# uci-cbcl/RP-Net

Hardware: AMD Instinct MI355X
Metric: support/query pairs/sec (fwd+bwd, 1-shot 256x256, T=5) (higher is better)
Workload: dtype f32

## Files before the change

include/rpnet_abi.h:

```cpp
#ifndef RPNET_ABI_H
#define RPNET_ABI_H

#include <stddef.h>
#include <stdint.h>

#ifdef __cplusplus
extern "C" {
#endif

typedef void* rpnet_stream_t;

enum rpnet_status {
    RPNET_OK = 0,
    RPNET_ERR_SHAPE = -1,
    RPNET_ERR_ARG = -2,
    RPNET_ERR_WORKSPACE = -3
};

#define RPNET_ABI_VERSION 109
int rpnet_version(void);
const char* rpnet_last_error_string(void);

int rpnet_pack_conv_weight(const float* w, float* wp, float* wd, int cout, int cin, int taps,
                           int cin_off0, int cin_split, int cin_off1, int cin_pad, rpnet_stream_t stream);

int rpnet_split_bf16(const float* x, const float* scale, int scale_mode, void* out, size_t rows, int C, int planes,
                     rpnet_stream_t stream);
int rpnet_predict_scales(const float* measured, float* bound, float* scale, int n, float safety, int check, int* violations,
                         rpnet_stream_t stream);
int rpnet_pow2_scale(const float* bound, float* s_out, rpnet_stream_t stream);
int rpnet_split_f16(const float* x, const float* mask, int mask_mode, const float* s_a, const float* s_b, float* s_out,
                    void* out, size_t rows, int C, int planes ,
                    int a_is_bound ,
                    rpnet_stream_t stream);
int rpnet_pack_conv_weight_split(const float* w, void* wp, void* wd, int cout, int cin, int taps, int cin_off0,
                                 int cin_split, int cin_off1, int cin_pad, int planes, float* row_scale_wp,
                                 float* row_scale_wd, rpnet_stream_t stream);
typedef struct rpnet_pack_item {
    const float* w; void* wp; void* wd;
    float* row_scale_wp; float* row_scale_wd;
    int cout, cin, taps, cin_off0, cin_split, cin_off1, cin_pad;
} rpnet_pack_item;
int rpnet_pack_conv_weights_split(const rpnet_pack_item* items, int n, int planes, rpnet_stream_t stream);

typedef struct rpnet_conv_desc {
    const float* x0; const float* x1;
    int C0, C1;
    const float* w;
    const float* bias;
    const float* in_scale;
    int in_scale_mode;
    float* y0; float* y1;
    int Co0, Co1;
    const float* ep_scale; const float* ep_shift;
    int ep_relu;
    const float* out_scale;
    int out_scale_mode;
    int accumulate;
    int N, H, W;
    int taps;
    int upsample;
    int groups;
    int dilation;
    double* stats_partial;
    int split_planes;
    void* y_split;
    int split_out_planes;
    const float* acc_scale_col; const float* acc_scale_x; const float* acc_scale_dy;
    const float* bnb_y; const float* bnb_stats; double* bnb_partial; float* bnb_pmax; int bnb_groups;
    const float* acc_scale_x1;
    float* out_absmax;
    int tune;
    const float* y_split_scale;
    void* splitk_ws;
    size_t splitk_ws_bytes;
    const float* skip_mask; int skip_mode; int skip_halo; unsigned char* skip_ws;
    const unsigned char* tile_skip;
    const float* y_enc; int y_enc_stride;
} rpnet_conv_desc;

int rpnet_conv_fwd(const rpnet_conv_desc* d, rpnet_stream_t stream);
int rpnet_conv_stats_blocks(const rpnet_conv_desc* d);
int rpnet_conv_tile_variant(const rpnet_conv_desc* d);
size_t rpnet_conv_splitk_workspace_bytes(const rpnet_conv_desc* d);

int rpnet_upconv_collapse_weights(const float* w, float* wc, int Cout, int Cin, rpnet_stream_t stream);
int rpnet_conv_up4_supported(const rpnet_conv_desc* d, int mode);
int rpnet_conv_up4_stats_blocks(const rpnet_conv_desc* d);
int rpnet_conv_up4(const rpnet_conv_desc* d, int mode, rpnet_stream_t stream);
int rpnet_conv_wgrad_up4_supported(const rpnet_conv_desc* d);
size_t rpnet_conv_wgrad_up4_workspace_bytes(int N, int H, int W, int cin, int cout);
int rpnet_conv_wgrad_up4(const rpnet_conv_desc* d, const void* dy, float* dw, void* workspace, size_t workspace_bytes,
                         rpnet_stream_t stream);

size_t rpnet_conv_wgrad_workspace_bytes(int N, int H, int W, int cin_gathered, int cout, int taps);
int rpnet_conv_wgrad(const rpnet_conv_desc* d, const float* dy, float* dw, int cin_w,
                     int cin_off0, int cin_split, int cin_off1,
                     void* workspace, size_t workspace_bytes, rpnet_stream_t stream);

int rpnet_conv1_fwd(const float* x, const float* w , const float* bias, float* y,
                    const float* ep_scale, const float* ep_shift, int N, int H, int W, int cout,
                    float* out_absmax ,
                    double* stats_partial ,
                    int groups, rpnet_stream_t stream);
int rpnet_conv1_stats_blocks(int N, int H, int W, int cout, int groups);
size_t rpnet_conv1_wgrad_workspace_bytes(int N, int H, int W, int cout);
int rpnet_conv1_wgrad(const float* x, const float* dy, float* dw, int N, int H, int W, int cout,
                      void* workspace, size_t workspace_bytes, rpnet_stream_t stream);
int rpnet_conv1_wgrad_bn(const float* x, const float* dz, const float* y ,
                         const float* stats, const float* coef, float* dw,
                         int N, int H, int W, int cout, int groups, void* workspace, size_t workspace_bytes,
                         const float* w , const float* bias, rpnet_stream_t stream);
int rpnet_conv1_bn_relu(const float* x, const float* w, const float* bias, const float* scale ,
                        const float* shift, float* z, void* z_split, int planes, const float* gamma, const float* beta,
                        float* split_scale, int N, int H, int W, int cout, int groups, rpnet_stream_t stream);
int rpnet_conv1_bn_bwd_rows(int N, int H, int W, int cout, int groups);
int rpnet_conv1_bn_bwd_partial(const float* x, const float* w, const float* bias, const float* dz,
                               const float* stats , double* partial,
                               int N, int H, int W, int cout, int groups, rpnet_stream_t stream);
int rpnet_conv1_dgrad_bn(const float* dz, const float* y, const float* stats, const float* coef, const float* w,
                         const float* bias, const float* x, float* dx, int N, int H, int W, int cout, int groups,
                         rpnet_stream_t stream);

size_t rpnet_bn_workspace_bytes(int C, int groups);
size_t rpnet_bn_bwd_coef_offset(int C, int groups);
int rpnet_bn_stats(const float* y, int N, int HW, int C, int groups, const float* gamma, const float* beta,
                   float* running_mean, float* running_var, long long* num_batches_tracked,
                   float momentum, float eps, float* scale, float* shift, float* mean, float* invstd,
                   void* workspace, size_t workspace_bytes, rpnet_stream_t stream);
int rpnet_bn_stats_from_partial(const double* partial, int nblk, int N, int HW, int C, int groups,
                                const float* gamma, const float* beta, float* running_mean, float* running_var,
                                long long* num_batches_tracked, float momentum, float eps, float* scale, float* shift, float* mean, float* invstd,
                                rpnet_stream_t stream);
int rpnet_bn_eval_affine(const float* gamma, const float* beta, const float* running_mean,
                         const float* running_var, float eps, float* scale, float* shift, int C,
                         rpnet_stream_t stream);
int rpnet_bn_relu(const float* y, const float* scale, const float* shift, float* z, void* z_split, int planes,
                  const float* gamma, const float* beta, float* split_scale, int N, int HW, int C, int groups,
                  int pool_w, const float* y_dec, int y_dec_stride, rpnet_stream_t stream);
int rpnet_bn_act_scale(const float* gamma, const float* beta, float* split_scale, int N, int HW, int C, int groups,
                       rpnet_stream_t stream);
int rpnet_bn_bwd(const float* dz, const float* y, const float* gamma, const float* scale, const float* shift,
                 const float* mean, const float* invstd, float* dy, void* dy_split, int planes, float* split_scale,
                 float* dgamma, float* dbeta, int N, int HW, int C, int groups, int accumulate,
                 const double* given_partial, const float* given_pmax, int given_rows ,
                 int pool_w, void* workspace, size_t workspace_bytes, const float* y_dec , int y_dec_stride,
                 rpnet_stream_t stream);

int rpnet_bn_eval_relu(const float* y, const float* scale, const float* shift, float* z, float* out_absmax, size_t P, int C,
                       rpnet_stream_t stream);
int rpnet_bn_eval_bwd(const float* dz, const float* y, const float* scale, const float* shift, const float* mean,
                      const float* invstd, float* dy, void* dy_split, int planes, float* split_scale, float* dgamma,
                      float* dbeta, int N, int HW, int C, int groups, int accumulate, void* workspace, size_t workspace_bytes,
                      rpnet_stream_t stream);

size_t rpnet_bias_relu_bwd_workspace_bytes(int C);
int rpnet_bias_relu_bwd(const float* dz, const float* z, float* dy, float* db, size_t P, int C,
                        void* workspace, size_t workspace_bytes, rpnet_stream_t stream);
int rpnet_maxpool3_fwd(const float* z, float* out, int N, int H, int W, int C, int stride, rpnet_stream_t stream);
int rpnet_maxpool3_bwd(const float* z, const float* dpool, float* dz, int N, int H, int W, int C, int stride,
                       rpnet_stream_t stream);

int rpnet_maxpool2_fwd(const float* z, float* out, int N, int H, int W, int C, rpnet_stream_t stream);
int rpnet_maxpool2_bwd(const float* z, const float* dpool, const float* skip, float* dz, int N, int H, int W,
                       int C, rpnet_stream_t stream);
int rpnet_upsample2_bwd(const float* dyu, float* dx, int N, int H, int W, int C, rpnet_stream_t stream);
int rpnet_sum_n(const float* const* srcs, int n, float* out, size_t numel, rpnet_stream_t stream);

int rpnet_mask_avgpool(const float* mask, float* out, int B, int H, int W, int scale, rpnet_stream_t stream);

int rpnet_local_corr_fwd(const float* f1, const float* f2, float* corr, int B, int h, int w, int C, int r,
                         int cstride, rpnet_stream_t stream);
size_t rpnet_local_corr_bwd_workspace_bytes(int B, int h, int w, int cstride);
int rpnet_local_corr_bwd(const float* f1, const float* f2, const float* dcorr, float* df1, float* df2,
                         int B, int h, int w, int C, int r, int cstride, const float* df1_add,
                         void* workspace, size_t workspace_bytes, rpnet_stream_t stream);
int rpnet_local_corr_split_fwd(const void* f1_split, const void* f2_split, float* corr, int B, int h, int w, int C, int r,
                               int cstride, int planes, const float* scale1, const float* scale2,
                               float* out_absmax ,
                               void* corr_planes ,
                               const float* corr_plane_scale, rpnet_stream_t stream);
int rpnet_local_corr_split_bwd(const void* f1_split, const void* f2_split, const float* dcorr, float* df1, float* df2,
                               int B, int h, int w, int C, int r, int cstride, int planes, const float* scale1,
                               const float* scale2, const float* df1_add, void* workspace, size_t workspace_bytes,
                               rpnet_stream_t stream);

int rpnet_mask_adjoint(const float* masks, float* am, float* msum, int B, int nmask, int H, int W, int h, int w,
                       rpnet_stream_t stream);
size_t rpnet_masked_pool_workspace_bytes(int B, int nmask, int hw, int C);
int rpnet_masked_pool_fwd(const float* f, const float* am, const float* msum, float* proto, int B, int nmask,
                          int hw, int C, void* workspace, size_t workspace_bytes, rpnet_stream_t stream);
int rpnet_masked_pool_bwd(const float* dproto, const float* am, const float* msum, float* df, int B, int nmask,
                          int hw, int C, int accumulate, rpnet_stream_t stream);

int rpnet_cosine_match_fwd(const float* f, const float* proto, float* pred, int B, int K, int hw, int C,
                           float scaler, rpnet_stream_t stream);
size_t rpnet_cosine_match_bwd_workspace_bytes(int B, int K, int hw, int C);
int rpnet_cosine_match_bwd(const float* f, const float* proto, const float* dpred, float* df, float* dproto,
                           int B, int K, int hw, int C, float scaler, int accumulate_df,
                           void* workspace, size_t workspace_bytes, rpnet_stream_t stream);

int rpnet_bilinear_up_fwd(const float* in, float* out, int planes, int h, int w, int H, int W, rpnet_stream_t stream);
int rpnet_bilinear_up_bwd(const float* dout, float* din, int planes, int h, int w, int H, int W, rpnet_stream_t stream);

int rpnet_softmax_thresh_pool(const float* logits, float* mask, int B, int K, int H, int W, int scale, int soft,
                              rpnet_stream_t stream);

int rpnet_refine_glue_supported(int K, int h, int w, int F, int C, int planes);
int rpnet_refine_glue_fwd(const float* y, const float* bn_scale, const float* bn_shift, const float* proto, float scaler,
                          float* z, float* pred, float* logits, float* mask_next, int soft, const float* x,
                          const float* x_scale, void* xk_planes, void* xq_planes, int planes, int B, int K, int h, int w,
                          int F, int C, rpnet_stream_t stream);
size_t rpnet_refine_glue_bwd_workspace_bytes(int B, int K, int h, int w, int F);
int rpnet_refine_glue_bwd(const float* dlogits, const float* f, const float* proto, float scaler, float* df, float* dproto,
                          int B, int K, int h, int w, int F, void* workspace, size_t workspace_bytes, rpnet_stream_t stream);

int rpnet_rowdot_scale(const float* g, const float* x, const float* scale, float* dx, float* dscale, size_t P, int C,
                       int mode, int accumulate_dscale, rpnet_stream_t stream);
int rpnet_softmax_pool_bwd(const float* logits, const float* dmask, float* dlogits, int B, int K, int H, int W,
                           int scale, rpnet_stream_t stream);

size_t rpnet_loss_workspace_bytes(int B, int K, int H, int W);
int rpnet_dice_ce_fwd(const float* logits, const int64_t* labels, float* loss, float* stats, int B, int K, int H,
                      int W, int with_dice, int ignore_index, int per_sample, const float* sample_weight,
                      void* workspace, size_t workspace_bytes, rpnet_stream_t stream);
int rpnet_dice_ce_bwd(const float* logits, const int64_t* labels, const float* stats, const float* gscale,
                      float* dlogits, int B, int K, int H, int W, int with_dice, int ignore_index, int per_sample,
                      const float* sample_weight, int accumulate, rpnet_stream_t stream);
int rpnet_dice_ce_multi_fwd(const float* const* logits, int n, const int64_t* labels, float* loss, float* stats, int B,
                            int K, int H, int W, void* workspace, size_t workspace_bytes, rpnet_stream_t stream);
int rpnet_dice_ce_multi_bwd(const float* const* logits, float* const* dlogits, int n, const int64_t* labels,
                            const float* stats, const float* gscale, int B, int K, int H, int W, rpnet_stream_t stream);
int rpnet_objective_fwd(const float* const* logits, const float* weights, int n, const int64_t* labels, const float* extra,
                        float extra_scale, float* loss, float* stats, int B, int K, int H, int W, void* workspace,
                        size_t workspace_bytes, rpnet_stream_t stream);
// ... 31 lines not shown
```

rpnet_amd/csrc/conv_epilogue.h:

```cpp
#pragma once
#include "common.h"
#include "split_bf16.h"

namespace rpnet {

struct LinearRows {
    static constexpr bool kAlwaysValid = false;
    int m0, M;
    __device__ __forceinline__ int operator()(int local) const { const int r = m0 + local; return r < M ? r : -1; }
};
template <int TW>
struct PatchRows {
    static constexpr bool kAlwaysValid = true;
    int base, W;
    __device__ __forceinline__ int operator()(int local) const { return base + (local / TW) * W + (local % TW); }
};

template <int WN, int WGM>
constexpr int epilogue_lds_bytes() {
    constexpr int stats = WGM * 64 * WN * (2 * 8 + 4), slabs = WGM * 2 * 32 * (WN * 32 + 4) * 4;
    return stats > slabs ? stats : slabs;
}
constexpr int cmax(int a, int b) { return a > b ? a : b; }

template <int WM, int WN, typename RowMap, bool AFF, bool ROWOPS>
__device__ __forceinline__ float conv_epilogue_store(const rpnet_conv_desc& d, f32x16 (&acc)[WM][WN], const RowMap rows, const int M,
                                                     const int Cout, const int per_group, const int n0, const int wm,
                                                     const int wn, const int li, const int h, float* slab, const int cso = 0) {
    constexpr int SW = WN * 32 + 4;
    const int lane = li + 32 * h;
    const int colbase = n0 + wn * WN * 32;
    const float xs = d.acc_scale_x ? *d.acc_scale_x : 1.f;
    float* dstb;
    int Cd, cd0;
    if (colbase < d.Co0) { dstb = d.y0; Cd = d.Co0; cd0 = colbase; } else { dstb = d.y1; Cd = d.Co1; cd0 = colbase - d.Co0; }
    float asv[WN], bvv[WN], es[WN], eh[WN];
    const int r_first = rows(wm * WM * 32), r_last = rows(wm * WM * 32 + WM * 32 - 1);
    const int g0 = (r_first >= 0 ? r_first : 0) / per_group;
    const bool one_group = !AFF || !d.ep_scale || RowMap::kAlwaysValid || (r_last >= 0 && r_last / per_group == g0);
#pragma unroll
    for (int j = 0; j < WN; ++j) {
        const int col = colbase + j * 32 + li;
        bvv[j] = d.bias ? d.bias[col] : 0.f;
        asv[j] = d.acc_scale_col ? d.acc_scale_col[col + cso] * xs : xs;
        es[j] = 1.f;
        eh[j] = 0.f;
        if (AFF && d.ep_scale) {
            es[j] = d.ep_scale[g0 * Cout + col];
            eh[j] = d.ep_shift[g0 * Cout + col];
        }
    }
    float amax = 0.f;
    constexpr int NQA = WN * 4;
    float sc_all[ROWOPS ? WM : 1][NQA];
    if (ROWOPS && d.out_scale_mode) {
#pragma unroll
        for (int i = 0; i < WM; ++i)
#pragma unroll
            for (int q = 0; q < NQA; ++q) {
                const int row = rows(wm * WM * 32 + i * 32 + (q * 64 + lane) / (WN * 8));
                const float f = (RowMap::kAlwaysValid || row >= 0) ? d.out_scale[row] : 0.f;
                sc_all[i][q] = d.out_scale_mode == 2 ? 1.f - f : f;
            }
    }
    unsigned short* ys = reinterpret_cast<unsigned short*>(d.y_split);
    const size_t yplane = (size_t)M * Cout;
    const float ysinv = (ROWOPS && d.y_split && d.y_split_scale) ? 1.f / *d.y_split_scale : 1.f;
#pragma unroll
    for (int i = 0; i < WM; ++i) {
#pragma unroll
        for (int r = 0; r < 16; ++r) {
            const int rl = (r & 3) + 8 * (r >> 2) + 4 * h;
#pragma unroll
            for (int j = 0; j < WN; ++j) {
                float v = acc[i][j][r] * asv[j] + bvv[j];
                if (AFF) {
                    if (one_group) v = v * es[j] + eh[j];
                    else {
                        const int row = rows(wm * WM * 32 + i * 32 + rl);
                        const int g = (row >= 0 ? row : 0) / per_group;
                        const int col = colbase + j * 32 + li;
                        v = v * d.ep_scale[g * Cout + col] + d.ep_shift[g * Cout + col];
                    }
                    if (d.ep_relu) v = fmaxf(v, 0.f);
                }
                slab[rl * SW + j * 32 + li] = v;
            }
        }
        __builtin_amdgcn_wave_barrier();
        constexpr int NQ = WN * 4;
        int orow[NQ];
        f32x4 v4[NQ];
#pragma unroll
        for (int q = 0; q < NQ; ++q) {
            const int gidx = q * 64 + lane;
            const int rr = gidx / (WN * 8), c4 = gidx - rr * (WN * 8);
            orow[q] = rows(wm * WM * 32 + i * 32 + rr);
            v4[q] = *reinterpret_cast<const f32x4*>(&slab[rr * SW + c4 * 4]);
        }
        if (ROWOPS) {
            if (d.out_scale_mode) {
#pragma unroll
                for (int q = 0; q < NQ; ++q) v4[q] *= sc_all[ROWOPS ? i : 0][q];
            }
            if (d.accumulate) {
                f32x4 prev[NQ];
#pragma unroll
                for (int q = 0; q < NQ; ++q) {
                    const int c4 = (q * 64 + lane) % (WN * 8);
                    prev[q] = (RowMap::kAlwaysValid || orow[q] >= 0) ? *reinterpret_cast<const f32x4*>(dstb + (size_t)orow[q] * Cd + cd0 + c4 * 4)
                                                                     : f32x4{0.f, 0.f, 0.f, 0.f};
                }
#pragma unroll
                for (int q = 0; q < NQ; ++q) v4[q] += prev[q];
            }
#pragma unroll
            for (int q = 0; q < NQ; ++q)
                if (RowMap::kAlwaysValid || orow[q] >= 0)
                    amax = fmaxf(fmaxf(amax, fmaxf(fabsf(v4[q][0]), fabsf(v4[q][1]))), fmaxf(fabsf(v4[q][2]), fabsf(v4[q][3])));
            if (d.y_split) {
#pragma unroll
                for (int q = 0; q < NQ; ++q) {
                    const int gidx = q * 64 + lane;
                    const int rr = gidx / (WN * 8), c4 = gidx - rr * (WN * 8);
                    *reinterpret_cast<f32x4*>(&slab[rr * SW + c4 * 4]) = v4[q];
                }
            }
        }
#pragma unroll
        for (int q = 0; q < NQ; ++q) {
            const int c4 = (q * 64 + lane) % (WN * 8);
            if (RowMap::kAlwaysValid || orow[q] >= 0)
                *reinterpret_cast<f32x4*>(dstb + (size_t)orow[q] * Cd + cd0 + c4 * 4) = v4[q];
        }
        __builtin_amdgcn_wave_barrier();
        if (ROWOPS && d.y_split) {
#pragma unroll
            for (int q = 0; q < 2 * WN; ++q) {
                const int gidx = q * 64 + lane;
                const int rr = gidx / (WN * 4), cg = gidx - rr * (WN * 4);
                const int row = rows(wm * WM * 32 + i * 32 + rr);
                if (RowMap::kAlwaysValid || row >= 0) {
                    const f32x4 a = *reinterpret_cast<const f32x4*>(&slab[rr * SW + cg * 8]);
                    const f32x4 b = *reinterpret_cast<const f32x4*>(&slab[rr * SW + cg * 8 + 4]);
                    float v8[8] = {a[0], a[1], a[2], a[3], b[0], b[1], b[2], b[3]};
                    const size_t o = (size_t)row * Cout + colbase + cg * 8;
                    if (d.split_out_planes == 3) {
                        u32x4 pl[3];
                        split8<3>(v8, pl);
#pragma unroll
                        for (int p = 0; p < 3; ++p) *reinterpret_cast<u32x4*>(ys + p * yplane + o) = pl[p];
                    } else {
#pragma unroll
                        for (int k = 0; k < 8; ++k) v8[k] *= ysinv;
                        if (d.split_out_planes == 2) {
                            u32x4 pl[2];
                            split8<2>(v8, pl);
#pragma unroll
                            for (int p = 0; p < 2; ++p) *reinterpret_cast<u32x4*>(ys + p * yplane + o) = pl[p];
                        } else {
                            u32x4 pl[1];
                            split8<1>(v8, pl);
                            *reinterpret_cast<u32x4*>(ys + o) = pl[0];
                        }
                    }
                }
            }
            __builtin_amdgcn_wave_barrier();
        }
    }
    return amax;
}

template <int WM, int WN, int WGM = 2, typename RowMap = LinearRows, bool WIDE = false>
__device__ __forceinline__ void conv_epilogue(const rpnet_conv_desc& d, f32x16 (&acc)[WM][WN], const RowMap rows,
                                              const int M, const int Cout, const int HW, const int n0, const int tm,
                                              const int wm, const int wn, const int li, const int h, void* lds, const int cso = 0) {
    const int per_group = d.groups > 0 ? (d.N / d.groups) * HW : M;
    const float xs = d.acc_scale_x ? *d.acc_scale_x : 1.f;
    if (d.stats_partial) {
        constexpr int BNC = 64 * WN;
        double* red = reinterpret_cast<double*>(lds);
        __syncthreads();
        bool valid[WM][16];
#pragma unroll
        for (int i = 0; i < WM; ++i)
#pragma unroll
            for (int r = 0; r < 16; ++r)
                valid[i][r] = RowMap::kAlwaysValid || rows(wm * WM * 32 + i * 32 + (r & 3) + 8 * (r >> 2) + 4 * h) >= 0;
#pragma unroll
        for (int j = 0; j < WN; ++j) {
            const int col = n0 + wn * WN * 32 + j * 32 + li;
            const float bv = d.bias ? d.bias[col] : 0.f;
            const float as = d.acc_scale_col ? d.acc_scale_col[col + cso] * xs : xs;
            double sm = 0.0, sq = 0.0;
#pragma unroll
            for (int i = 0; i < WM; ++i)
#pragma unroll
                for (int r = 0; r < 16; ++r) {
                    const double v = valid[i][r] ? (double)(acc[i][j][r] * as + bv) : 0.0;
                    sm += v;
                    sq += v * v;
                }
            sm += __shfl_xor(sm, 32, 64);
            sq += __shfl_xor(sq, 32, 64);
            if (h == 0) {
                double* o = red + ((size_t)wm * BNC + wn * WN * 32 + j * 32 + li) * 2;
                o[0] = sm;
                o[1] = sq;
            }
        }
        __syncthreads();
        for (int e = threadIdx.x; e < BNC * 2; e += WGM * 128) {
            double sacc = 0.0;
#pragma unroll
            for (int r = 0; r < WGM; ++r) sacc += red[(size_t)r * BNC * 2 + e];
            d.stats_partial[((size_t)tm * Cout + n0) * 2 + e] = sacc;
        }
    }
    __syncthreads();
    float* slab = reinterpret_cast<float*>(lds) + (size_t)(wm * 2 + wn) * 32 * (WN * 32 + 4);
    const bool aff = d.ep_scale != nullptr || d.ep_relu != 0;
    const bool rowops = d.out_scale_mode != 0 || d.accumulate != 0 || d.out_absmax != nullptr || d.y_split != nullptr;
    float amax = 0.f;
    if (!aff && !rowops) conv_epilogue_store<WM, WN, RowMap, false, false>(d, acc, rows, M, Cout, per_group, n0, wm, wn, li, h, slab, cso);
    else if (!aff) amax = conv_epilogue_store<WM, WN, RowMap, false, true>(d, acc, rows, M, Cout, per_group, n0, wm, wn, li, h, slab, cso);
    else if (!rowops) conv_epilogue_store<WM, WN, RowMap, true, false>(d, acc, rows, M, Cout, per_group, n0, wm, wn, li, h, slab, cso);
    else amax = conv_epilogue_store<WM, WN, RowMap, true, true>(d, acc, rows, M, Cout, per_group, n0, wm, wn, li, h, slab, cso);
    if (d.out_absmax) {
#pragma unroll
        for (int o = 32; o > 0; o >>= 1) amax = fmaxf(amax, __shfl_xor(amax, o, 64));
        if ((threadIdx.x & 63) == 0 && amax > __hip_atomic_load(d.out_absmax, __ATOMIC_RELAXED, __HIP_MEMORY_SCOPE_AGENT))
            atomicMax(reinterpret_cast<unsigned*>(d.out_absmax), __float_as_uint(amax));
    }
}

}
```

rpnet_amd/csrc/conv_igemm.hip:

```cpp
#include "conv_epilogue.h"

namespace rpnet {

template <int WM, int WN, bool INSCALE>
__global__ __launch_bounds__(256, (WM * WN >= 8 ? 2 : (WM * WN == 4 ? 3 : 4))) void conv_igemm_kernel(const rpnet_conv_desc d, const int M,
                                                          const int Cin, const int Cout,
                                                          const int tiles_n, const int ntiles) {
    constexpr int BM = 64 * WM, BN = 64 * WN, BK = 32;
    constexpr int ASTR = BK + 4;
    constexpr int A_F4 = BM / 32;
    constexpr int B_F4 = BN / 32;
    __shared__ __attribute__((aligned(16))) float smem[cmax(BM * ASTR + BK * BN, epilogue_lds_bytes<WN, 2>() / 4)];

    const int t = threadIdx.x;
    const int lane = t & 63, wv = t >> 6;
    const int li = lane & 31, h = lane >> 5;
    const int wm = wv >> 1, wn = wv & 1;

    const int tile = xcd_swizzle(blockIdx.x, ntiles);
    const int tm = tile / tiles_n, tn = tile - tm * tiles_n;
    const int m0 = tm * BM, n0 = tn * BN;

    const int H = d.H, W = d.W, HW = H * W;
    const int ups = d.upsample;
    const int Hs = H >> ups, Ws = W >> ups;
    const int dil = d.dilation > 1 ? d.dilation : 1;

    int rn[A_F4], ry[A_F4], rx[A_F4];
#pragma unroll
    for (int j = 0; j < A_F4; ++j) {
        const int m = m0 + (t >> 3) + 32 * j;
        if (m < M) {
            const int n = m / HW, rem = m - n * HW;
            rn[j] = n;
            ry[j] = rem / W;
            rx[j] = rem - ry[j] * W;
        } else {
            rn[j] = -1; ry[j] = 0; rx[j] = 0;
        }
    }
    const int acol = (t & 7) * 4;
    const int kchunks = Cin >> 5;
    const int nsteps = d.taps * kchunks;
    const int Cin4 = Cin >> 2;

    const int rot = (int)(blockIdx.x % (unsigned)kchunks);
    int l_tap = 0, l_c0 = rot << 5, l_kc = 0;
    const __amdgpu_buffer_rsrc_t rs0 = __builtin_amdgcn_make_buffer_rsrc(
        const_cast<float*>(d.x0), (short)0, (int)((size_t)d.N * Hs * Ws * d.C0 * 4), 0x00020000);
    const __amdgpu_buffer_rsrc_t rs1 = __builtin_amdgcn_make_buffer_rsrc(
        const_cast<float*>(d.x1 ? d.x1 : d.x0), (short)0, (int)((size_t)d.N * Hs * Ws * (d.x1 ? d.C1 : d.C0) * 4), 0x00020000);
    const __amdgpu_buffer_rsrc_t rsw = __builtin_amdgcn_make_buffer_rsrc(
        const_cast<float*>(d.w), (short)0, (int)((size_t)d.taps * Cin * Cout * 4), 0x00020000);
    int roff[A_F4];
    float rsc[A_F4];
    auto tap_setup = [&](int tap) {
        int ky = 0, kx = 0;
        if (d.taps == 9) { ky = (tap / 3 - 1) * dil; kx = (tap - (tap / 3) * 3 - 1) * dil; }
#pragma unroll
        for (int j = 0; j < A_F4; ++j) {
            const int iy = ry[j] + ky, ix = rx[j] + kx;
            const bool inb = rn[j] >= 0 && iy >= 0 && iy < H && ix >= 0 && ix < W;
            const int pix = (rn[j] * Hs + (iy >> ups)) * Ws + (ix >> ups);
            roff[j] = inb ? pix : -1;
            if (INSCALE) {
                const float sv = d.in_scale[inb ? pix : 0];
                rsc[j] = d.in_scale_mode == 2 ? 1.f - sv : sv;
            }
        }
    };
    tap_setup(0);
    int wvoff[B_F4];
#pragma unroll
    for (int j = 0; j < B_F4; ++j) {
        const int idx = t + 256 * j;
        const int k4 = idx / BN, nn = idx - k4 * BN;
        wvoff[j] = (k4 * Cout + nn) * 16;
    }

    f32x4 ra[A_F4], rb[B_F4];
    float rsc_st[A_F4];
    auto load_tile = [&]() {
        const bool first = l_c0 < d.C0;
        const int Cs = first ? d.C0 : d.C1;
        const int cc = first ? l_c0 : l_c0 - d.C0;
        const int soff = cc * 4;
        const int cs4 = Cs * 4, ac4 = acol * 4;
#pragma unroll
        for (int j = 0; j < A_F4; ++j) {
            const int voff = roff[j] * cs4 + ac4;
            ra[j] = first ? __builtin_bit_cast(f32x4, __builtin_amdgcn_raw_buffer_load_b128(rs0, voff, soff, 0))
                          : __builtin_bit_cast(f32x4, __builtin_amdgcn_raw_buffer_load_b128(rs1, voff, soff, 0));
            if (INSCALE) rsc_st[j] = rsc[j];
        }
        const int wsoff = ((l_tap * Cin4 + (l_c0 >> 2)) * Cout + n0) * 16;
#pragma unroll
        for (int j = 0; j < B_F4; ++j)
            rb[j] = __builtin_bit_cast(f32x4, __builtin_amdgcn_raw_buffer_load_b128(rsw, wvoff[j], wsoff, 0));
        l_c0 += 32;
        if (l_c0 == Cin) l_c0 = 0;
        if (++l_kc == kchunks) {
            l_kc = 0;
            if (++l_tap < d.taps) tap_setup(l_tap);
        }
    };
    auto store_tile = [&]() {
        float* As = smem;
        float* Bs = As + BM * ASTR;
#pragma unroll
        for (int j = 0; j < A_F4; ++j)
            *reinterpret_cast<f32x4*>(&As[((t >> 3) + 32 * j) * ASTR + acol]) = INSCALE ? ra[j] * rsc_st[j] : ra[j];
#pragma unroll
        for (int j = 0; j < B_F4; ++j) *reinterpret_cast<f32x4*>(&Bs[(t + 256 * j) * 4]) = rb[j];
    };

    f32x16 acc[WM][WN];
#pragma unroll
    for (int i = 0; i < WM; ++i)
#pragma unroll
        for (int j = 0; j < WN; ++j)
#pragma unroll
            for (int r = 0; r < 16; ++r) acc[i][j][r] = 0.f;

    auto mma_group = [&](const float* As, const float* Bs, int g) {
        f32x4 af[WM], bf[WN];
#pragma unroll
        for (int i = 0; i < WM; ++i)
            af[i] = *reinterpret_cast<const f32x4*>(&As[(wm * WM * 32 + i * 32 + li) * ASTR + g * 8 + h * 4]);
#pragma unroll
        for (int j = 0; j < WN; ++j)
            bf[j] = *reinterpret_cast<const f32x4*>(&Bs[((g * 2 + h) * BN + wn * WN * 32 + j * 32 + li) * 4]);
#pragma unroll
        for (int q = 0; q < 4; ++q)
#pragma unroll
            for (int i = 0; i < WM; ++i)
#pragma unroll
                for (int j = 0; j < WN; ++j)
                    acc[i][j] = __builtin_amdgcn_mfma_f32_32x32x2f32(af[i][q], bf[j][q], acc[i][j], 0, 0, 0);
    };

    load_tile();
    store_tile();
    __syncthreads();
    const float* As = smem;
    const float* Bs = As + BM * ASTR;
    for (int ks = 0; ks < nsteps; ++ks) {
        const bool more = ks + 1 < nsteps;
        if (more) load_tile();
        mma_group(As, Bs, 0);
        mma_group(As, Bs, 1);
        mma_group(As, Bs, 2);
        mma_group(As, Bs, 3);
        __syncthreads();
        if (more) store_tile();
        __syncthreads();
    }

    conv_epilogue<WM, WN>(d, acc, LinearRows{m0, M}, M, Cout, HW, n0, tm, wm, wn, li, h, smem);
}

template <int WM, int WN, bool INSCALE>
static int launch_igemm_t(const rpnet_conv_desc* d, int M, int Cin, int Cout, hipStream_t s) {
    constexpr int BM = 64 * WM, BN = 64 * WN;
    const int tiles_m = cdiv(M, BM), tiles_n = Cout / BN;
    const int ntiles = tiles_m * tiles_n;
    hipLaunchKernelGGL((conv_igemm_kernel<WM, WN, INSCALE>), dim3(ntiles), dim3(256), 0, s, *d, M, Cin, Cout, tiles_n, ntiles);
    return check_launch("conv_igemm");
}

template <int WM, int WN>
static int launch_igemm(const rpnet_conv_desc* d, int M, int Cin, int Cout, hipStream_t s) {
    if (d->in_scale_mode) return launch_igemm_t<WM, WN, true>(d, M, Cin, Cout, s);
    return launch_igemm_t<WM, WN, false>(d, M, Cin, Cout, s);
}

int choose_tile_split(const rpnet_conv_desc* d, int M, int Cout);
int split_tile_rows(int variant, int* wave_rows);
int conv_fwd_split(const rpnet_conv_desc* d, int M, int Cin, int Cout, hipStream_t s);
size_t conv_splitk_bytes(const rpnet_conv_desc* d, int M, int Cin, int Cout);

}


static int choose_tile(const rpnet_conv_desc* d, int M, int Cout) {
    const bool n128 = (Cout % 128 == 0) && (d->Co1 == 0 || d->Co0 % 128 == 0);
    struct Cand { int wm, wn, slots; } cands[4] = {{2, 2, 768}, {2, 1, 1024}, {1, 2, 1024}, {1, 1, 1536}};
    int best = -1;
    double best_fill = -1.0;
    for (int c = 0; c < 4; ++c) {
        if (cands[c].wn == 2 && !n128) continue;
        const long tiles = (long)rpnet::cdiv(M, 64 * cands[c].wm) * (Cout / (64 * cands[c].wn));
        const long waves = (tiles + cands[c].slots - 1) / cands[c].slots;
        const double fill = (double)tiles / (double)(waves * cands[c].slots);
        if (fill > best_fill + 0.02) { best_fill = fill; best = c; }
    }
    return best;
}

extern "C" int rpnet_conv_stats_blocks(const rpnet_conv_desc* d) {
    if (!d || d->groups < 1 || d->N % d->groups) return 0;
    const int M = d->N * d->H * d->W, Cout = d->Co0 + d->Co1;
    int bm, wave_rows = 2;
    if (d->split_planes) {
        bm = rpnet::split_tile_rows(rpnet::choose_tile_split(d, M, Cout), &wave_rows);
    } else {
        const int best = choose_tile(d, M, Cout);
        bm = (best == 0 || best == 1) ? 128 : 64;
    }
    const long per_group = (long)(d->N / d->groups) * d->H * d->W;
    if (per_group % bm) return 0;
    return (int)(per_group / bm);
}

extern "C" int rpnet_conv_tile_variant(const rpnet_conv_desc* d) {
    if (!d || !d->split_planes) return -1;
    return rpnet::choose_tile_split(d, d->N * d->H * d->W, d->Co0 + d->Co1);
}

extern "C" size_t rpnet_conv_splitk_workspace_bytes(const rpnet_conv_desc* d) {
    if (!d || !d->split_planes || d->taps != 9) return 0;
    return rpnet::conv_splitk_bytes(d, d->N * d->H * d->W, d->C0 + d->C1, d->Co0 + d->Co1);
}

extern "C" int rpnet_conv_fwd(const rpnet_conv_desc* d, rpnet_stream_t stream) {
    using namespace rpnet;
    RPNET_REQUIRE(d && d->x0 && d->w && d->y0, RPNET_ERR_ARG, "conv_fwd: null pointer");
    const int Cin = d->C0 + d->C1, Cout = d->Co0 + d->Co1;
    RPNET_REQUIRE(d->taps == 9 || d->taps == 1, RPNET_ERR_ARG, "conv_fwd: taps must be 9 or 1");
    RPNET_REQUIRE(Cin % 32 == 0 && d->C0 % 32 == 0 && (d->C1 == 0 || d->x1), RPNET_ERR_SHAPE,
                  "conv_fwd: Cin (%d+%d) must be a multiple of 32 per source", d->C0, d->C1);
    RPNET_REQUIRE(Cout % 64 == 0 && (d->Co1 == 0 || (d->y1 && d->Co0 % 64 == 0)), RPNET_ERR_SHAPE,
                  "conv_fwd: Cout (%d+%d) must be a multiple of 64 per destination", d->Co0, d->Co1);
    RPNET_REQUIRE(!d->stats_partial || rpnet_conv_stats_blocks(d) > 0, RPNET_ERR_SHAPE,
                  "conv_fwd: statistic groups do not split into whole tiles; use rpnet_bn_stats");
    RPNET_REQUIRE(!d->upsample || (d->H % 2 == 0 && d->W % 2 == 0), RPNET_ERR_SHAPE, "conv_fwd: odd size with upsample");
    RPNET_REQUIRE(!d->y_split || (d->Co1 == 0 && d->split_out_planes >= 1 && d->split_out_planes <= 3), RPNET_ERR_ARG,
                  "conv_fwd: y_split needs a single destination and 1 to 3 planes");
    RPNET_REQUIRE(!d->y_split || d->split_out_planes == 3 || d->y_split_scale, RPNET_ERR_ARG,
                  "conv_fwd: fp16 output planes (split_out_planes 1 / 2) need y_split_scale");
    RPNET_REQUIRE(!d->y_enc && !d->y_enc_stride, RPNET_ERR_ARG, "conv_fwd: y_enc / y_enc_stride are reserved (must be NULL / 0)");
    RPNET_REQUIRE(!d->bnb_y && !d->bnb_stats && !d->bnb_partial && !d->bnb_pmax, RPNET_ERR_ARG, "conv_fwd: the bnb_* fields are reserved (must be NULL)");
    RPNET_REQUIRE((long)d->N * d->H * d->W < (1L << 31), RPNET_ERR_SHAPE, "conv_fwd: too many pixels");
    RPNET_REQUIRE((size_t)d->N * d->H * d->W * (d->C0 > d->C1 ? d->C0 : d->C1) * 4 < (1UL << 31) &&
                      (size_t)d->taps * Cin * Cout * 4 < (1UL << 31),
                  RPNET_ERR_SHAPE, "conv_fwd: a source tensor exceeds the 2 GiB buffer-descriptor range");
    const int M = d->N * d->H * d->W;
    hipStream_t s = (hipStream_t)stream;
    if (d->split_planes) {
        RPNET_REQUIRE(d->split_planes >= 1 && d->split_planes <= 3 && d->in_scale_mode == 0, RPNET_ERR_ARG,
                      "conv_fwd: split operands take 1 to 3 planes and no in_scale (fold it into rpnet_split_bf16 / _f16)");
        RPNET_REQUIRE(d->split_planes == 3 || (d->acc_scale_col && d->acc_scale_x), RPNET_ERR_ARG,
                      "conv_fwd: one / two planes are fp16 planes of operand / scale: acc_scale_col and acc_scale_x are required");
        return conv_fwd_split(d, M, Cin, Cout, s);
    }
    const int best = choose_tile(d, M, Cout);
    switch (best) {
        case 0: return launch_igemm<2, 2>(d, M, Cin, Cout, s);
        case 1: return launch_igemm<2, 1>(d, M, Cin, Cout, s);
        case 2: return launch_igemm<1, 2>(d, M, Cin, Cout, s);
        default: return launch_igemm<1, 1>(d, M, Cin, Cout, s);
    }
}
```

rpnet_amd/csrc/conv_split.hip:

```cpp
#include <algorithm>

#include "conv_epilogue.h"
#include "split_bf16.h"

namespace rpnet {

constexpr bool IGLP = true;

template <int NP>
__global__ __launch_bounds__(256) void split_bf16_kernel(const float* __restrict__ x, const float* __restrict__ scale,
                                                          const int mode, unsigned short* __restrict__ out,
                                                          const size_t n8, const FastDiv fC, const size_t plane_elems) {
    RPNET_PASS_PRIORITY();
    for (size_t i = (size_t)blockIdx.x * 256 + threadIdx.x; i < n8; i += (size_t)gridDim.x * 256) {
        const f32x4 a = *reinterpret_cast<const f32x4*>(x + i * 8);
        const f32x4 b = *reinterpret_cast<const f32x4*>(x + i * 8 + 4);
        float v[8] = {a[0], a[1], a[2], a[3], b[0], b[1], b[2], b[3]};
        if (mode) {
            float s = scale[fC.div((unsigned)i)];
            if (mode == 2) s = 1.f - s;
#pragma unroll
            for (int q = 0; q < 8; ++q) v[q] *= s;
        }
        u32x4 o[NP];
// ... 240 lines not shown
    int roff[AJ];
    auto tap_setup = [&](int tap) {
        int ky = 0, kx = 0;
        if (d.taps == 9) { ky = (tap / 3 - 1) * dil; kx = (tap - (tap / 3) * 3 - 1) * dil; }
#pragma unroll
        for (int j = 0; j < AJ; ++j) {
            const int iy = ry[j] + ky, ix = rx[j] + kx;
            const bool inb = rn[j] >= 0 && iy >= 0 && iy < H && ix >= 0 && ix < W;
            roff[j] = inb ? (rn[j] * Hs + (iy >> ups)) * Ws + (ix >> ups) : -1;
        }
    };
    tap_setup(0);
    const bool stage_b = !B_PART || srow < BN;
    int wvoff[BJ];
#pragma unroll
    for (int j = 0; j < BJ; ++j) wvoff[j] = stage_b ? (srow + RP * j) * 64 + skg * 16 : -1;

    u32x4 ra[NP][AJ], rb[NP][BJ];
    auto load_tile = [&]() {
        const bool first = l_c0 < d.C0;
        const int Cs = first ? d.C0 : d.C1;
        const int cc = first ? l_c0 : l_c0 - d.C0;
        const int soff = cc * 2;
#pragma unroll
        for (int j = 0; j < AJ; ++j) {
            const int voff = roff[j] * (Cs * 2) + skg * 16;
#pragma unroll
            for (int p = 0; p < NP; ++p)
                ra[p][j] = first ? __builtin_bit_cast(u32x4, __builtin_amdgcn_raw_buffer_load_b128(rs0[p], voff, soff, 0))
                                 : __builtin_bit_cast(u32x4, __builtin_amdgcn_raw_buffer_load_b128(rs1[p], voff, soff, 0));
        }
        const int wsoff = ((l_tap * kchunks + (l_c0 >> 5)) * Cout + n0) * 64;
#pragma unroll
        for (int j = 0; j < BJ; ++j)
#pragma unroll
            for (int p = 0; p < NP; ++p)
                rb[p][j] = __builtin_bit_cast(u32x4, __builtin_amdgcn_raw_buffer_load_b128(rsw[p], wvoff[j], wsoff, 0));
        l_c0 += 32;
        if (l_c0 == Cin) l_c0 = 0;
        if (++l_kc == kchunks) {
            l_kc = 0;
            if (++l_tap < d.taps) tap_setup(l_tap);
        }
    };
    const int sdst = srow * 64 + 16 * (skg ^ ((srow >> 2) & 3));
    auto store_tile = [&](unsigned char* st) {
#pragma unroll
        for (int p = 0; p < NP; ++p) {
#pragma unroll
            for (int j = 0; j < AJ; ++j)
                *reinterpret_cast<u32x4*>(st + p * A_BYTES + j * (RP * 64) + sdst) = ra[p][j];
            if (stage_b) {
#pragma unroll
                for (int j = 0; j < BJ; ++j)
                    *reinterpret_cast<u32x4*>(st + NP * A_BYTES + p * B_BYTES + j * (RP * 64) + sdst) = rb[p][j];
            }
        }
    };

    f32x16 acc[WM][WN];
#pragma unroll
    for (int i = 0; i < WM; ++i)
#pragma unroll
        for (int j = 0; j < WN; ++j)
#pragma unroll
            for (int r = 0; r < 16; ++r) acc[i][j][r] = 0.f;

    const int sw = (li >> 2) & 3;
    const int a_row = (wm * WM * 32 + li) * 64, b_row = (wn * WN * 32 + li) * 64;
    auto mma_slice = [&](const unsigned char* st, int s) {
        const int koff = 16 * ((2 * s + h) ^ sw);
        bf16x8 af[NP][WM], bfr[NP][WN];
#pragma unroll
        for (int p = 0; p < NP; ++p) {
#pragma unroll
            for (int i = 0; i < WM; ++i)
                af[p][i] = *reinterpret_cast<const bf16x8*>(st + p * A_BYTES + a_row + i * 2048 + koff);
#pragma unroll
            for (int j = 0; j < WN; ++j)
                bfr[p][j] = *reinterpret_cast<const bf16x8*>(st + NP * A_BYTES + p * B_BYTES + b_row + j * 2048 + koff);
        }
        constexpr int NPROD = nprod<NP>();
#pragma unroll
        for (int q = 0; q < NPROD; ++q) {
            const int pa = prod_a<NP>(q), pb = prod_b<NP>(q);
#pragma unroll
            for (int i = 0; i < WM; ++i)
#pragma unroll
                for (int j = 0; j < WN; ++j)
                    acc[i][j] = mma16<NP>(af[pa][i], bfr[pb][j], acc[i][j]);
        }
    };

    const bool two_scales = d.acc_scale_x1 != nullptr && d.C1 > 0;
    const float r01 = two_scales ? *d.acc_scale_x / *d.acc_scale_x1 : 1.f;
    int cur_src = 0;
    auto enter_tile = [&](int ks) {
        if (!two_scales) return;
        int c = rot + ks;
        c -= (c / kchunks) * kchunks;
        const int src = (c << 5) < d.C0 ? 0 : 1;
        if (src != cur_src) {
            const float f = src ? r01 : 1.f / r01;
#pragma unroll
            for (int i = 0; i < WM; ++i)
#pragma unroll
                for (int j = 0; j < WN; ++j)
#pragma unroll
                    for (int r = 0; r < 16; ++r) acc[i][j][r] *= f;
            cur_src = src;
        }
    };
    if (DB) {
        load_tile();
        store_tile(smem);
        if (nsteps > 1) load_tile();
        __syncthreads();
        for (int ks = 0; ks < nsteps; ++ks) {
            enter_tile(ks);
            unsigned char* cur = smem + (ks & 1) * STAGE;
            unsigned char* nxt = smem + ((ks + 1) & 1) * STAGE;
            if (ks + 1 < nsteps) {
                store_tile(nxt);
                if (ks + 2 < nsteps) load_tile();
            }
            mma_slice(cur, 0);
            mma_slice(cur, 1);
            __syncthreads();
        }
    } else {
        load_tile();
        store_tile(smem);
        __syncthreads();
        for (int ks = 0; ks < nsteps; ++ks) {
            enter_tile(ks);
            const bool more = ks + 1 < nsteps;
            if (more) load_tile();
            mma_slice(smem, 0);
            mma_slice(smem, 1);
            __syncthreads();
            if (more) store_tile(smem);
            __syncthreads();
        }
    }
    if (two_scales && cur_src) {
        const float f = 1.f / r01;
#pragma unroll
        for (int i = 0; i < WM; ++i)
#pragma unroll
            for (int j = 0; j < WN; ++j)
#pragma unroll
                for (int r = 0; r < 16; ++r) acc[i][j][r] *= f;
    }
    conv_epilogue<WM, WN, WGM, LinearRows, NP == 1>(d, acc, LinearRows{m0, M}, M, Cout, HW, n0, tm, wm, wn, li, h, smem);
}

template <int TW, int NP, int WN>
__global__ __launch_bounds__(512, 1) void conv_igemm_split_halo_kernel(const rpnet_conv_desc d, const int Cin, const int Cout,
                                                                        const int tiles_n, const int ntiles) {
    constexpr int NT = 512, BM = 256, BN = 64 * WN, TH = BM / TW, PW = TW + 2, HALO = (TH + 2) * PW;
    constexpr int A_BYTES = HALO * 64, B_BYTES = BN * 64;
    constexpr int HJ = (HALO * 4 + NT - 1) / NT;
    constexpr int WM = 2;
    __shared__ __attribute__((aligned(16))) unsigned char smem[cmax(NP * A_BYTES + 2 * NP * B_BYTES, epilogue_lds_bytes<WN, 4>())];
    unsigned char* const bsm = smem + NP * A_BYTES;

    const int t = threadIdx.x;
    const int lane = t & 63, wv = t >> 6;
    const int li = lane & 31, h = lane >> 5;
    const int wm = wv >> 1, wn = wv & 1;

    const int tile = xcd_swizzle(blockIdx.x, ntiles);
    const int tm = tile / tiles_n, tn = tile - tm * tiles_n;
    const int n0 = tn * BN;
    const int H = d.H, W = d.W, HW = H * W;
    const int ups = d.upsample;
    const int Hs = H >> ups, Ws = W >> ups;
    const int pxn = W / TW, ppi = (H / TH) * pxn;
    const int n = tm / ppi, prem = tm - n * ppi;
    const int y0 = (prem / pxn) * TH, x0 = (prem % pxn) * TW;

    int hoff[HJ], hdst[HJ];
#pragma unroll
    for (int j = 0; j < HJ; ++j) {
        const int e = t + NT * j;
        const int hr = e >> 2, kg = e & 3;
        const int hy = hr / PW, hx = hr - hy * PW;
        const int iy = y0 + hy - 1, ix = x0 + hx - 1;
        const bool inb = e < HALO * 4 && iy >= 0 && iy < H && ix >= 0 && ix < W;
        hoff[j] = inb ? (n * Hs + (iy >> ups)) * Ws + (ix >> ups) : -1;
        hdst[j] = e < HALO * 4 ? hr * 64 + 16 * (kg ^ ((hr >> 2) & 3)) : -1;
    }
    const int skg16 = (t & 3) * 16;
    const int kchunks = Cin >> 5;
    const int nsteps = 9 * kchunks;
    const int rot = (int)(blockIdx.x % (unsigned)kchunks);
    auto chunk_c0 = [&](int ci) { int c = rot + ci; if (c >= kchunks) c -= kchunks; return c << 5; };

    const size_t plane0 = (size_t)d.N * Hs * Ws * d.C0, plane1 = (size_t)d.N * Hs * Ws * d.C1;
    const size_t planew = (size_t)9 * Cin * Cout;
    const unsigned short* x0p = reinterpret_cast<const unsigned short*>(d.x0);
    const unsigned short* x1p = reinterpret_cast<const unsigned short*>(d.x1 ? d.x1 : d.x0);
    const unsigned short* wq = reinterpret_cast<const unsigned short*>(d.w);
    __amdgpu_buffer_rsrc_t rs0[NP], rs1[NP], rsw[NP];
#pragma unroll
    for (int p = 0; p < NP; ++p) {
        rs0[p] = __builtin_amdgcn_make_buffer_rsrc(const_cast<unsigned short*>(x0p + p * plane0), (short)0,
                                                   (int)(plane0 * 2), 0x00020000);
        rs1[p] = __builtin_amdgcn_make_buffer_rsrc(const_cast<unsigned short*>(x1p + p * (d.x1 ? plane1 : plane0)), (short)0,
                                                   (int)((d.x1 ? plane1 : plane0) * 2), 0x00020000);
        rsw[p] = __builtin_amdgcn_make_buffer_rsrc(const_cast<unsigned short*>(wq + p * planew), (short)0,
                                                   (int)(planew * 2), 0x00020000);
    }
    u32x4 ha[NP][HJ], rb[NP];
    auto load_halo = [&](int c0) {
        const bool first = c0 < d.C0;
        const int Cs = first ? d.C0 : d.C1;
        const int soff = (first ? c0 : c0 - d.C0) * 2;
#pragma unroll
        for (int j = 0; j < HJ; ++j) {
            const int voff = hoff[j] * (Cs * 2) + skg16;
#pragma unroll
            for (int p = 0; p < NP; ++p)
                ha[p][j] = first ? __builtin_bit_cast(u32x4, __builtin_amdgcn_raw_buffer_load_b128(rs0[p], voff, soff, 0))
                                 : __builtin_bit_cast(u32x4, __builtin_amdgcn_raw_buffer_load_b128(rs1[p], voff, soff, 0));
        }
    };
    auto store_halo = [&]() {
#pragma unroll
        for (int p = 0; p < NP; ++p)
#pragma unroll
            for (int j = 0; j < HJ; ++j)
                if (hdst[j] >= 0) *reinterpret_cast<u32x4*>(smem + p * A_BYTES + hdst[j]) = ha[p][j];
    };
    const int brow = t >> 2;
    const bool stage_b = brow < BN;
    const int wvoff = stage_b ? brow * 64 + skg16 : -1;
    const int bdst = brow * 64 + 16 * ((t & 3) ^ ((brow >> 2) & 3));
    auto load_b = [&](int tap, int c0) {
        const int wsoff = ((tap * kchunks + (c0 >> 5)) * Cout + n0) * 64;
#pragma unroll
        for (int p = 0; p < NP; ++p)
            rb[p] = __builtin_bit_cast(u32x4, __builtin_amdgcn_raw_buffer_load_b128(rsw[p], wvoff, wsoff, 0));
    };
    auto store_b = [&](int stage) {
        if (stage_b) {
#pragma unroll
            for (int p = 0; p < NP; ++p) *reinterpret_cast<u32x4*>(bsm + (stage * NP + p) * B_BYTES + bdst) = rb[p];
        }
    };

    f32x16 acc[WM][WN];
#pragma unroll
    for (int i = 0; i < WM; ++i)
#pragma unroll
        for (int j = 0; j < WN; ++j)
#pragma unroll
            for (int r = 0; r < 16; ++r) acc[i][j][r] = 0.f;

    int hr00[WM];
#pragma unroll
    for (int i = 0; i < WM; ++i) {
        const int mloc = (wm * WM + i) * 32 + li;
        hr00[i] = (mloc / TW) * PW + (mloc % TW);
    }
    const int sw = (li >> 2) & 3;
    const int b_row = (wn * WN * 32 + li) * 64;
    auto mma_tap = [&](int tap, int stage) {
        const int ky = tap / 3, kx = tap - ky * 3;
        int arow[WM], asw[WM];
#pragma unroll
        for (int i = 0; i < WM; ++i) {
            const int hr = hr00[i] + ky * PW + kx;
            arow[i] = hr * 64;
            asw[i] = (hr >> 2) & 3;
        }
        const unsigned char* bst = bsm + stage * NP * B_BYTES;
#pragma unroll
        for (int s = 0; s < 2; ++s) {
            const int kg = 2 * s + h;
            bf16x8 af[NP][WM], bfr[NP][WN];
#pragma unroll
            for (int p = 0; p < NP; ++p) {
#pragma unroll
                for (int i = 0; i < WM; ++i)
                    af[p][i] = *reinterpret_cast<const bf16x8*>(smem + p * A_BYTES + arow[i] + 16 * (kg ^ asw[i]));
#pragma unroll
                for (int j = 0; j < WN; ++j)
                    bfr[p][j] = *reinterpret_cast<const bf16x8*>(bst + p * B_BYTES + b_row + j * 2048 + 16 * (kg ^ sw));
            }
            constexpr int NPROD = nprod<NP>();
#pragma unroll
            for (int q = 0; q < NPROD; ++q) {
                const int pa = prod_a<NP>(q), pb = prod_b<NP>(q);
#pragma unroll
                for (int i = 0; i < WM; ++i)
#pragma unroll
                    for (int j = 0; j < WN; ++j)
                        acc[i][j] = mma16<NP>(af[pa][i], bfr[pb][j], acc[i][j]);
            }
            if (NP <= 2 && IGLP) __builtin_amdgcn_iglp_opt(0);
        }
    };

    load_halo(chunk_c0(0));
    store_halo();
    load_b(0, chunk_c0(0));
    store_b(0);
    load_b(1, chunk_c0(0));
    __syncthreads();
    int ci = 0, tap = 0;
    for (int ks = 0; ks < nsteps; ++ks) {
        if (ks + 1 < nsteps) {
            store_b((ks + 1) & 1);
            if (ks + 2 < nsteps) {
                int t2 = tap + 2, c2 = ci;
                if (t2 >= 9) { t2 -= 9; ++c2; }
                load_b(t2, chunk_c0(c2));
            }
        }
        const bool next_chunk = ci + 1 < kchunks;
        if (tap == 0 && next_chunk) load_halo(chunk_c0(ci + 1));
        mma_tap(tap, ks & 1);
        __syncthreads();
        if (++tap == 9) {
            tap = 0;
            ++ci;
            if (next_chunk) {
                store_halo();
                __syncthreads();
            }
        }
    }
    conv_epilogue<WM, WN, 4, PatchRows<TW>, NP == 1>(d, acc, PatchRows<TW>{(n * H + y0) * W + x0, W}, d.N * HW, Cout, HW, n0, tm, wm, wn,
                                            li, h, smem);
}

template <int TW, int NP, int WN, int WMT = 2>
__global__ __launch_bounds__(256, 2) void conv_igemm_split_halo4_kernel(const rpnet_conv_desc d, const int Cin, const int Cout,
                                                                        const int tiles_n, const int ntiles) {
    constexpr int NT = 256, BM = 64 * WMT, BN = 64 * WN, TH = BM / TW, PW = TW + 2, HALO = (TH + 2) * PW;
    constexpr int A_BYTES = HALO * 64, B_BYTES = BN * 64;
    constexpr int HJ = (HALO * 4 + NT - 1) / NT;
    constexpr int WM = WMT;
    constexpr int BJ = (BN * 4 + NT - 1) / NT;
    __shared__ __attribute__((aligned(16))) unsigned char smem[cmax(NP * A_BYTES + NP * B_BYTES, epilogue_lds_bytes<WN, 2>())];
    unsigned char* const bsm = smem + NP * A_BYTES;

    const int t = threadIdx.x;
    const int lane = t & 63, wv = t >> 6;
    const int li = lane & 31, h = lane >> 5;
    const int wm = wv >> 1, wn = wv & 1;

    const int tile = xcd_swizzle(blockIdx.x, ntiles);
    const int tm = tile / tiles_n, tn = tile - tm * tiles_n;
    const int n0 = tn * BN;
    const int H = d.H, W = d.W, HW = H * W;
    const int ups = d.upsample;
    const int Hs = H >> ups, Ws = W >> ups;
    const int pxn = W / TW, ppi = (H / TH) * pxn;
    const int n = tm / ppi, prem = tm - n * ppi;
    const int y0 = (prem / pxn) * TH, x0 = (prem % pxn) * TW;

    int hoff[HJ], hdst[HJ];
#pragma unroll
    for (int j = 0; j < HJ; ++j) {
        const int e = t + NT * j;
        const int hr = e >> 2, kg = e & 3;
        const int hy = hr / PW, hx = hr - hy * PW;
        const int iy = y0 + hy - 1, ix = x0 + hx - 1;
        const bool inb = e < HALO * 4 && iy >= 0 && iy < H && ix >= 0 && ix < W;
        hoff[j] = inb ? (n * Hs + (iy >> ups)) * Ws + (ix >> ups) : -1;
        hdst[j] = e < HALO * 4 ? hr * 64 + 16 * (kg ^ ((hr >> 2) & 3)) : -1;
    }
    const int skg16 = (t & 3) * 16;
    const int kchunks = Cin >> 5;
    const int nsteps = 9 * kchunks;
    const int rot = (int)(blockIdx.x % (unsigned)kchunks);
    auto chunk_c0 = [&](int ci) { int c = rot + ci; if (c >= kchunks) c -= kchunks; return c << 5; };

    const size_t plane0 = (size_t)d.N * Hs * Ws * d.C0, plane1 = (size_t)d.N * Hs * Ws * d.C1;
    const size_t planew = (size_t)9 * Cin * Cout;
    const unsigned short* x0p = reinterpret_cast<const unsigned short*>(d.x0);
    const unsigned short* x1p = reinterpret_cast<const unsigned short*>(d.x1 ? d.x1 : d.x0);
    const unsigned short* wq = reinterpret_cast<const unsigned short*>(d.w);
    __amdgpu_buffer_rsrc_t rs0[NP], rs1[NP], rsw[NP];
#pragma unroll
    for (int p = 0; p < NP; ++p) {
        rs0[p] = __builtin_amdgcn_make_buffer_rsrc(const_cast<unsigned short*>(x0p + p * plane0), (short)0,
                                                   (int)(plane0 * 2), 0x00020000);
        rs1[p] = __builtin_amdgcn_make_buffer_rsrc(const_cast<unsigned short*>(x1p + p * (d.x1 ? plane1 : plane0)), (short)0,
                                                   (int)((d.x1 ? plane1 : plane0) * 2), 0x00020000);
        rsw[p] = __builtin_amdgcn_make_buffer_rsrc(const_cast<unsigned short*>(wq + p * planew), (short)0,
                                                   (int)(planew * 2), 0x00020000);
    }
    u32x4 ha[NP][HJ], rb[NP][BJ];
    auto load_halo = [&](int c0) {
        const bool first = c0 < d.C0;
        const int Cs = first ? d.C0 : d.C1;
        const int soff = (first ? c0 : c0 - d.C0) * 2;
#pragma unroll
        for (int j = 0; j < HJ; ++j) {
            const int voff = hoff[j] * (Cs * 2) + skg16;
#pragma unroll
            for (int p = 0; p < NP; ++p)
                ha[p][j] = first ? __builtin_bit_cast(u32x4, __builtin_amdgcn_raw_buffer_load_b128(rs0[p], voff, soff, 0))
                                 : __builtin_bit_cast(u32x4, __builtin_amdgcn_raw_buffer_load_b128(rs1[p], voff, soff, 0));
        }
    };
    auto store_halo = [&]() {
#pragma unroll
        for (int p = 0; p < NP; ++p)
#pragma unroll
            for (int j = 0; j < HJ; ++j)
                if (hdst[j] >= 0) *reinterpret_cast<u32x4*>(smem + p * A_BYTES + hdst[j]) = ha[p][j];
    };
    const int brow = t >> 2;
    const bool stage_b = brow < BN;
    const int bdst = brow * 64 + 16 * ((t & 3) ^ ((brow >> 2) & 3));
    auto load_b = [&](int tap, int c0) {
        const int wsoff = ((tap * kchunks + (c0 >> 5)) * Cout + n0) * 64;
#pragma unroll
        for (int j = 0; j < BJ; ++j) {
            const int wvoff = (brow + 64 * j) < BN ? (brow + 64 * j) * 64 + skg16 : -1;
#pragma unroll
            for (int p = 0; p < NP; ++p)
                rb[p][j] = __builtin_bit_cast(u32x4, __builtin_amdgcn_raw_buffer_load_b128(rsw[p], wvoff, wsoff, 0));
        }
    };
    auto store_b = [&]() {
#pragma unroll
        for (int j = 0; j < BJ; ++j)
            if (brow + 64 * j < BN) {
#pragma unroll
                for (int p = 0; p < NP; ++p) *reinterpret_cast<u32x4*>(bsm + p * B_BYTES + j * 4096 + bdst) = rb[p][j];
            }
    };
    (void)stage_b;

    f32x16 acc[WM][WN];
#pragma unroll
    for (int i = 0; i < WM; ++i)
#pragma unroll
        for (int j = 0; j < WN; ++j)
#pragma unroll
            for (int r = 0; r < 16; ++r) acc[i][j][r] = 0.f;

    int hr00[WM];
#pragma unroll
    for (int i = 0; i < WM; ++i) {
        const int mloc = (wm * WM + i) * 32 + li;
        hr00[i] = (mloc / TW) * PW + (mloc % TW);
    }
    const int sw = (li >> 2) & 3;
    const int b_row = (wn * WN * 32 + li) * 64;
    auto mma_tap = [&](int tap, int stage) {
        const int ky = tap / 3, kx = tap - ky * 3;
        int arow[WM], asw[WM];
#pragma unroll
        for (int i = 0; i < WM; ++i) {
            const int hr = hr00[i] + ky * PW + kx;
            arow[i] = hr * 64;
            asw[i] = (hr >> 2) & 3;
        }
        const unsigned char* bst = bsm + stage * NP * B_BYTES;
#pragma unroll
        for (int s = 0; s < 2; ++s) {
            const int kg = 2 * s + h;
            bf16x8 af[NP][WM], bfr[NP][WN];
#pragma unroll
            for (int p = 0; p < NP; ++p) {
#pragma unroll
                for (int i = 0; i < WM; ++i)
                    af[p][i] = *reinterpret_cast<const bf16x8*>(smem + p * A_BYTES + arow[i] + 16 * (kg ^ asw[i]));
#pragma unroll
                for (int j = 0; j < WN; ++j)
                    bfr[p][j] = *reinterpret_cast<const bf16x8*>(bst + p * B_BYTES + b_row + j * 2048 + 16 * (kg ^ sw));
            }
            constexpr int NPROD = nprod<NP>();
#pragma unroll
            for (int q = 0; q < NPROD; ++q) {
                const int pa = prod_a<NP>(q), pb = prod_b<NP>(q);
#pragma unroll
                for (int i = 0; i < WM; ++i)
#pragma unroll
                    for (int j = 0; j < WN; ++j)
                        acc[i][j] = mma16<NP>(af[pa][i], bfr[pb][j], acc[i][j]);
            }
        }
    };

    load_halo(chunk_c0(0));
    store_halo();
    load_b(0, chunk_c0(0));
    store_b();
    __syncthreads();
    int ci = 0, tap = 0;
    for (int ks = 0; ks < nsteps; ++ks) {
        const bool more = ks + 1 < nsteps;
        const bool next_chunk = ci + 1 < kchunks;
        if (more) {
            int t1 = tap + 1, c1 = ci;
            if (t1 == 9) { t1 = 0; ++c1; }
            load_b(t1, chunk_c0(c1));
        }
        if (WMT == 2 && tap == 0 && next_chunk) load_halo(chunk_c0(ci + 1));
        mma_tap(tap, 0);
        __syncthreads();
        if (more) store_b();
        if (tap == 8 && next_chunk) {
            if (WMT != 2) load_halo(chunk_c0(ci + 1));
            store_halo();
        }
        __syncthreads();
        if (++tap == 9) { tap = 0; ++ci; }
    }
    conv_epilogue<WM, WN, 2, PatchRows<TW>, NP == 1>(d, acc, PatchRows<TW>{(n * H + y0) * W + x0, W}, d.N * HW, Cout, HW, n0, tm, wm, wn,
                                            li, h, smem);
}

template <int TW, int WN>
static int launch_split_halo(const rpnet_conv_desc* d, int M, int Cin, int Cout, hipStream_t s) {
    const int tiles_m = M / 256, tiles_n = Cout / (64 * WN);
    const int ntiles = tiles_m * tiles_n;
    if (d->split_planes == 3)
        hipLaunchKernelGGL((conv_igemm_split_halo_kernel<TW, 3, WN>), dim3(ntiles), dim3(512), 0, s, *d, Cin, Cout, tiles_n, ntiles);
    else if (d->split_planes == 2)
        hipLaunchKernelGGL((conv_igemm_split_halo_kernel<TW, 2, WN>), dim3(ntiles), dim3(512), 0, s, *d, Cin, Cout, tiles_n, ntiles);
    else
        hipLaunchKernelGGL((conv_igemm_split_halo_kernel<TW, 1, WN>), dim3(ntiles), dim3(512), 0, s, *d, Cin, Cout, tiles_n, ntiles);
    return check_launch("conv_igemm_split_halo");
}

template <int TW, int WN, int WMT = 2>
static int launch_split_halo4(const rpnet_conv_desc* d, int M, int Cin, int Cout, hipStream_t s) {
    const int tiles_m = M / (64 * WMT), tiles_n = Cout / (64 * WN);
    const int ntiles = tiles_m * tiles_n;
    if (d->split_planes == 3) {
        if constexpr (WMT == 2)
            hipLaunchKernelGGL((conv_igemm_split_halo4_kernel<TW, 3, WN, WMT>), dim3(ntiles), dim3(256), 0, s, *d, Cin, Cout, tiles_n, ntiles);
        else {
            set_error("conv_igemm_split_halo4: the 4-wave 256-pixel form exists for fp16 planes only");
            return RPNET_ERR_ARG;
        }
    } else if (d->split_planes == 2)
        hipLaunchKernelGGL((conv_igemm_split_halo4_kernel<TW, 2, WN, WMT>), dim3(ntiles), dim3(256), 0, s, *d, Cin, Cout, tiles_n, ntiles);
    else
        hipLaunchKernelGGL((conv_igemm_split_halo4_kernel<TW, 1, WN, WMT>), dim3(ntiles), dim3(256), 0, s, *d, Cin, Cout, tiles_n, ntiles);
    return check_launch("conv_igemm_split_halo4");
}

static int halo_bn(const rpnet_conv_desc* d, int Cout) {
    return ((Cout % 128 == 0) && (d->Co1 == 0 || d->Co0 % 128 == 0)) ? 128 : 64;
}

static int halo_tw(const rpnet_conv_desc* d, int Cout) {
    if (d->taps != 9 || d->dilation > 1) return 0;
    if (d->W % 32 == 0 && d->H % 8 == 0) return 32;
    if (d->W % 16 == 0 && d->H % 16 == 0) return 16;
    return 0;
}

struct SplitVariant { int wgm, wm, wn, db, slots; };
static const SplitVariant kSplitVariants[] = {
    {2, 2, 2, 0, 768},
    {2, 2, 1, 0, 1024},
    {2, 1, 2, 0, 1024},
    {2, 1, 1, 0, 1536},
    {4, 2, 2, 1, 256},
    {4, 2, 2, 0, 256},
    {2, 2, 2, 1, 256},
    {4, 2, 2, 1, 256},
    {2, 2, 2, 0, 512},
    {2, 2, 1, 0, 512},
    {2, 4, 2, 0, 512},
    {2, 4, 2, 0, 256},
    {2, 4, 1, 0, 256},
    {2, 4, 2, 0, 256},
    {2, 2, 1, 0, 256},
};
constexpr int kNumSplitVariants = sizeof(kSplitVariants) / sizeof(kSplitVariants[0]);

template <int WGM, int WM, int WN, bool DB>
static int launch_split(const rpnet_conv_desc* d, int M, int Cin, int Cout, hipStream_t s) {
    constexpr int BM = 32 * WGM * WM, BN = 64 * WN;
    const int tiles_m = cdiv(M, BM), tiles_n = Cout / BN;
    const int ntiles = tiles_m * tiles_n;
    if (d->split_planes == 3)
        hipLaunchKernelGGL((conv_igemm_split_kernel<WGM, WM, WN, 3, DB>), dim3(ntiles), dim3(WGM * 128), 0, s, *d, M, Cin,
                           Cout, tiles_n, ntiles);
    else if (d->split_planes == 2)
        hipLaunchKernelGGL((conv_igemm_split_kernel<WGM, WM, WN, 2, DB>), dim3(ntiles), dim3(WGM * 128), 0, s, *d, M, Cin,
                           Cout, tiles_n, ntiles);
    else
        hipLaunchKernelGGL((conv_igemm_split_kernel<WGM, WM, WN, 1, DB>), dim3(ntiles), dim3(WGM * 128), 0, s, *d, M, Cin,
                           Cout, tiles_n, ntiles);
    return check_launch("conv_igemm_split");
}

static int halo4_tw(const rpnet_conv_desc* d) {
    if (d->taps != 9 || d->dilation > 1) return 0;
    if (d->W % 32 == 0 && d->H % 4 == 0) return 32;
    if (d->W % 16 == 0 && d->H % 8 == 0) return 16;
    return 0;
}

int conv_fwd_split_dma(const rpnet_conv_desc* d, int M, int Cin, int Cout, int tw, int wn, hipStream_t s, int parts = 1, int bm = 256);
int conv_splitk_parts(const rpnet_conv_desc* d, int M, int Cin, int Cout);

static bool dma_addressable(const rpnet_conv_desc* d, int Cout) {
    const size_t msrc = (size_t)d->N * (d->H >> d->upsample) * (d->W >> d->upsample);
    const size_t np = d->split_planes > 0 ? d->split_planes : 1, lim = (size_t)1 << 31;
    return np * msrc * d->C0 * 2 < lim && np * msrc * d->C1 * 2 < lim && np * 9 * (size_t)(d->C0 + d->C1) * Cout * 2 < lim;
}

int choose_tile_split(const rpnet_conv_desc* d, int M, int Cout) {
    const bool n128 = (Cout % 128 == 0) && (d->Co1 == 0 || d->Co0 % 128 == 0);
    const bool addr = dma_addressable(d, Cout);
    if (d->tune > 0) {
        const int v = (d->tune & 0xff) - 1;
        if ((v == 12 || v == 14) && d->split_planes == 2 && halo_tw(d, Cout) && addr) return v;
        if (v == 13 && d->split_planes == 1 && halo_tw(d, Cout) && halo_bn(d, Cout) == 128 && (d->C0 + d->C1) % 64 == 0 && d->C0 % 64 == 0 && addr)
            return v;
        if (((v == 7 || (v == 11 && d->split_planes == 2 && addr)) && halo_tw(d, Cout) &&
             halo_bn(d, Cout) == 128) ||
            ((v == 8 || v == 9) && halo4_tw(d)))
            return v;
        if (v >= 0 && v < 4 && (kSplitVariants[v].wn == 1 || n128)) return v;
    }
    const int hbn = halo_bn(d, Cout);
    if (d->split_planes == 1 && !(d->tune & 0x10000) && addr && hbn == 128 && halo_tw(d, Cout) && (d->C0 + d->C1) % 64 == 0 && d->C0 % 64 == 0 &&
        (long)(M / 256) * (Cout / 128) >= 192)
        return 13;
    const bool dma = d->split_planes == 2 && !(d->tune & 0x10000) && addr;
    if (hbn == 128 && halo_tw(d, Cout) && (long)(M / 256) * (Cout / 128) >= (dma ? 192 : 224)) return dma ? 11 : 7;
    if (dma && halo_tw(d, Cout) && d->C0 + d->C1 >= 128 && (long)(M / 256) * (Cout / 64) >= 128) return 12;
    if (halo4_tw(d)) {
        const long t8 = (long)(M / 128) * (Cout / hbn);
        if (hbn == 128 && t8 >= 1024) return 8;
        if ((long)(M / 128) * (Cout / 64) >= 64) return 9;
    }
    int best = -1;
    double best_fill = -1.0;
    for (int c = 0; c < 4; ++c) {
        const SplitVariant& v = kSplitVariants[c];
        if (v.wn == 2 && !n128) continue;
        const long tiles = (long)cdiv(M, 32 * v.wgm * v.wm) * (Cout / (64 * v.wn));
        const long waves = (tiles + v.slots - 1) / v.slots;
        const double fill = (double)tiles / (double)(waves * v.slots);
        if (fill > best_fill + 0.02) { best_fill = fill; best = c; }
    }
    return best;
}

int split_tile_rows(int variant, int* wave_rows) {
    const SplitVariant& v = kSplitVariants[variant];
    *wave_rows = v.wgm;
    return 32 * v.wgm * v.wm;
}

static int splitk_parts_for(const rpnet_conv_desc* d, int M, int Cin, int Cout) {
    if (!halo_tw(d, Cout) || !dma_addressable(d, Cout)) return 1;
    return conv_splitk_parts(d, M, Cin, Cout);
}

size_t conv_splitk_bytes(const rpnet_conv_desc* d, int M, int Cin, int Cout) {
    const int parts = splitk_parts_for(d, M, Cin, Cout);
    return parts > 1 ? (size_t)parts * M * Cout * sizeof(float) : 0;
}

// ... 120 lines not shown
```

rpnet_amd/csrc/conv_split_dma.hip:

```cpp
#include <type_traits>

#include "conv_epilogue.h"
#include "lds_dma.h"
#include "split_bf16.h"

namespace rpnet {

template <int N, int I = 0, typename F>
__device__ __forceinline__ void static_for(F&& f) {
    if constexpr (I < N) {
        f(std::integral_constant<int, I>{});
        static_for<N, I + 1>(f);
    }
}

template <int TW, int NP, int WN, bool K64 = false, int WM = 4>
__global__ __launch_bounds__(256, 1) void conv_igemm_split_dma_kernel(const rpnet_conv_desc d, const int Cin, const int Cout,
                                                                       const int tiles_n, const int ntiles, const int kshift) {
    constexpr int BM = 64 * WM, BN = 64 * WN, TH = BM / TW, PW = TW + 2, HALO = (TH + 2) * PW;
    constexpr int HP = (HALO + 15) / 16;
    constexpr int HPW = (HP + 3) / 4;
    constexpr int A_BYTES = HP * 1024, HBUF = NP * A_BYTES;
    constexpr int B_BYTES = BN * 64, STAGE = NP * B_BYTES;
    constexpr int NS = 4;
    constexpr int NW = WN * NP;
    static_assert(HPW <= 6, "halo pieces are issued during taps 0 .. HPW-1; the wait counts below assume HPW <= 6");
    __shared__ __attribute__((aligned(1024))) unsigned char smem[cmax(cmax(2 * HBUF + NS * STAGE, epilogue_lds_bytes<WN, 2>()),
                                                                       kLdsPerCu - kGuardedPassLds + 1024)];
    RPNET_ASSERT_NO_CORESIDENCE(sizeof(smem));
    constexpr int WOFF = 2 * HBUF;

    const int t = threadIdx.x;
    const int lane = t & 63;
    const int wv = __builtin_amdgcn_readfirstlane(t >> 6);
    const int li = lane & 31, h = lane >> 5;
    const int wm = wv >> 1, wn = wv & 1;

    const int tile = xcd_swizzle(blockIdx.x, ntiles);
    const int tm = uni(tile / tiles_n), tn = tile - tm * tiles_n;
    const int n0 = tn * BN;
    const int H = d.H, W = d.W, HW = H * W;
    const int ups = d.upsample;
    const int Hs = H >> ups, Ws = W >> ups;
    const int pxn = W / TW, ppi = (H / TH) * pxn;
    const int n = uni(tm / ppi), prem = tm - n * ppi;
    const int y0 = uni(prem / pxn) * TH, x0 = uni(prem % pxn) * TW;

    constexpr int CSH = K64 ? 6 : 5;
    const int kchunks = (Cin >> CSH) >> kshift;
    const int cbase = (int)blockIdx.y * kchunks;
    const int nsteps = 9 * kchunks;
    const int rot = uni((int)(blockIdx.x % (unsigned)kchunks));
    auto chunk_c0 = [&](int ci) { int c = rot + ci; if (c >= kchunks) c -= kchunks; return (cbase + c) << CSH; };

    const size_t plane0 = (size_t)d.N * Hs * Ws * d.C0, plane1 = (size_t)d.N * Hs * Ws * d.C1;
    const size_t planew = (size_t)9 * Cin * Cout;
    const unsigned short* x0p = reinterpret_cast<const unsigned short*>(d.x0);
    const unsigned short* x1p = reinterpret_cast<const unsigned short*>(d.x1 ? d.x1 : d.x0);
    const unsigned short* wq = reinterpret_cast<const unsigned short*>(d.w);
    const int pb0 = (int)(plane0 * 2), pb1 = (int)((d.x1 ? plane1 : plane0) * 2), pbw = (int)(planew * 2);
    constexpr int NPM = K64 ? 1 : NP;
    const __amdgpu_buffer_rsrc_t rs0 = __builtin_amdgcn_make_buffer_rsrc(const_cast<unsigned short*>(x0p), (short)0, NPM * pb0, 0x00020000);
    const __amdgpu_buffer_rsrc_t rs1 = __builtin_amdgcn_make_buffer_rsrc(const_cast<unsigned short*>(x1p), (short)0, NPM * pb1, 0x00020000);
    const __amdgpu_buffer_rsrc_t rsw = __builtin_amdgcn_make_buffer_rsrc(const_cast<unsigned short*>(wq), (short)0, NPM * pbw, 0x00020000);
    const int ps0 = K64 ? 64 : pb0, ps1 = K64 ? 64 : pb1, psw = K64 ? Cout * 64 : pbw;

    const int drow = lane >> 2;
    const int dkg16 = ((lane & 3) ^ ((lane >> 4) & 3)) * 16;
    int hoff[HPW];
    int hpos[HPW];
#pragma unroll
    for (int i = 0; i < HPW; ++i) {
        int pos = wv + 4 * i;
        if (pos >= HP) pos -= 4;
        hpos[i] = pos;
        const int hr = pos * 16 + drow;
        const int hy = hr / PW, hx = hr - hy * PW;
        const int iy = y0 + hy - 1, ix = x0 + hx - 1;
        const bool inb = hr < HALO && iy >= 0 && iy < H && ix >= 0 && ix < W;
        hoff[i] = inb ? (n * Hs + (iy >> ups)) * Ws + (ix >> ups) : -1;
    }
    auto dma_halo = [&](auto ic, int c0, int buf) {
        constexpr int i = decltype(ic)::value;
        const bool first = c0 < d.C0;
        const int Cs = first ? d.C0 : d.C1;
        const int soff = uni((first ? c0 : c0 - d.C0) * 2);
        const int voff = hoff[i] * (Cs * 2) + dkg16;
#pragma unroll
        for (int p = 0; p < NP; ++p) {
            auto* dst = (__attribute__((address_space(3))) void*)(smem + buf * HBUF + p * A_BYTES + hpos[i] * 1024);
            if (first) __builtin_amdgcn_raw_ptr_buffer_load_lds(rs0, dst, 16, voff, soff + p * ps0, 0, 0);
            else __builtin_amdgcn_raw_ptr_buffer_load_lds(rs1, dst, 16, voff, soff + p * ps1, 0, 0);
        }
    };
    const int wvoff = (16 * WN * wv + drow) * 64 + dkg16;
    auto dma_w = [&](int tap, int c0, int stage) {
        const int wsoff = uni(((tap * (Cin >> 5) + (c0 >> 5)) * Cout + n0) * 64);
#pragma unroll
        for (int p = 0; p < NP; ++p)
#pragma unroll
            for (int q = 0; q < WN; ++q) {
                auto* dst = (__attribute__((address_space(3))) void*)(smem + WOFF + stage * STAGE + p * B_BYTES + (16 * WN * wv + 16 * q) * 64);
                __builtin_amdgcn_raw_ptr_buffer_load_lds(rsw, dst, 16, wvoff + q * 1024, wsoff + p * psw, 0, 0);
            }
    };

    f32x16 acc[WM][WN];
#pragma unroll
    for (int i = 0; i < WM; ++i)
#pragma unroll
        for (int j = 0; j < WN; ++j)
#pragma unroll
            for (int r = 0; r < 16; ++r) acc[i][j][r] = 0.f;

    int hr00[WM];
#pragma unroll
    for (int i = 0; i < WM; ++i) {
        const int mloc = (wm * WM + i) * 32 + li;
        hr00[i] = (mloc / TW) * PW + (mloc % TW);
    }
    const int b_off = WOFF + (wn * WN * 32 + li) * 64 + 16 * (h ^ ((li >> 2) & 3));

    bf16x8 af[2][NP][WM], bfr[2][NP][WN];
    int aaddr[WM];
    auto a_addr_tap = [&](auto tapc) {
        constexpr int tap = decltype(tapc)::value;
        constexpr int ky = tap / 3, kx = tap - ky * 3;
#pragma unroll
        for (int i = 0; i < WM; ++i) {
            const int hr = hr00[i] + ky * PW + kx;
            aaddr[i] = hr * 64 + 16 * (h ^ ((hr >> 2) & 3));
        }
    };
    constexpr int NPROD = K64 ? 2 : nprod<NP>();
    constexpr int NR = NP * (WM + WN), NMMA = NPROD * WM * WN;
    static_assert(NR <= NMMA, "one fragment read of the next slice behind each MFMA of this one");
    auto read_frag = [&](auto sc, auto kc, const int abase, const int bbase) {
        constexpr int s = decltype(sc)::value, k = decltype(kc)::value;
        constexpr int grp = k / (WM + WN), r = k - grp * (WM + WN);
        constexpr int pa = K64 ? grp : NP - 1 - grp, pb = grp;
        if constexpr (r == 0 || r > WN) {
            constexpr int i = r == 0 ? 0 : r - WN;
            af[s][pa][i] = *reinterpret_cast<const bf16x8*>(smem + abase + (aaddr[i] ^ (32 * s)) + pa * A_BYTES);
        } else {
            constexpr int j = r - 1;
            bfr[s][pb][j] = *reinterpret_cast<const bf16x8*>(smem + bbase + (b_off ^ (32 * s)) + pb * B_BYTES + j * 2048);
        }
    };
    auto mma_one = [&](auto sc, auto mc) {
        constexpr int s = decltype(sc)::value, m = decltype(mc)::value;
        constexpr int q = m / (WM * WN), ij = m - q * (WM * WN), i = ij / WN, j = ij - i * WN;
        constexpr int pa = K64 ? q : prod_a<NP>(q), pb = K64 ? q : prod_b<NP>(q);
        acc[i][j] = mma16<NP>(af[s][pa][i], bfr[s][pb][j], acc[i][j]);
    };
    using I0 = std::integral_constant<int, 0>;
    using I1 = std::integral_constant<int, 1>;
    auto dma_w_one = [&](auto ec, const int wsoff, const int stage) {
        constexpr int e = decltype(ec)::value, p = e / WN, q = e - p * WN;
        auto* dst = (__attribute__((address_space(3))) void*)(smem + WOFF + stage * STAGE + p * B_BYTES + (16 * WN * wv + 16 * q) * 64);
        __builtin_amdgcn_raw_ptr_buffer_load_lds(rsw, dst, 16, wvoff + q * 1024, wsoff + p * psw, 0, 0);
    };

    const bool skip_tile = d.tile_skip != nullptr && d.tile_skip[tm] == 0;
    if (!skip_tile) {
    {
        const int c0 = chunk_c0(0);
        dma_halo(std::integral_constant<int, 0>{}, c0, 0);
        if constexpr (HPW > 1) dma_halo(std::integral_constant<int, 1>{}, c0, 0);
        if constexpr (HPW > 2) dma_halo(std::integral_constant<int, 2>{}, c0, 0);
        if constexpr (HPW > 3) dma_halo(std::integral_constant<int, 3>{}, c0, 0);
        if constexpr (HPW > 4) dma_halo(std::integral_constant<int, 4>{}, c0, 0);
        if constexpr (HPW > 5) dma_halo(std::integral_constant<int, 5>{}, c0, 0);
        dma_w(0, c0, 0);
        dma_w(1, c0, 1);
        dma_w(2, c0, 2);
    }
    static_assert(NW == 1 || NW == 2 || NW == 4, "weight DMAs per wave and step");
    if constexpr (NW == 4) asm volatile("s_waitcnt vmcnt(4)" ::: "memory");
    if constexpr (NW == 2) asm volatile("s_waitcnt vmcnt(2)" ::: "memory");
    if constexpr (NW == 1) asm volatile("s_waitcnt vmcnt(1)" ::: "memory");
    __builtin_amdgcn_s_barrier();
    a_addr_tap(I0{});
    static_for<NR>([&](auto kc) { read_frag(I0{}, kc, 0, 0); });

    auto step = [&](auto tapc, const int ci, const int ks) {
        constexpr int TAP = decltype(tapc)::value;
        const int hb = ci & 1;
        const bool last_chunk = ci + 1 >= kchunks;
        constexpr int t3 = TAP + 3 < 9 ? TAP + 3 : TAP - 6;
        const int c3 = chunk_c0((TAP + 3 < 9 || last_chunk) ? ci : ci + 1);
        const int wsoff = uni(((t3 * (Cin >> 5) + (c3 >> 5)) * Cout + n0) * 64);
        const int wstage = (ks + 3) & 3;
        const int abase = hb * HBUF, bbase = (ks & 3) * STAGE;
        static_for<NMMA>([&](auto mc) {
            constexpr int m = decltype(mc)::value;
            mma_one(I0{}, mc);
            __builtin_amdgcn_sched_barrier(0);
            if constexpr (m < NR) {
                read_frag(I1{}, mc, abase, bbase);
                __builtin_amdgcn_sched_barrier(0);
            }
            if constexpr (m >= NMMA - 2 * NW && (NMMA - 1 - m) % 2 == 0) {
                dma_w_one(std::integral_constant<int, NW - 1 - (NMMA - 1 - m) / 2>{}, wsoff, wstage);
                __builtin_amdgcn_sched_barrier(0);
            }
        });
        constexpr int TN = TAP < 8 ? TAP + 1 : 0;
        a_addr_tap(std::integral_constant<int, TN>{});
        const int abase_n = (TAP < 8 ? hb : hb ^ 1) * HBUF, bbase_n = ((ks + 1) & 3) * STAGE;
        __builtin_amdgcn_sched_barrier(0);
        static_for<NMMA>([&](auto mc) {
            constexpr int m = decltype(mc)::value;
            mma_one(I1{}, mc);
            __builtin_amdgcn_sched_barrier(0);
            if constexpr (m < NR) {
                read_frag(I0{}, mc, abase_n, bbase_n);
                __builtin_amdgcn_sched_barrier(0);
            }
            if constexpr (m == NMMA - 1 && TAP < HPW) {
                dma_halo(std::integral_constant<int, (TAP < HPW ? TAP : 0)>{}, chunk_c0(last_chunk ? ci : ci + 1), hb ^ 1);
                __builtin_amdgcn_sched_barrier(0);
            }
        });
        constexpr int HPREV = (TAP >= 1 && TAP - 1 < HPW) ? NP : 0;
        constexpr int HCUR = TAP < HPW ? NP : 0;
        constexpr int N = HPREV + NW + HCUR;
        static_assert(N == 1 || N == 2 || N == 3 || N == 4 || N == 6 || N == 8, "wait count");
        if constexpr (N == 1) asm volatile("s_waitcnt vmcnt(1)" ::: "memory");
        if constexpr (N == 2) asm volatile("s_waitcnt vmcnt(2)" ::: "memory");
        if constexpr (N == 3) asm volatile("s_waitcnt vmcnt(3)" ::: "memory");
        if constexpr (N == 4) asm volatile("s_waitcnt vmcnt(4)" ::: "memory");
        if constexpr (N == 6) asm volatile("s_waitcnt vmcnt(6)" ::: "memory");
        if constexpr (N == 8) asm volatile("s_waitcnt vmcnt(8)" ::: "memory");
        __builtin_amdgcn_s_barrier();
    };

    const int nchunks_run = ((d.tune >> 8) & 1) ? 1 : kchunks;
    int ks = 0;
    for (int ci = 0; ci < nchunks_run; ++ci) {
        step(std::integral_constant<int, 0>{}, ci, ks + 0);
        step(std::integral_constant<int, 1>{}, ci, ks + 1);
        step(std::integral_constant<int, 2>{}, ci, ks + 2);
        step(std::integral_constant<int, 3>{}, ci, ks + 3);
        step(std::integral_constant<int, 4>{}, ci, ks + 4);
        step(std::integral_constant<int, 5>{}, ci, ks + 5);
        step(std::integral_constant<int, 6>{}, ci, ks + 6);
        step(std::integral_constant<int, 7>{}, ci, ks + 7);
        step(std::integral_constant<int, 8>{}, ci, ks + 8);
        ks += 9;
    }
    (void)nsteps;
    asm volatile("s_waitcnt vmcnt(0)" ::: "memory");
    __builtin_amdgcn_s_barrier();
    }
    const int dbg = d.tune >> 8;
    if (dbg & 2) {
        float sacc = 0.f;
#pragma unroll
        for (int i = 0; i < WM; ++i)
#pragma unroll
            for (int j = 0; j < WN; ++j)
#pragma unroll
                for (int r = 0; r < 16; ++r) sacc += acc[i][j][r];
        if (sacc == 123.456f) d.y0[t] = sacc;
        return;
    }
    conv_epilogue<WM, WN, 2, PatchRows<TW>, false>(d, acc, PatchRows<TW>{(n * H + y0) * W + x0 + (int)blockIdx.y * d.N * HW, W},
                                                    d.N * HW, Cout, HW, n0, tm, wm, wn, li, h, smem);
}

__global__ __launch_bounds__(256) void conv_splitk_reduce_kernel(const float* __restrict__ ws, const int S, const size_t MC, const int Cout,
                                                                 const float* __restrict__ bias, const float* __restrict__ ep_scale,
                                                                 const float* __restrict__ ep_shift, const int relu, float* __restrict__ y,
                                                                 unsigned short* __restrict__ ys, const int planes,
                                                                 const float* __restrict__ ysc, float* __restrict__ out_absmax) {
    const size_t i = (size_t)blockIdx.x * 256 + threadIdx.x;
    float amax = 0.f;
    if (i * 8 < MC) {
        const int col = (int)((i * 8) % (size_t)Cout);
        f32x4 a = *reinterpret_cast<const f32x4*>(ws + i * 8), b = *reinterpret_cast<const f32x4*>(ws + i * 8 + 4);
        for (int s = 1; s < S; ++s) {
            a += *reinterpret_cast<const f32x4*>(ws + (size_t)s * MC + i * 8);
            b += *reinterpret_cast<const f32x4*>(ws + (size_t)s * MC + i * 8 + 4);
        }
        float v8[8] = {a[0], a[1], a[2], a[3], b[0], b[1], b[2], b[3]};
        if (bias) {
#pragma unroll
            for (int k = 0; k < 8; ++k) v8[k] += bias[col + k];
        }
        if (ep_scale) {
#pragma unroll
            for (int k = 0; k < 8; ++k) {
                v8[k] = v8[k] * ep_scale[col + k] + ep_shift[col + k];
                if (relu) v8[k] = fmaxf(v8[k], 0.f);
            }
        }
        *reinterpret_cast<f32x4*>(y + i * 8) = f32x4{v8[0], v8[1], v8[2], v8[3]};
        *reinterpret_cast<f32x4*>(y + i * 8 + 4) = f32x4{v8[4], v8[5], v8[6], v8[7]};
#pragma unroll
        for (int k = 0; k < 8; ++k) amax = fmaxf(amax, fabsf(v8[k]));
        if (ys) {
            if (planes == 3) {
                u32x4 pl[3];
                split8<3>(v8, pl);
#pragma unroll
                for (int p = 0; p < 3; ++p) *reinterpret_cast<u32x4*>(ys + p * MC + i * 8) = pl[p];
            } else {
                const float ysinv = 1.f / *ysc;
#pragma unroll
                for (int k = 0; k < 8; ++k) v8[k] *= ysinv;
                if (planes == 2) {
                    u32x4 pl[2];
                    split8<2>(v8, pl);
#pragma unroll
                    for (int p = 0; p < 2; ++p) *reinterpret_cast<u32x4*>(ys + p * MC + i * 8) = pl[p];
                } else {
                    u32x4 pl[1];
                    split8<1>(v8, pl);
                    *reinterpret_cast<u32x4*>(ys + i * 8) = pl[0];
                }
            }
        }
    }
    if (out_absmax) {
        __shared__ float wave_max[4];
#pragma unroll
        for (int o = 32; o > 0; o >>= 1) amax = fmaxf(amax, __shfl_xor(amax, o, 64));
        if ((threadIdx.x & 63) == 0) wave_max[threadIdx.x >> 6] = amax;
        __syncthreads();
        if (threadIdx.x == 0) {
            amax = fmaxf(fmaxf(wave_max[0], wave_max[1]), fmaxf(wave_max[2], wave_max[3]));
            if (amax > __hip_atomic_load(out_absmax, __ATOMIC_RELAXED, __HIP_MEMORY_SCOPE_AGENT))
                atomicMax(reinterpret_cast<unsigned*>(out_absmax), __float_as_uint(amax));
        }
    }
}

__global__ __launch_bounds__(64) void mask_tile_flags_kernel(const float* __restrict__ mask, const int mode, const int halo,
                                                              const int H, const int W, const int TW, const int TH,
                                                              unsigned char* __restrict__ flags) {
    const int tm = blockIdx.x, lane = threadIdx.x;
    const int pxn = W / TW, ppi = (H / TH) * pxn;
    const int n = tm / ppi, prem = tm - n * ppi;
    const int y0 = (prem / pxn) * TH - halo, x0 = (prem % pxn) * TW - halo;
    const int ph = TH + 2 * halo, pw = TW + 2 * halo;
    bool any = false;
    for (int i = lane; i < ph * pw; i += 64) {
        const int yy = y0 + i / pw, xx = x0 + i % pw;
        if (yy >= 0 && yy < H && xx >= 0 && xx < W) {
            const float m = mask[((size_t)n * H + yy) * W + xx];
            any = any || (mode == 2 ? (1.f - m) != 0.f : m != 0.f);
        }
    }
    const bool r = __any(any);
    if (lane == 0) flags[tm] = r ? 1 : 0;
}

int conv_splitk_parts(const rpnet_conv_desc* d, int M, int Cin, int Cout) {
    if (d->split_planes != 2 || d->tune != 0 || d->taps != 9 || d->dilation > 1 || Cin < 128 || M % 256) return 1;
    if (d->stats_partial || d->bnb_partial || d->bnb_y || d->accumulate || d->out_scale_mode || d->Co1 || d->y1 || d->acc_scale_x1 ||
        d->groups > 1)
        return 1;
    const long tiles = (long)(M / 256) * (Cout / 64);
    const int kchunks = Cin >> 5;
    if (tiles > 128 || (tiles > 64 && kchunks < 32)) return 1;
    int parts = 1;
    while (parts < 8 && tiles * parts * 2 <= 256 && kchunks % (parts * 2) == 0 && kchunks / (parts * 2) >= 2) parts *= 2;
    return parts;
}

int conv_fwd_split_dma(const rpnet_conv_desc* d, int M, int Cin, int Cout, int tw, int wn, hipStream_t s, int parts, int bm) {
    const int tiles_m = M / bm, tiles_n = Cout / (64 * wn);
    const int ntiles = tiles_m * tiles_n;
    rpnet_conv_desc dp = *d;
    dp.tile_skip = nullptr;
    if (d->skip_mask && d->skip_ws && (d->skip_mode == 1 || d->skip_mode == 2) && !d->upsample && d->H % (bm / tw) == 0 && d->W % tw == 0) {
        hipLaunchKernelGGL(mask_tile_flags_kernel, dim3(tiles_m), dim3(64), 0, s, d->skip_mask, d->skip_mode, d->skip_halo ? 1 : 0, d->H,
                           d->W, tw, bm / tw, d->skip_ws);
        dp.tile_skip = d->skip_ws;
    }
    int kshift = 0;
    if (parts > 1) {
        if (d->split_planes != 2 || wn != 1 || (size_t)parts * M * Cout * sizeof(float) > d->splitk_ws_bytes || !d->splitk_ws) {
            set_error("conv_igemm_split_dma: split K needs two planes, 64-wide tiles and the workspace");
            return RPNET_ERR_WORKSPACE;
        }
        while ((1 << kshift) < parts) ++kshift;
        dp.y0 = (float*)d->splitk_ws;
        dp.bias = nullptr; dp.ep_scale = nullptr; dp.ep_shift = nullptr; dp.ep_relu = 0;
        dp.out_absmax = nullptr; dp.y_split = nullptr; dp.split_out_planes = 0; dp.y_split_scale = nullptr;
    }
#define RPNET_DMA(TWV, WNV, K64V) \
    hipLaunchKernelGGL((conv_igemm_split_dma_kernel<TWV, 2, WNV, K64V>), dim3(ntiles, parts), dim3(256), 0, s, dp, Cin, Cout, tiles_n, ntiles, kshift)
    if (d->split_planes == 1) {
        if (wn != 2 || Cin % 64 || d->C0 % 64) {
            set_error("conv_igemm_split_dma: one plane needs 128-wide tiles and channel counts in multiples of 64 per source");
            return RPNET_ERR_ARG;
        }
        if (tw == 32) RPNET_DMA(32, 2, true); else RPNET_DMA(16, 2, true);
    } else if (d->split_planes == 2 && bm == 128) {
        if (wn != 1 || parts != 1) {
            set_error("conv_igemm_split_dma: 128-pixel patches come in 64-wide tiles, unsplit");
            return RPNET_ERR_ARG;
        }
        if (tw == 32)
            hipLaunchKernelGGL((conv_igemm_split_dma_kernel<32, 2, 1, false, 2>), dim3(ntiles, 1), dim3(256), 0, s, dp, Cin, Cout, tiles_n, ntiles, 0);
        else
            hipLaunchKernelGGL((conv_igemm_split_dma_kernel<16, 2, 1, false, 2>), dim3(ntiles, 1), dim3(256), 0, s, dp, Cin, Cout, tiles_n, ntiles, 0);
    } else if (d->split_planes == 2) {
        if (wn == 2) { if (tw == 32) RPNET_DMA(32, 2, false); else RPNET_DMA(16, 2, false); }
        else { if (tw == 32) RPNET_DMA(32, 1, false); else RPNET_DMA(16, 1, false); }
    } else {
        set_error("conv_igemm_split_dma: fp16 planes only");
        return RPNET_ERR_ARG;
    }
#undef RPNET_DMA
    if (parts > 1) {
        const size_t MC = (size_t)M * Cout;
        hipLaunchKernelGGL(conv_splitk_reduce_kernel, dim3((unsigned)((MC / 8 + 255) / 256)), dim3(256), 0, s, (const float*)d->splitk_ws, parts, MC,
                           Cout, d->bias, d->ep_scale, d->ep_shift, d->ep_relu, d->y0, (unsigned short*)d->y_split, d->split_out_planes,
                           d->y_split_scale, d->out_absmax);
    }
    return check_launch("conv_igemm_split_dma");
}

}
```

rpnet_amd/csrc/conv_up4_dma.hip:

```cpp
#include <type_traits>

#include "conv_epilogue.h"
#include "lds_dma.h"
#include "split_bf16.h"

namespace rpnet {

template <int N, int I = 0, typename F>
__device__ __forceinline__ void static_for_u(F&& f) {
    if constexpr (I < N) {
        f(std::integral_constant<int, I>{});
        static_for_u<N, I + 1>(f);
    }
}

template <int N>
__device__ __forceinline__ void wait_vmcnt() {
    static_assert(N >= 0 && N < 64, "vmcnt is a 6-bit counter");
    asm volatile("s_waitcnt vmcnt(%0)" ::"n"(N) : "memory");
}

template <int TW>
struct PatchRowsUp {
    static constexpr bool kAlwaysValid = true;
// ... 76 lines not shown
            const int ph = uni(c0 / C0);
            cs = c0 - ph * C0;
            pix += (ph >> 1) * W + (ph & 1);
        }
        const int voff = hok[i] ? pix * (C0 * 2) + dkg16 : (int)0x80000000;
#pragma unroll
        for (int p = 0; p < NP; ++p) {
            auto* dst = (__attribute__((address_space(3))) void*)(smem + buf * HBUF + p * A_BYTES + hpos[i] * 1024);
            __builtin_amdgcn_raw_ptr_buffer_load_lds(rs0, dst, 16, voff, uni(cs * 2) + p * ps0, 0, 0);
        }
    };
    const int wvoff = (16 * WN * wv + drow) * 64 + dkg16;
    auto w_soff = [&](int idx, int c0) { return uni(((idx * (Kc >> 5) + (c0 >> 5)) * Ncols + n0) * 64); };
    auto dma_w = [&](int idx, int c0, int stage) {
        const int wsoff = w_soff(idx, c0);
#pragma unroll
        for (int p = 0; p < NP; ++p)
#pragma unroll
            for (int q = 0; q < WN; ++q) {
                auto* dst = (__attribute__((address_space(3))) void*)(smem + WOFF + stage * STAGE + p * B_BYTES + (16 * WN * wv + 16 * q) * 64);
                __builtin_amdgcn_raw_ptr_buffer_load_lds(rsw, dst, 16, wvoff + q * 1024, wsoff + p * psw, 0, 0);
            }
    };

    f32x16 acc[WM][WN];
#pragma unroll
    for (int i = 0; i < WM; ++i)
#pragma unroll
        for (int j = 0; j < WN; ++j)
#pragma unroll
            for (int r = 0; r < 16; ++r) acc[i][j][r] = 0.f;

    int hr00[WM];
#pragma unroll
    for (int i = 0; i < WM; ++i) {
        const int mloc = (wm * WM + i) * 32 + li;
        hr00[i] = (mloc / TW) * PW + (mloc % TW);
    }
    const int b_off = WOFF + (wn * WN * 32 + li) * 64 + 16 * (h ^ ((li >> 2) & 3));

    bf16x8 af[2][NP][WM], bfr[2][NP][WN];
    int aaddr[WM];
    auto a_addr = [&](const int ky, const int kx) {
        const int off = ky * PW + kx;
#pragma unroll
        for (int i = 0; i < WM; ++i) {
            const int hr = hr00[i] + off;
            aaddr[i] = hr * 64 + 16 * (h ^ ((hr >> 2) & 3));
        }
    };
    constexpr int NPROD = K64 ? 2 : nprod<NP>();
    constexpr int NR = NP * (WM + WN), NMMA = NPROD * WM * WN;
    static_assert(NR <= NMMA, "one fragment read of the next slice behind each MFMA of this one");
    auto read_frag = [&](auto sc, auto kc, const int abase, const int bbase) {
        constexpr int s = decltype(sc)::value, k = decltype(kc)::value;
        constexpr int grp = k / (WM + WN), r = k - grp * (WM + WN);
        constexpr int pa = K64 ? grp : NP - 1 - grp, pb = grp;
        if constexpr (r == 0 || r > WN) {
            constexpr int i = r == 0 ? 0 : r - WN;
            af[s][pa][i] = *reinterpret_cast<const bf16x8*>(smem + abase + (aaddr[i] ^ (32 * s)) + pa * A_BYTES);
        } else {
            constexpr int j = r - 1;
            bfr[s][pb][j] = *reinterpret_cast<const bf16x8*>(smem + bbase + (b_off ^ (32 * s)) + pb * B_BYTES + j * 2048);
        }
    };
    auto mma_one = [&](auto sc, auto mc) {
        constexpr int s = decltype(sc)::value, m = decltype(mc)::value;
        constexpr int q = m / (WM * WN), ij = m - q * (WM * WN), i = ij / WN, j = ij - i * WN;
        constexpr int pa = K64 ? q : prod_a<NP>(q), pb = K64 ? q : prod_b<NP>(q);
        acc[i][j] = mma16<NP>(af[s][pa][i], bfr[s][pb][j], acc[i][j]);
    };
    using I0 = std::integral_constant<int, 0>;
    using I1 = std::integral_constant<int, 1>;
    auto dma_w_one = [&](auto ec, const int wsoff, const int stage) {
        constexpr int e = decltype(ec)::value, p = e / WN, q = e - p * WN;
        auto* dst = (__attribute__((address_space(3))) void*)(smem + WOFF + stage * STAGE + p * B_BYTES + (16 * WN * wv + 16 * q) * 64);
        __builtin_amdgcn_raw_ptr_buffer_load_lds(rsw, dst, 16, wvoff + q * 1024, wsoff + p * psw, 0, 0);
    };

    {
        const int c0 = chunk_c0(0);
        static_for_u<HPW>([&](auto ic) { dma_halo(ic, c0, 0); });
        dma_w(0, c0, 0);
        dma_w(1, c0, 1);
        dma_w(2, c0, 2);
        wait_vmcnt<NW>();
        __builtin_amdgcn_s_barrier();
        a_addr(chunk_py(c0), chunk_px(c0));
    }
    static_for_u<NR>([&](auto kc) { read_frag(I0{}, kc, 0, 0); });

    auto step = [&](auto idxc, const int ci, const int ks) {
        constexpr int IDX = decltype(idxc)::value;
        const int hb = ci & 1;
        const bool last_chunk = ci + 1 >= kchunks;
        constexpr int I3 = (IDX + 3) & 3;
        const int c3 = chunk_c0((IDX + 3 < 4 || last_chunk) ? ci : ci + 1);
        const int wsoff = w_soff(I3, c3);
        const int wstage = (ks + 3) & 3;
        const int abase = hb * HBUF, bbase = (ks & 3) * STAGE;
        static_for_u<NMMA>([&](auto mc) {
            constexpr int m = decltype(mc)::value;
            mma_one(I0{}, mc);
            __builtin_amdgcn_sched_barrier(0);
            if constexpr (m < NR) {
                read_frag(I1{}, mc, abase, bbase);
                __builtin_amdgcn_sched_barrier(0);
            }
            if constexpr (m >= NMMA - 2 * NW && (NMMA - 1 - m) % 2 == 0) {
                dma_w_one(std::integral_constant<int, NW - 1 - (NMMA - 1 - m) / 2>{}, wsoff, wstage);
                __builtin_amdgcn_sched_barrier(0);
            }
        });
        constexpr int IN = (IDX + 1) & 3;
        const int cn = chunk_c0((IDX < 3 || last_chunk) ? ci : ci + 1);
        a_addr(chunk_py(cn) + (IN >> 1), chunk_px(cn) + (IN & 1));
        const int abase_n = (IDX < 3 ? hb : hb ^ 1) * HBUF, bbase_n = ((ks + 1) & 3) * STAGE;
        const int ch = chunk_c0(last_chunk ? ci : ci + 1);
        __builtin_amdgcn_sched_barrier(0);
        static_for_u<NMMA>([&](auto mc) {
            constexpr int m = decltype(mc)::value;
            mma_one(I1{}, mc);
            __builtin_amdgcn_sched_barrier(0);
            if constexpr (m < NR) {
                read_frag(I0{}, mc, abase_n, bbase_n);
                __builtin_amdgcn_sched_barrier(0);
            }
            if constexpr (IDX == 0 && m >= NMMA - 3 * NPOS0 && (NMMA - 1 - m) % 3 == 0) {
                dma_halo(std::integral_constant<int, NPOS0 - 1 - (NMMA - 1 - m) / 3>{}, ch, hb ^ 1);
                __builtin_amdgcn_sched_barrier(0);
            }
            if constexpr (IDX == 1 && NPOS1 > 0 && m >= NMMA - 3 * NPOS1 && (NMMA - 1 - m) % 3 == 0) {
                dma_halo(std::integral_constant<int, NPOS0 + NPOS1 - 1 - (NMMA - 1 - m) / 3>{}, ch, hb ^ 1);
                __builtin_amdgcn_sched_barrier(0);
            }
        });
        constexpr int N = IDX == 0 ? NW + NPOS0 * NP : (IDX == 1 ? NPOS0 * NP + NW + NPOS1 * NP : NW);
        wait_vmcnt<N>();
        __builtin_amdgcn_s_barrier();
    };

    int ks = 0;
    for (int ci = 0; ci < kchunks; ++ci) {
        step(std::integral_constant<int, 0>{}, ci, ks + 0);
        step(std::integral_constant<int, 1>{}, ci, ks + 1);
        step(std::integral_constant<int, 2>{}, ci, ks + 2);
        step(std::integral_constant<int, 3>{}, ci, ks + 3);
        ks += 4;
    }
    asm volatile("s_waitcnt vmcnt(0)" ::: "memory");
    __builtin_amdgcn_s_barrier();

    if constexpr (DG) {
        conv_epilogue<WM, WN, 2, PatchRows<TW>, false>(d, acc, PatchRows<TW>{(n * Hl + y0) * Wl + x0, Wl}, d.N * Hl * Wl, Ncols, Hl * Wl, n0, tm,
                                                        wm, wn, li, h, smem);
    } else {
        conv_epilogue<WM, WN, 2, PatchRowsUp<TW>, false>(d, acc, PatchRowsUp<TW>{(n * H + 2 * y0 + fpy) * W + 2 * x0 + fpx, 2 * W}, d.N * H * W,
                                                          Cout_out, H * W, n0 - fphase * Cout_out, tm * 4 + fphase, wm, wn, li, h, smem,
                                                          fphase * Cout_out);
    }
}

__global__ __launch_bounds__(256) void upconv_collapse_kernel(const float* __restrict__ w, float* __restrict__ wc, const int Cout, const int Cin) {
    const size_t i = (size_t)blockIdx.x * 256 + threadIdx.x;
    if (i >= (size_t)4 * Cout * Cin) return;
    const int ci = (int)(i % Cin);
    const int co = (int)((i / Cin) % Cout), ph = (int)(i / ((size_t)Cin * Cout));
    const int py = ph >> 1, px = ph & 1;
    float k[9];
#pragma unroll
    for (int q = 0; q < 9; ++q) k[q] = w[((size_t)co * Cin + ci) * 9 + q];
    float o[4];
#pragma unroll
    for (int r = 0; r < 2; ++r)
#pragma unroll
        for (int c = 0; c < 2; ++c) {
            const int ya = r == 0 ? 0 : (py ? 2 : 1), yb = r == 0 ? (py ? 1 : 0) : 2;
            const int xa = c == 0 ? 0 : (px ? 2 : 1), xb = c == 0 ? (px ? 1 : 0) : 2;
            float s = 0.f;
            for (int ky = ya; ky <= yb; ++ky)
                for (int kx = xa; kx <= xb; ++kx) s += k[ky * 3 + kx];
            o[r * 2 + c] = s;
        }
    *reinterpret_cast<f32x4*>(wc + i * 4) = f32x4{o[0], o[1], o[2], o[3]};
}

static int up4_tw(int Hl, int Wl) {
    if (Wl % 32 == 0 && Hl % 8 == 0) return 32;
    if (Wl % 16 == 0 && Hl % 16 == 0) return 16;
    return 0;
}

static int up4_plan(const rpnet_conv_desc* d, int mode, int* tw, int* Kc, int* Ncols) {
    if (!d || (d->split_planes != 2 && d->split_planes != 1) || d->H % 2 || d->W % 2 || d->C1 || d->Co1 || d->x1 || d->y1) return 0;
    const int Hl = d->H / 2, Wl = d->W / 2;
    const bool one = d->split_planes == 1;
    *tw = up4_tw(Hl, Wl);
    if (!*tw || d->C0 % (one ? 64 : 32) || d->Co0 % (one ? 128 : 64)) return 0;
    *Kc = mode == 1 ? d->C0 : 4 * d->C0;
    *Ncols = mode == 1 ? 4 * d->Co0 : d->Co0;
    const size_t lim = (size_t)1 << 31;
    const size_t src = (size_t)d->N * (mode == 1 ? Hl * Wl : d->H * d->W) * d->C0 * 2 * d->split_planes;
    if (src >= lim || (size_t)2 * 4 * *Kc * *Ncols * 2 >= lim || (size_t)d->N * d->H * d->W >= lim) return 0;
    const long tiles_m = (long)d->N * Hl * Wl / 256;
    if (mode == 1) return (d->Co0 % 128 == 0) ? 2 : 1;
    if (one) return 2;
    return (*Ncols % 128 == 0 && tiles_m * (*Ncols / 128) >= 192) ? 2 : 1;
}

}

extern "C" int rpnet_conv_up4_supported(const rpnet_conv_desc* d, int mode) {
    int tw, Kc, Nc;
    return (mode == 1 || mode == 2) && rpnet::up4_plan(d, mode, &tw, &Kc, &Nc) > 0;
}

extern "C" int rpnet_conv_up4_stats_blocks(const rpnet_conv_desc* d) {
    int tw, Kc, Nc;
    if (!rpnet::up4_plan(d, 1, &tw, &Kc, &Nc) || d->groups < 1 || d->N % d->groups) return 0;
    return (int)((long)(d->N / d->groups) * d->H * d->W / 256);
}

extern "C" int rpnet_upconv_collapse_weights(const float* w, float* wc, int Cout, int Cin, rpnet_stream_t stream) {
    using namespace rpnet;
    RPNET_REQUIRE(w && wc && Cout > 0 && Cin > 0, RPNET_ERR_ARG, "upconv_collapse_weights: bad argument");
    hipLaunchKernelGGL(upconv_collapse_kernel, dim3(cdiv((long)4 * Cout * Cin, 256)), dim3(256), 0, (hipStream_t)stream, w, wc, Cout, Cin);
    return check_launch("upconv_collapse_weights");
}

extern "C" int rpnet_conv_up4(const rpnet_conv_desc* d, int mode, rpnet_stream_t stream) {
    using namespace rpnet;
    RPNET_REQUIRE(d && d->x0 && d->w && d->y0 && (mode == 1 || mode == 2), RPNET_ERR_ARG, "conv_up4: null pointer / mode");
    int tw = 0, Kc = 0, Nc = 0;
    const int wn = up4_plan(d, mode, &tw, &Kc, &Nc);
    RPNET_REQUIRE(wn > 0, RPNET_ERR_SHAPE, "conv_up4: N=%d H=%d W=%d C0=%d Co0=%d planes=%d do not fit (rpnet_conv_up4_supported)", d->N, d->H, d->W,
                  d->C0, d->Co0, d->split_planes);
    RPNET_REQUIRE(d->acc_scale_col && d->acc_scale_x, RPNET_ERR_ARG, "conv_up4: fp16 planes need acc_scale_col and acc_scale_x");
    RPNET_REQUIRE(mode == 1 || !d->stats_partial, RPNET_ERR_ARG, "conv_up4: statistics belong to the forward launch");
    RPNET_REQUIRE(!d->stats_partial || rpnet_conv_up4_stats_blocks(d) > 0, RPNET_ERR_SHAPE, "conv_up4: statistic groups do not split into whole tiles");
    RPNET_REQUIRE(!d->out_scale_mode && !d->y_split && !d->bnb_y && !d->tile_skip && !d->splitk_ws && !d->y_enc, RPNET_ERR_ARG,
                  "conv_up4: plain epilogue only (bias, eval affine, statistics, accumulate, out_absmax)");
    const int tiles_m = d->N * (d->H / 2) * (d->W / 2) / 256, tiles_n = Nc / (64 * wn), ntiles = tiles_m * tiles_n;
    hipStream_t s = (hipStream_t)stream;
#define RPNET_UP4(TWV, WNV, DGV) hipLaunchKernelGGL((conv_up4_dma_kernel<TWV, WNV, DGV>), dim3(ntiles), dim3(256), 0, s, *d, Kc, Nc, tiles_n, ntiles)
#define RPNET_UP4K(TWV, DGV) hipLaunchKernelGGL((conv_up4_dma_kernel<TWV, 2, DGV, true>), dim3(ntiles), dim3(256), 0, s, *d, Kc, Nc, tiles_n, ntiles)
    if (d->split_planes == 1) {
        if (mode == 1) { if (tw == 32) RPNET_UP4K(32, false); else RPNET_UP4K(16, false); }
        else { if (tw == 32) RPNET_UP4K(32, true); else RPNET_UP4K(16, true); }
    } else if (mode == 1) {
        if (tw == 32) { if (wn == 2) RPNET_UP4(32, 2, false); else RPNET_UP4(32, 1, false); }
        else { if (wn == 2) RPNET_UP4(16, 2, false); else RPNET_UP4(16, 1, false); }
    } else {
        if (tw == 32) { if (wn == 2) RPNET_UP4(32, 2, true); else RPNET_UP4(32, 1, true); }
        else { if (wn == 2) RPNET_UP4(16, 2, true); else RPNET_UP4(16, 1, true); }
    }
#undef RPNET_UP4
#undef RPNET_UP4K
    return check_launch("conv_up4");
}
```

rpnet_amd/functional.py:

```python
import collections
import ctypes as C
import os

import torch
from torch.autograd import Function
from torch.autograd.function import once_differentiable

from . import hip
from .hip import ConvDesc, call, ptr, query

BN_EPS = 1e-5
BN_MOMENTUM = 0.1

_ASYNC = {"on": False, "side": {}, "pending": set(), "queued": False, "fifo": [], "keep": []}

_MODES = {"f32": (0, False, 0), "bf16x3": (3, False, 0), "f16x2": (3, True, 2), "f16": (3, True, 1)}
_CORR16 = True
_CORR_PRED_PLANES = True
_MATH = {}


def set_conv_math(mode):
    _MATH["mode"] = mode
    _MATH["planes"], _MATH["f16"], _MATH["f16_planes"] = _MODES[mode]
# ... 210 lines not shown
    probe.N, probe.H, probe.W, probe.C0, probe.Co0, probe.split_planes = N, H, W, pw.cin, cout, planes
    probe.x0, probe.y0 = ptr(xs0), ptr(xs0)
    return bool(query("rpnet_conv_up4_supported", C.byref(probe), 1))


def up4_layer_ok(weight, planes, calls):
    cout, cin = weight.shape[0], weight.shape[1]
    if not (_UP4 and planes in (1, 2) and cin % 32 == 0 and cout % 64 == 0):
        return False
    for N, H, W in calls:
        probe = ConvDesc()
        probe.N, probe.H, probe.W, probe.C0, probe.Co0, probe.split_planes = N, H, W, cin, cout, planes
        probe.x0 = probe.y0 = ptr(weight)
        if not query("rpnet_conv_up4_supported", C.byref(probe), 1):
            return False
    return True


_ABSMAX = {}
_ABSMAX_SLOTS = 256


def reset_absmax_pool(device):
    pool = _ABSMAX.get(device)
    if pool is None or pool[1] > 0:
        if pool is None:
            _ABSMAX[device] = [torch.zeros(_ABSMAX_SLOTS, device=device, dtype=torch.float32), 0]
        else:
            pool[0].zero_()
            pool[1] = 0


def _absmax_slot(device):
    pool = _ABSMAX.get(device)
    if pool is None or pool[1] >= _ABSMAX_SLOTS:
        pool = _ABSMAX[device] = [torch.zeros(_ABSMAX_SLOTS, device=device, dtype=torch.float32), 0]
        torch.cuda.current_stream(device).synchronize()
    pool[1] += 1
    return pool[0][pool[1] - 1:pool[1]]


PRED_SAFETY = float(os.environ.get("RPNET_EVAL_PRED_SAFETY", "4"))
_EVAL_PREDICT = True
_PRED = {}


def _pred_dev(device):
    pd = _PRED.get(device)
    if pd is None:
        pd = _PRED[device] = {"by_key": {}, "cur": None, "last_key": None, "calls": 0, "predicted_calls": 0, "violations": 0}
    return pd


def _pred_state(device, key):
    pd = _pred_dev(device)
    st = pd["by_key"].get(key)
    if st is None:
        st = pd["by_key"][key] = {"scale": torch.zeros(_ABSMAX_SLOTS, device=device), "bound": torch.zeros(_ABSMAX_SLOTS, device=device),
                                  "viol": torch.zeros(1, device=device, dtype=torch.int32), "n": 0, "active": False, "pending": False}
    return st


def pred_ready(device, key):
    pd = _PRED.get(device)
    st = pd["by_key"].get(key) if pd is not None else None
    return _EVAL_PREDICT and st is not None and st["n"] > 0


def pred_begin(device, key, allow=True):
    pd = _pred_dev(device)
    ready = pred_ready(device, key)
    st = _pred_state(device, key)
    st["active"] = bool(allow and ready)
    pd["cur"] = st
    pd["calls"] += 1
    pd["predicted_calls"] += int(st["active"])
    return st["active"]


def pred_scale(device):
    pd = _PRED.get(device)
    st = pd["cur"] if pd is not None else None
    pool = _ABSMAX.get(device)
    if st is None or not st["active"] or pool is None or pool[1] > st["n"]:
        return None
    return st["scale"][pool[1] - 1:pool[1]]


def pred_end(device, key):
    pd = _pred_dev(device)
    st = _pred_state(device, key)
    pd["cur"], pd["last_key"] = None, key
    pool = _ABSMAX.get(device)
    n = pool[1] if pool is not None else 0
    ran_predicted = st["active"]
    if ran_predicted and n != st["n"]:
        raise RuntimeError(f"rpnet_amd: an eval call of key {key} took {n} absmax slots, its predecessor {st['n']}")
    st["active"] = False
    if n == 0:
        st["n"] = 0
        return False
    if ran_predicted:
        st["viol"].zero_()
    call("rpnet_predict_scales", ptr(pool[0]), ptr(st["bound"]), ptr(st["scale"]), n, PRED_SAFETY, 1 if ran_predicted else 0,
         ptr(st["viol"]))
    st["n"] = n
    if not ran_predicted:
        return False
    if torch.cuda.is_current_stream_capturing():
        st["pending"] = True
        return False
    bad = int(st["viol"].item()) > 0
    pd["violations"] += int(bad)
    if bad:
        st["n"] = 0
    return bad


def pred_last_key(device):
    pd = _PRED.get(device)
    return pd["last_key"] if pd is not None else None


def pred_check_pending(device, key=None):
    pd = _PRED.get(device)
    if pd is None:
        return False
    st = pd["by_key"].get(key if key is not None else pd["last_key"])
    if st is None or not st["pending"]:
        return False
    bad = int(st["viol"].item()) > 0
    pd["violations"] += int(bad)
    return bad


def pred_stats(device=None):
    out = {"calls": 0, "predicted_calls": 0, "violations": 0}
    for dv, pd in _PRED.items():
        if device is None or dv == device:
            for k in out:
                out[k] += pd[k]
    return out


def _empty(shape, like, dtype=torch.float32):
    return torch.empty(shape, device=like.device, dtype=dtype)


def _ws(nbytes, like):
    return torch.empty((max(int(nbytes), 16) + 7) // 8, device=like.device, dtype=torch.float64)


class Operand:
    __slots__ = ("x", "p16", "pbf", "scale", "planes_only", "deferred", "masked")

    def __init__(self, x, p16=None, pbf=None, scale=None, planes_only=False, deferred=None, masked=None):
        self.x, self.p16, self.pbf, self.scale = x, p16, pbf, scale
        self.deferred = deferred
        self.masked = masked
        self.planes_only = planes_only

    def values(self):
        if self.planes_only:
            raise RuntimeError("rpnet_amd: this operand exists as fp16 planes only (its producer was told that its single "
                               "consumer is a 3x3 convolution on fp16 planes); a consumer asked for the fp32 values")
        return self.x

    @property
    def shape(self):
        return self.x.shape

    def derive(self, x):
        return Operand(x, scale=self.scale)


_WGRAD_DEFER = 1
_EVAL_SPLITK = True
_POOL_FUSE = True
_CONV1_BN_FUSE = True
_CONV1_RECOMP = True
_UP4 = True
_MASK_SKIP = os.environ.get("RPNET_MASK_SKIP", "1") == "1"


_SKIP_STATS = None


def _set_skip(d, mask, mode, halo, N, H, W, on=None):
    if (_MASK_SKIP if on is None else on) and mask is not None and mode in (1, 2):
        if _SKIP_STATS is not None:
            d._skip_ws = torch.full((max(N * H * W // 128, 16),), 255, device=mask.device, dtype=torch.uint8)
            _SKIP_STATS.append(d._skip_ws)
        else:
            d._skip_ws = torch.empty(max(N * H * W // 128, 16), device=mask.device, dtype=torch.uint8)
        d.skip_mask, d.skip_mode, d.skip_halo, d.skip_ws = ptr(mask), mode, halo, ptr(d._skip_ws)
        ARITH[("zero_tile_skip", "armed")] += 1


def as_operand(t):
    return t if (t is None or isinstance(t, Operand)) else Operand(t)


def split_bf16(x, planes, scale=None, mode=0):
    hip.require_gpu(x)
    x = x.contiguous()
    out = torch.empty((planes,) + tuple(x.shape), device=x.device, dtype=torch.bfloat16)
    c = x.shape[-1]
    call("rpnet_split_bf16", ptr(x), ptr(scale), mode if scale is not None else 0, ptr(out), x.numel() // c, c, planes)
    return out


def _split_operand(op, planes, scale=None, mode=0):
    if scale is not None and mode:
        pre = op.masked
        if pre is not None and pre[0] is scale and pre[1] == mode and pre[2].shape[0] == planes and pre[2].dtype == torch.bfloat16:
            return pre[2]
        return split_bf16(op.values(), planes, scale, mode)
    if op.pbf is not None and op.pbf.shape[0] == planes and op.pbf.shape[1:] == op.x.shape:
        return op.pbf
    op.pbf = split_bf16(op.values(), planes)
    return op.pbf


_CONV1X1_SPLIT = True


def _use_split(pw, x0, x1):
    if not (_MATH["planes"] and pw is not None and x0.shape[-1] % 32 == 0 and (x1 is None or x1.shape[-1] % 32 == 0)):
        return False
    if pw.taps == 9:
        return (pw.cin_pad == pw.cin and pw.cin % 32 == 0) or (pw.cin_pad != pw.cin and pw.cin_pad % 64 == 0)
    return _CONV1X1_SPLIT and pw.taps == 1 and pw.cin_pad % 64 == 0 and pw.cout % 64 == 0 and x0.shape[-1] % 64 == 0


def split_f16(x, s_a, s_b=None, mask=None, mode=0, want_scale=True, planes=None, a_is_bound=False):
    hip.require_gpu(x)
    x = x.contiguous()
    planes = planes or _MATH["f16_planes"] or 2
    out = torch.empty((planes,) + tuple(x.shape), device=x.device, dtype=torch.float16)
    s = torch.empty(1, device=x.device, dtype=torch.float32) if want_scale else None
    c = x.shape[-1]
    call("rpnet_split_f16", ptr(x), ptr(mask), mode if mask is not None else 0, ptr(s_a), ptr(s_b), ptr(s), ptr(out),
         x.numel() // c, c, planes, 1 if a_is_bound else 0)
    return out, s


def _f16_sources(op0, op1, in_scale, in_mode, two_scales=False):
    s0 = op0.scale
    s1 = op1.scale if op1 is not None else None
    if s0 is None or (op1 is not None and s1 is None):
        return None
    masked = in_scale is not None and in_mode
    fp = _MATH["f16_planes"]

    def ready(op):
        return op.p16 is not None and op.p16.shape[1:] == op.x.shape and op.p16.shape[0] == fp

    if op1 is None and not masked and ready(op0):
        return op0.p16, None, s0, None
    pre = op0.masked
    if (op1 is None and masked and pre is not None and pre[0] is in_scale and pre[1] == in_mode and pre[2].shape[0] == fp
            and pre[2].dtype == torch.float16):
        return pre[2], None, s0, None
    if two_scales and op1 is not None and not masked and ready(op0) and ready(op1):
        return op0.p16, op1.p16, s0, s1
    xs0, s = split_f16(op0.values(), s0, s1, in_scale if masked else None, in_mode if masked else 0)
    xs1 = split_f16(op1.values(), s0, s1, want_scale=False)[0] if op1 is not None else None
    if op1 is None and not masked:
        op0.p16 = xs0
    return xs0, xs1, s, None


class PackedWeight:

    def __init__(self, weight, split=None, pool=None):
        cout, cin, kh, kw = weight.shape
        self._pool = pool
        self.taps = kh * kw
        if split is None:
            self.off0, self.split, self.off1, self.cin_pad = 0, cin, cin, cin
        else:
            n0, n0_pad = split[:2]
            self.off0, self.split, self.off1 = 0, n0, n0_pad
            self.cin_pad = split[2] if len(split) > 2 else n0_pad + (cin - n0)
        self.cout, self.cin = cout, cin
        self.has_wd = cin >= 32
        self._weight = weight
        self._wp = self._wd = self.wps = self.wds = None

    def _pack_f32(self):
        w, n = self._weight, self.taps * self.cin_pad * self.cout
        mk = torch.zeros if self.cin_pad != self.cin else torch.empty
        self._wp = mk(n, device=w.device, dtype=torch.float32)
        self._wd = mk(n, device=w.device, dtype=torch.float32) if self.has_wd else None
        call("rpnet_pack_conv_weight", ptr(w), ptr(self._wp), ptr(self._wd), self.cout, self.cin, self.taps, self.off0,
             self.split, self.off1, self.cin_pad)

    @property
    def wp(self):
        if self._wp is None:
            self._pack_f32()
        return self._wp

    @property
    def wd(self):
        if self._wp is None:
            self._pack_f32()
        return self._wd

    def split_packs(self, planes):
        pk = self.wps.get(planes) if self.wps else None
        if pk is None:
            w = self._weight
            pk = self.alloc_split(planes)
            call("rpnet_pack_conv_weight_split", ptr(w), ptr(pk[0]), ptr(pk[1]), self.cout, self.cin, self.taps,
                 self.off0, self.split, self.off1, self.cin_pad, planes, ptr(pk[2]) if planes <= 2 else None,
                 ptr(pk[3]) if planes <= 2 else None)
        return pk

    def up4_packs(self, planes):
        up = getattr(self, "_up4", None)
        if up is None:
            up = self._up4 = {}
        pk = up.get(planes)
        if pk is None:
            w = self._weight
            wc = torch.empty((4 * self.cout, self.cin, 2, 2), device=w.device, dtype=torch.float32)
            call("rpnet_upconv_collapse_weights", ptr(w), ptr(wc), self.cout, self.cin)
            n = 4 * self.cin * 4 * self.cout
            wp4 = torch.empty((planes, n), device=w.device, dtype=torch.float16)
            wd4 = torch.empty((planes, n), device=w.device, dtype=torch.float16)
            t4 = torch.empty(4 * self.cout, device=w.device, dtype=torch.float32)
# ... 168 lines not shown
                    d.split_planes = fp
                    d.acc_scale_col, d.acc_scale_x, d.acc_scale_x1 = ptr(t_row), ptr(f16[2]), ptr(f16[3])
                    d._keep = f16
                    if pw.taps == 9 and x1 is None and not upsample:
                        _set_skip(d, in_scale, in_mode, 1, N, H, W)
                else:
                    np_ = _MATH["planes"]
                    d = _desc(_split_operand(op0, np_, in_scale, in_mode), None if x1 is None else _split_operand(op1, np_),
                              pw.split_packs(np_)[0], bias, None, 0, z, None, N, H, W, pw.taps, upsample, 1, scale, shift, 1)
                    d.split_planes = np_
                if up4e:
                    d.out_absmax = ptr(mx)
                else:
                    d.y_split, d.split_out_planes, d.out_absmax = ptr(zs), np_out, ptr(mx)
                if sp is not None and out_split in (True, "corr") and not up4e:
                    fpo = _MATH["f16_planes"]
                    z16 = torch.empty((fpo, N, H, W, cout), device=x0.device, dtype=torch.float16)
                    d.y_split, d.split_out_planes, d.y_split_scale = ptr(z16), fpo, ptr(sp)
                if up4e:
                    _cup4(d, 1)
                else:
                    if _EVAL_SPLITK and d.split_planes == 2 and pw.taps == 9 and N * H * W * cout <= 128 * 256 * 64:
                        nb = query("rpnet_conv_splitk_workspace_bytes", C.byref(d))
                        if nb:
                            d._ws = _ws(nb, x0)
                            d.splitk_ws, d.splitk_ws_bytes = ptr(d._ws), nb
                    _cconv("rpnet_conv_fwd", d)
            else:
                d = _desc(x0, x1, pw.wp, bias, in_scale, in_mode, z, None, N, H, W, pw.taps, upsample, 1, scale, shift, 1)
                d.y_split, d.split_out_planes, d.out_absmax = ptr(zs), np_out, ptr(mx)
                _cconv("rpnet_conv_fwd", d)
            if zs is not None:
                produced["pbf"] = zs
            if want16 and sp is not None:
                if z16 is not None:
                    produced["p16"], produced["scale"] = z16, sp
                elif out_split in (True, "corr"):
                    produced["p16"], produced["scale"] = split_f16(z, sp, want_scale=False)[0], sp
                else:
                    produced["scale"] = sp
            elif want16:
                if out_split in (True, "corr"):
                    produced["p16"], produced["scale"] = split_f16(z, mx, a_is_bound=True)
                else:
                    sz = torch.empty(1, device=x0.device, dtype=torch.float32)
                    call("rpnet_pow2_scale", ptr(mx), ptr(sz))
                    produced["scale"] = sz
            ctx.eval_mode = True
            return z
        if bn_eval:
            groups = 1
        recomp = bool(not bn_eval and first and _CONV1_RECOMP and f16_mode() and cout % 8 == 0 and 256 % (cout // 8) == 0 and out_split is True
                      and produced.get("z_unused") and not produced.get("pool_req") and _CONV1_BN_FUSE
                      and query("rpnet_conv1_stats_blocks", N, H, W, cout, groups) > 0)
        y = None if recomp else _empty((N, H, W, cout), x0)
        stats = _empty((4, groups, cout), x0)
        fused, xs, sx, sx1 = 0, None, None, None
        if first:
            fused = 0 if bn_eval else query("rpnet_conv1_stats_blocks", N, H, W, cout, groups)
            part = torch.empty(groups * fused * cout * 2, device=x0.device, dtype=torch.float64) if fused else None
            call("rpnet_conv1_fwd", ptr(x0), ptr(weight), ptr(bias), ptr(y), None, None, N, H, W, cout, None, ptr(part), groups)
        else:
            f16 = _f16_sources(op0, op1, in_scale, in_mode, pw.taps == 1) if (f16_mode() and _use_split(pw, x0, x1)) else None
            if op0.planes_only and not (f16 is not None and op1 is None and in_scale is None and pw.cin % 64 == 0 and cout % 64 == 0):
                raise RuntimeError("rpnet_amd: a planes-only operand (conv_bn_relu_op(z_unused=True)) reached a convolution "
                                   "that cannot run forward AND weight gradient from its fp16 planes")
            if op1 is not None and op1.planes_only and not (f16 is not None and f16[1] is op1.p16 and pw.cin_pad % 64 == 0
                                                            and cout % 64 == 0 and x0.shape[-1] % 64 == 0):
                raise RuntimeError("rpnet_amd: a planes-only second source reached a convolution that does not read its "
                                   "fp16 planes as they are (forward and weight gradient)")
            up4 = False
            if f16 is not None:
                xs, sx, sx1 = (f16[0], f16[1]), f16[2], f16[3]
                fp = _MATH["f16_planes"]
                up4 = _up4_ok(pw, fp, upsample, x1, in_scale, xs[0], N, H, W, cout)
                wps, t_row = (pw.up4_packs(fp)[0], pw.up4_packs(fp)[2]) if up4 else (pw.split_packs(fp)[0], pw.split_packs(fp)[2])
                d = _desc(xs[0], xs[1], wps, bias, None, 0, y, None, N, H, W, pw.taps, upsample, groups)
                d.split_planes = fp
                d.acc_scale_col, d.acc_scale_x, d.acc_scale_x1 = ptr(t_row), ptr(sx), ptr(sx1)
                if pw.taps == 9 and x1 is None and not upsample:
                    _set_skip(d, in_scale, in_mode, 1, N, H, W)
            elif _use_split(pw, x0, x1):
                np_ = _MATH["planes"]
                xs = (_split_operand(op0, np_, in_scale, in_mode), None if x1 is None else _split_operand(op1, np_))
                d = _desc(xs[0], xs[1], pw.split_packs(np_)[0], bias, None, 0, y, None, N, H, W, pw.taps, upsample, groups)
                d.split_planes = np_
            else:
                d = _desc(x0, x1, pw.wp, bias, in_scale, in_mode, y, None, N, H, W, pw.taps, upsample, groups)
            fused = 0 if bn_eval else query("rpnet_conv_up4_stats_blocks" if up4 else "rpnet_conv_stats_blocks", C.byref(d))
            if fused:
                part = torch.empty(groups * fused * cout * 2, device=x0.device, dtype=torch.float64)
                d.stats_partial = ptr(part)
            if up4:
                _cup4(d, 1)
            else:
                _cconv("rpnet_conv_fwd", d)
        if bn_eval:
            return ConvBnRelu._eval_grad_tail(ctx, x0, x1, in_scale, weight, bias, gamma, beta, running_mean, running_var, y,
                                              z, pw, upsample, in_mode, first, out_split, produced, xs, sx, sx1,
                                              (not first) and up4)
        _order_wait(gamma.data_ptr())
        if fused:
            call("rpnet_bn_stats_from_partial", ptr(part), fused, N, H * W, cout, groups, ptr(gamma), ptr(beta),
                 ptr(running_mean), ptr(running_var), ptr(nbt), BN_MOMENTUM, BN_EPS, ptr(stats[0]), ptr(stats[1]),
                 ptr(stats[2]), ptr(stats[3]))
        else:
            wsb = query("rpnet_bn_workspace_bytes", cout, groups)
            ws = _ws(wsb, x0)
            call("rpnet_bn_stats", ptr(y), N, H * W, cout, groups, ptr(gamma), ptr(beta), ptr(running_mean),
                 ptr(running_var), ptr(nbt), BN_MOMENTUM, BN_EPS, ptr(stats[0]), ptr(stats[1]), ptr(stats[2]), ptr(stats[3]),
                 ptr(ws), wsb)
        _order_done(gamma.data_ptr())
        want16 = f16_mode() and cout % 32 == 0 and out_split in ((True, "scale", "corr") if _CORR16 else (True, "scale"))
        np_out = 0
        if out_split in (True, "corr") and cout % 32 == 0 and _MATH["planes"]:
            np_out = _MATH["f16_planes"] if want16 else _MATH["planes"]
        pool = bool(produced.get("pool")) and np_out > 0 and out_split is True and xs is not None and not first and \
            H % 2 == 0 and W % 2 == 0 and pw.cin_pad % 64 == 0 and cout % 64 == 0 and x0.shape[-1] % 64 == 0
        produced["pooled"] = pool
        Hz, Wz = (H // 2, W // 2) if pool else (H, W)
        if pool:
            z = _empty((N, Hz, Wz, cout), x0)
        zs = torch.empty((np_out, N, Hz, Wz, cout), device=x0.device, dtype=torch.float16 if np_out <= 2 else torch.bfloat16) if np_out else None
        sz = torch.empty(1, device=x0.device, dtype=torch.float32) if want16 else None
        if produced.get("z_unused") and want16 and np_out and out_split in (True, "corr") and (pool or not produced.get("pool_req")):
            z = torch.empty(1, device=x0.device, dtype=torch.float32).expand(N, Hz, Wz, cout)
            produced["planes_only"] = True
        defer = (bool(produced.get("defer_act")) and not pool and not np_out and not want16 and not recomp
                 and groups == 1 and not produced.get("planes_only"))
        if defer:
            produced["deferred"] = (y, stats[0], stats[1])
        elif recomp:
            if not (produced.get("planes_only") and want16 and np_out):
                raise RuntimeError("rpnet_amd: the first layer was run without its pre-BatchNorm tensor but its output is not planes-only")
            call("rpnet_conv1_bn_relu", ptr(x0), ptr(weight), ptr(bias), ptr(stats[0]), ptr(stats[1]), None, ptr(zs), np_out,
                 ptr(gamma), ptr(beta), ptr(sz), N, H, W, cout, groups)
            ARITH[("bn_relu", "first layer made again from the image")] += 1
        else:
            call("rpnet_bn_relu", ptr(y), ptr(stats[0]), ptr(stats[1]), None if produced.get("planes_only") else ptr(z), ptr(zs),
                 np_out, ptr(gamma), ptr(beta),
                 ptr(sz) if want16 else None, N, H * W, cout, groups, W if pool else 0, None, 0)
        if pool:
            ARITH[("bn_relu", "with the 2x2 max-pool")] += 1
        if want16 and np_out:
            produced["p16"] = zs
        elif zs is not None:
            produced["pbf"] = zs
        if want16:
            produced["scale"] = sz
        _tap("fwd:y,stats", weight, y, stats)
        ctx.save_for_backward(x0, x1, in_scale, weight, gamma, y, stats)
        ctx.yshape = (N, H, W, cout)
        ctx.pw, ctx.cfg, ctx.eval_mode, ctx.pool = pw, (groups, upsample, in_mode, first), False, pool
        ctx.up4 = (not first) and up4
        ctx.bias, ctx.beta, ctx.xs, ctx.sx, ctx.sx1 = bias, beta, xs, sx, sx1
        ctx.opts = (_ASYNC["on"], _MASK_SKIP)
        return z

    @staticmethod
    def _eval_grad_tail(ctx, x0, x1, in_scale, weight, bias, gamma, beta, running_mean, running_var, y, z, pw, upsample, in_mode,
                        first, out_split, produced, xs, sx, sx1, up4):
        N, H, W, cout = y.shape
        stats = _empty((4, 1, cout), y)
        call("rpnet_bn_eval_affine", ptr(gamma), ptr(beta), ptr(running_mean), ptr(running_var), BN_EPS, ptr(stats[0]),
             ptr(stats[1]), cout)
        stats[2, 0].copy_(running_mean)
        torch.rsqrt(running_var + BN_EPS, out=stats[3, 0])
        mx = torch.zeros(1, device=y.device, dtype=torch.float32)
        call("rpnet_bn_eval_relu", ptr(y), ptr(stats[0]), ptr(stats[1]), ptr(z), ptr(mx), N * H * W, cout)
        ARITH[("bn_relu", "eval mode, with a gradient")] += 1
        if f16_mode() and cout % 32 == 0 and bool(out_split) and (_CORR16 or out_split != "corr"):
            if out_split in (True, "corr"):
                produced["p16"], produced["scale"] = split_f16(z, mx, a_is_bound=True)
            else:
                sz = torch.empty(1, device=y.device, dtype=torch.float32)
                call("rpnet_pow2_scale", ptr(mx), ptr(sz))
                produced["scale"] = sz
        ctx.save_for_backward(x0, x1, in_scale, weight, gamma, y, stats)
        ctx.yshape = (N, H, W, cout)
        ctx.pw, ctx.cfg, ctx.eval_mode, ctx.pool, ctx.bn_eval = pw, (1, upsample, in_mode, first), False, False, True
        ctx.up4 = up4
        ctx.bias, ctx.beta, ctx.xs, ctx.sx, ctx.sx1 = bias, beta, xs, sx, sx1
        ctx.opts = (_ASYNC["on"], _MASK_SKIP)
        return z

    @staticmethod
    @once_differentiable
    def backward(ctx, dz):
        if ctx.eval_mode:
            raise RuntimeError("rpnet_amd: an eval-mode layer made without a gradient-capable forward reached backward "
                               "(conv_bn_relu_op decides from torch.is_grad_enabled() and requires_grad at call time)")
        x0, x1, in_scale, weight, gamma, y, stats = ctx.saved_tensors
        async_on, skip_on = getattr(ctx, "opts", (None, None))
        pw = ctx.pw
        groups, upsample, in_mode, first = ctx.cfg
        dz = dz.contiguous()
        _tap("bwd_in:y,stats,dz", weight, y, stats, dz)
        N, H, W, cout = ctx.yshape
        wsb = query("rpnet_bn_workspace_bytes", cout, groups)
        ws = _ws(wsb, dz)
        beta, bias = ctx.beta, ctx.bias
        if y is None:
            direct = _direct(gamma, async_on) and _direct(beta, async_on)
            dgamma, dbeta = (None, None) if direct else (_empty((cout,), dz), _empty((cout,), dz))
            rows = query("rpnet_conv1_bn_bwd_rows", N, H, W, cout, groups)
            part = torch.empty(groups * rows * cout * 2, device=dz.device, dtype=torch.float64)
            call("rpnet_conv1_bn_bwd_partial", ptr(x0), ptr(weight), ptr(bias), ptr(dz), ptr(stats), ptr(part), N, H, W, cout, groups)
            ARITH[("bn_bwd", "first layer made again from the image")] += 1
            if direct:
                _order_wait(gamma.data_ptr())
            call("rpnet_bn_bwd", ptr(dz), None, ptr(gamma), ptr(stats[0]), ptr(stats[1]), ptr(stats[2]), ptr(stats[3]), None, None, 0,
                 None, ptr(gamma.grad if direct else dgamma), ptr(beta.grad if direct else dbeta), N, H * W, cout, groups,
                 1 if direct else 0, ptr(part), None, rows, 0, ptr(ws), wsb, None, 0)
            if direct:
                _order_done(gamma.data_ptr())
            dw = torch.empty_like(weight)
            wb = query("rpnet_conv1_wgrad_workspace_bytes", N, H, W, cout)
            ws2 = _ws(wb, dz)
            coef = ws.data_ptr() + query("rpnet_bn_bwd_coef_offset", cout, groups)
            call("rpnet_conv1_wgrad_bn", ptr(x0), ptr(dz), None, ptr(stats), coef, ptr(dw), N, H, W, cout, groups, ptr(ws2), wb,
                 ptr(weight), ptr(bias))
            dw = _accumulate_direct(weight, dw, async_on)
            dx0 = None
            if ctx.needs_input_grad[0]:
                dx0 = _empty(x0.shape, dz)
                call("rpnet_conv1_dgrad_bn", ptr(dz), None, ptr(stats), coef, ptr(weight), ptr(bias), ptr(x0), ptr(dx0), N, H, W, cout,
                     groups)
            db = None if _direct(bias, async_on) else torch.zeros_like(gamma)
            return dx0, None, None, dw, db, dgamma, dbeta, None, None, None, None, None, None, None, None, None, None, None
        np_ = ctx.xs[0].shape[0] if ctx.xs is not None else 0
        need_d = not first and (ctx.needs_input_grad[0] or (x1 is not None and ctx.needs_input_grad[1]))
        wsplit = bool(np_) and pw.cin_pad % 64 == 0 and cout % 64 == 0 and x0.shape[-1] % 64 == 0
        dsplit = bool(np_) and cout % 32 == 0 and need_d
        dys = torch.empty((np_,) + tuple(y.shape), device=y.device, dtype=torch.bfloat16) if (wsplit or dsplit) else None
        sdy = torch.empty(1, device=y.device, dtype=torch.float32) if (dys is not None and np_ <= 2) else None
        dy = _empty(ctx.yshape, dz) if (first or not wsplit or (need_d and not dsplit)) else None
        fuse1 = first and _CONV1_BN_FUSE and stats.is_contiguous()
        if fuse1:
            dy = None
        if ctx.pool and (dys is None or dz.shape[1] * 2 != H):
            raise RuntimeError("rpnet_amd: the pooled BatchNorm backward needs dy as split planes and the pooled gradient")
        bn_eval = getattr(ctx, "bn_eval", False)
        direct = _direct(gamma, async_on) and _direct(beta, async_on) and not bn_eval
        dgamma, dbeta = (None, None) if direct else (_empty((cout,), y), _empty((cout,), y))
        ARITH[("bn_bwd", "eval mode" if bn_eval else "own reduction pass")] += 1
        if direct:
            _order_wait(gamma.data_ptr())
        if bn_eval:
            call("rpnet_bn_eval_bwd", ptr(dz), ptr(y), ptr(stats[0]), ptr(stats[1]), ptr(stats[2]), ptr(stats[3]), ptr(dy),
                 ptr(dys), np_ if dys is not None else 0, ptr(sdy), ptr(dgamma), ptr(dbeta), N, H * W, cout, groups, 0,
                 ptr(ws), wsb)
        else:
            call("rpnet_bn_bwd", ptr(dz), ptr(y), ptr(gamma), ptr(stats[0]), ptr(stats[1]), ptr(stats[2]), ptr(stats[3]),
                 ptr(dy), ptr(dys), np_ if dys is not None else 0, ptr(sdy), ptr(gamma.grad if direct else dgamma),
                 ptr(beta.grad if direct else dbeta), N, H * W, cout, groups, 1 if direct else 0, None, None, 0,
                 W if ctx.pool else 0, ptr(ws), wsb, None, 0)
        if direct:
            _order_done(gamma.data_ptr())
        _tap("bn_bwd:dz,dy,dys,sdy,ws", weight, dz, dy, dys, sdy, ws)
        dw = torch.empty_like(weight)
        dx0 = dx1 = dscale = None
        if first:
            wb = query("rpnet_conv1_wgrad_workspace_bytes", N, H, W, cout)
            ws2 = _ws(wb, y)
            coef = ws.data_ptr() + query("rpnet_bn_bwd_coef_offset", cout, groups)
            if fuse1:
                call("rpnet_conv1_wgrad_bn", ptr(x0), ptr(dz), ptr(y), ptr(stats), coef, ptr(dw), N, H, W, cout, groups,
                     ptr(ws2), wb, None, None)
            else:
                call("rpnet_conv1_wgrad", ptr(x0), ptr(dy), ptr(dw), N, H, W, cout, ptr(ws2), wb)
            dw = _accumulate_direct(weight, dw, async_on)
            if ctx.needs_input_grad[0]:
                dx0 = _empty(x0.shape, dz)
                call("rpnet_conv1_dgrad_bn", ptr(dz), ptr(y), ptr(stats), coef, ptr(weight), None, None, ptr(dx0), N, H, W, cout,
                     groups)
        else:
            if wsplit:
                dyp = dys
                d = _desc(ctx.xs[0], ctx.xs[1], None, None, None, 0, None, None, N, H, W, pw.taps, upsample,
                          co_split=(cout, 0), wgrad=True)
                d.split_planes = np_
                if np_ <= 2:
                    d.acc_scale_x, d.acc_scale_dy, d.acc_scale_x1 = ptr(ctx.sx), ptr(sdy), ptr(ctx.sx1)
            else:
                dyp = dy
                d = _desc(x0, x1, None, None, in_scale, in_mode, dy, None, N, H, W, pw.taps, upsample, wgrad=True)
            wb = query("rpnet_conv_wgrad_workspace_bytes", N, H, W, pw.cin_pad, cout, pw.taps)
            wup4 = bool(getattr(ctx, "up4", False)) and wsplit and np_ in (1, 2) and bool(query("rpnet_conv_wgrad_up4_supported", C.byref(d)))
            if wup4:
                wb = query("rpnet_conv_wgrad_up4_workspace_bytes", N, H, W, pw.cin, cout)

            def wgrad(dy_ptr, dw_ptr, ws_t):
                if wup4:
                    if dy_ptr is not None:
                        ARITH[("wgrad3x3_up4", _PLANE_NAME[d.split_planes])] += 1
                    call("rpnet_conv_wgrad_up4", C.byref(d), dy_ptr, dw_ptr, ptr(ws_t), wb)
                else:
                    _cconv("rpnet_conv_wgrad", d, dy_ptr, dw_ptr, pw.cin, pw.off0, pw.split, pw.off1, ptr(ws_t), wb)
            deferred = None
            if _direct(weight, async_on):
                prod = torch.cuda.current_stream(y.device)

                def launch_async():
                    dev = y.device
                    side, main = _side_stream(dev), prod
                    side.wait_stream(main)
                    d.accumulate = 1
                    with torch.cuda.stream(side):
                        ws2 = _ws(wb, y)
                        if wsplit:
                            wgrad(ptr(dyp), None, ws2)
                            red = _reduce_stream(dev)
                            red.wait_stream(side)
                            _ASYNC["keep"].append(ws2)
                            with torch.cuda.stream(red):
                                wgrad(None, ptr(weight.grad), ws2)
                        else:
                            wgrad(ptr(dyp), ptr(weight.grad), ws2)
                    _ASYNC["keep"].append((x0, x1, in_scale, dy, dyp, ctx.sx, ctx.sx1, sdy, ctx.xs))
                    if not _ASYNC["queued"]:
                        torch.autograd.Variable._execution_engine.queue_callback(join_side_streams)
                        _ASYNC["queued"] = True
                    _ASYNC["pending"].add(dev)
                if _WGRAD_DEFER:
                    _defer_wgrad(launch_async)
                    deferred = True
                else:
                    launch_async()
                dw = None
            else:
                ws2 = _ws(wb, y)
                wgrad(ptr(dyp), ptr(dw), ws2)
            need0 = ctx.needs_input_grad[0]
            need1 = x1 is not None and ctx.needs_input_grad[1]
            if need0 or need1:
                c0, c1 = x0.shape[-1], (x1.shape[-1] if x1 is not None else 0)
                need_s = in_scale is not None and ctx.needs_input_grad[2]
                up4 = bool(getattr(ctx, "up4", False)) and dsplit and np_ in (1, 2)
                if up4:
                    pk4 = pw.up4_packs(np_)
                    g0, g1 = _empty(x0.shape, y), None
                    dd = _desc(dys, None, pk4[1], None, None, 0, g0, None, N, H, W, pw.taps, 1)
                    dd.split_planes = np_
                    dd.acc_scale_col, dd.acc_scale_x = ptr(pk4[3]), ptr(sdy)
                    up4 = bool(query("rpnet_conv_up4_supported", C.byref(dd), 2))
                if not up4:
                    g0 = _empty((N, H, W, c0), y)
                    g1 = _empty((N, H, W, c1), y) if x1 is not None else None
                if up4:
                    pass
                elif dsplit:
                    pk = pw.split_packs(np_)
                    dd = _desc(dys, None, pk[1], None, None, 0, g0, g1, N, H, W,
                               pw.taps, 0, out_scale=None if need_s else in_scale, out_mode=in_mode)
                    dd.split_planes = np_
                    if np_ <= 2:
                        dd.acc_scale_col, dd.acc_scale_x = ptr(pk[3]), ptr(sdy)
                        if pw.taps == 9 and x1 is None and not upsample and not need_s:
                            _set_skip(dd, in_scale, in_mode, 0, N, H, W, skip_on)
                else:
                    dd = _desc(dy, None, pw.wd, None, None, 0, g0, g1, N, H, W, pw.taps, 0,
                               out_scale=None if need_s else in_scale, out_mode=in_mode)
                if up4:
                    _cup4(dd, 2)
                else:
                    _cconv("rpnet_conv_fwd", dd)
                _tap("dgrad:g0,g1", weight, g0, g1)
                if deferred:
                    _release_wgrads(_WGRAD_DEFER - 1)
                    deferred = None
                if need_s:
                    gx, dscale = torch.empty_like(g0), torch.empty_like(in_scale)
                    call("rpnet_rowdot_scale", ptr(g0), ptr(x0), ptr(in_scale), ptr(gx), ptr(dscale), N * H * W, c0,
                         in_mode, 0)
                    g0 = gx
                if upsample and not up4:
                    h0 = _empty(x0.shape, y)
                    call("rpnet_upsample2_bwd", ptr(g0), ptr(h0), N, H, W, c0)
                    g0 = h0
                dx0 = g0 if need0 else None
                dx1 = g1 if need1 else None
            if deferred:
                _release_wgrads(_WGRAD_DEFER - 1)
        if bn_eval:
            db = _accumulate_direct(bias, stats[0, 0] * dbeta, async_on)
        else:
            db = None if _direct(bias, async_on) else torch.zeros_like(gamma)
        return dx0, dx1, dscale, dw, db, dgamma, dbeta, None, None, None, None, None, None, None, None, None, None, None


def conv_bn_relu_op(x0, conv, bn, cache, training, x1=None, in_scale=None, in_mode=0, groups=1, upsample=False, split=None,
                    out_split=True, z_unused=False, pool=False, defer_act=False):
    op0, op1 = as_operand(x0), as_operand(x1)
    pw = cache.get(conv.weight, split) if (conv.weight.shape[1] >= 32 or split is not None) else None
    produced = {"z_unused": bool(z_unused) and training and conv.weight.shape[0] % 64 == 0,
                "pool": bool(pool) and training and _POOL_FUSE, "pool_req": bool(pool),
                "defer_act": bool(defer_act) and training and not out_split}
    if not training and torch.is_grad_enabled() and any(
            t is not None and t.requires_grad for t in (op0.x, None if op1 is None else op1.x, in_scale, conv.weight, conv.bias,
                                                        bn.weight, bn.bias)):
        produced["eval_grad"] = True
    z = ConvBnRelu.apply(op0.x, None if op1 is None else op1.x, in_scale, conv.weight, conv.bias, bn.weight, bn.bias,
                         bn.running_mean, bn.running_var, bn.num_batches_tracked if training else None, pw, training, groups,
                         1 if upsample else 0, in_mode, out_split, (op0, op1), produced)
    out = Operand(z, produced.get("p16"), produced.get("pbf"), produced.get("scale"), bool(produced.get("planes_only")),
                  produced.get("deferred"))
    if pool and not produced.get("pooled"):
        out = maxpool2(out)
    return out


def conv_bn_relu(x0, conv, bn, cache, training, **kw):
    return conv_bn_relu_op(x0, conv, bn, cache, training, **kw).x


class ConvRelu(Function):

    @staticmethod
    def forward(ctx, x, weight, bias, pw, relu, dilation):
        hip.require_gpu(x, weight)
        N, H, W, _ = x.shape
        cout = weight.shape[0]
        z = _empty((N, H, W, cout), x)
        xs = None
        if _use_split(pw, x, None):
            np_ = _MATH["planes"]
            xs = split_bf16(x, np_)
            d = _desc(xs, None, pw.split_packs(np_)[0], bias, None, 0, z, None, N, H, W, pw.taps, 0, ep_relu=1 if relu else 0)
            d.split_planes = np_
        else:
            d = _desc(x, None, pw.wp, bias, None, 0, z, None, N, H, W, pw.taps, 0, ep_relu=1 if relu else 0)
        d.dilation = dilation
        _cconv("rpnet_conv_fwd", d)
        ctx.save_for_backward(x, weight, z)
        ctx.pw, ctx.cfg, ctx.xs = pw, (relu, dilation), xs
        return z

    @staticmethod
    @once_differentiable
    def backward(ctx, dz):
        x, weight, z = ctx.saved_tensors
        pw, xs = ctx.pw, ctx.xs
        relu, dilation = ctx.cfg
        N, H, W, cout = z.shape
        dy, db = torch.empty_like(z), _empty((cout,), z)
        wb = query("rpnet_bias_relu_bwd_workspace_bytes", cout)
        ws = _ws(wb, z)
        call("rpnet_bias_relu_bwd", ptr(dz.contiguous()), ptr(z) if relu else None, ptr(dy), ptr(db), N * H * W, cout,
             ptr(ws), wb)
        dw = torch.empty_like(weight)
        dys = split_bf16(dy, xs.shape[0]) if xs is not None and cout % 32 == 0 else None
        if dys is not None and dilation <= 1 and pw.cin % 64 == 0 and cout % 64 == 0:
            d = _desc(xs, None, None, None, None, 0, dy, None, N, H, W, pw.taps, 0, wgrad=True)
            d.split_planes, dyp = xs.shape[0], dys
        else:
            d = _desc(x, None, None, None, None, 0, dy, None, N, H, W, pw.taps, 0, wgrad=True)
            dyp = dy
        d.Co0, d.dilation = cout, dilation
        wb2 = query("rpnet_conv_wgrad_workspace_bytes", N, H, W, pw.cin_pad, cout, pw.taps)
        ws2 = _ws(wb2, z)
        _cconv("rpnet_conv_wgrad", d, ptr(dyp), ptr(dw), pw.cin, pw.off0, pw.split, pw.off1, ptr(ws2), wb2)
        dx = None
        if ctx.needs_input_grad[0] and pw.has_wd:
            dx = _empty(x.shape, z)
            if dys is not None:
                dd = _desc(dys, None, pw.split_packs(xs.shape[0])[1], None, None, 0, dx, None, N, H, W, pw.taps, 0)
                dd.split_planes = xs.shape[0]
            else:
                dd = _desc(dy, None, pw.wd, None, None, 0, dx, None, N, H, W, pw.taps, 0)
            dd.dilation = dilation
            _cconv("rpnet_conv_fwd", dd)
        return dx, dw, db, None, None, None


class MaxPool3(Function):

    @staticmethod
    def forward(ctx, z, stride):
        N, H, W, Cc = z.shape
        out = _empty((N, (H - 1) // stride + 1, (W - 1) // stride + 1, Cc), z)
        call("rpnet_maxpool3_fwd", ptr(z), ptr(out), N, H, W, Cc, stride)
        ctx.save_for_backward(z)
        ctx.stride = stride
        return out

    @staticmethod
    @once_differentiable
    def backward(ctx, dpool):
        (z,) = ctx.saved_tensors
        N, H, W, Cc = z.shape
        dz = torch.empty_like(z)
        call("rpnet_maxpool3_bwd", ptr(z), ptr(dpool.contiguous()), ptr(dz), N, H, W, Cc, ctx.stride)
        return dz, None


def sum_n(tensors):
    out = torch.empty_like(tensors[0])
    for i in range(0, len(tensors), 15):
        chunk = ([out] if i else []) + [t.contiguous() for t in tensors[i:i + 15]]
        arr = (C.c_void_p * len(chunk))(*[t.data_ptr() for t in chunk])
        call("rpnet_sum_n", arr, len(chunk), ptr(out), out.numel())
    return out


class FanOut(Function):

    @staticmethod
    def forward(ctx, x, n):
        ctx.shape = x.shape
        return tuple(x.view_as(x) for _ in range(n))

    @staticmethod
    @once_differentiable
    def backward(ctx, *grads):
        live = [g for g in grads if g is not None]
        if not live:
            return None, None
        return (live[0] if len(live) == 1 else sum_n(live)), None


class SplitRows(Function):

    @staticmethod
    def forward(ctx, x, n0):
        ctx.n = (n0, x.shape[0] - n0)
        ctx.meta = (tuple(x.shape[1:]), x.device, x.dtype)
        return x[:n0], x[n0:]

    @staticmethod
    @once_differentiable
    def backward(ctx, g0, g1):
        tail, dev, dt = ctx.meta
        parts = [g if g is not None else torch.zeros((n,) + tail, device=dev, dtype=dt) for g, n in zip((g0, g1), ctx.n)]
        return torch.cat(parts, 0), None


class SplitFan(Function):

    @staticmethod
    def forward(ctx, x, n0, k0, k1):
        ctx.cfg = (n0, k0, k1)
        ctx.meta = (tuple(x.shape), x.device, x.dtype)
        a, b = x[:n0], x[n0:]
        return tuple(a.view_as(a) for _ in range(k0)) + tuple(b.view_as(b) for _ in range(k1))

    @staticmethod
    @once_differentiable
    def backward(ctx, *grads):
        n0, k0, k1 = ctx.cfg
        shape, dev, dt = ctx.meta
        out = torch.empty(shape, device=dev, dtype=dt)
        for dst, gs in ((out[:n0], grads[:k0]), (out[n0:], grads[k0:])):
            live = [g.contiguous() for g in gs if g is not None]
            if not live:
                dst.zero_()
                continue
            for i in range(0, len(live), 15):
                chunk = ([dst] if i else []) + live[i:i + 15]
                if len(chunk) == 1:
# ... 437 lines not shown
```

rpnet_amd/hip.py:

```python
import ctypes as C
import os

import torch

_LIB_PATH = os.environ.get("RPNET_LIB_PATH") or os.path.join(os.path.dirname(os.path.abspath(__file__)), "librpnet_hip.so")
_lib = None

vp, ci, cf, cs, cd = C.c_void_p, C.c_int, C.c_float, C.c_size_t, C.c_double


class ConvDesc(C.Structure):
    _fields_ = [("x0", vp), ("x1", vp), ("C0", ci), ("C1", ci), ("w", vp), ("bias", vp), ("in_scale", vp),
                ("in_scale_mode", ci), ("y0", vp), ("y1", vp), ("Co0", ci), ("Co1", ci), ("ep_scale", vp),
                ("ep_shift", vp), ("ep_relu", ci), ("out_scale", vp), ("out_scale_mode", ci), ("accumulate", ci),
                ("N", ci), ("H", ci), ("W", ci), ("taps", ci), ("upsample", ci), ("groups", ci), ("dilation", ci), ("stats_partial", vp), ("split_planes", ci), ("y_split", vp), ("split_out_planes", ci),
                ("acc_scale_col", vp), ("acc_scale_x", vp), ("acc_scale_dy", vp), ("bnb_y", vp), ("bnb_stats", vp), ("bnb_partial", vp), ("bnb_pmax", vp), ("bnb_groups", ci),
                ("acc_scale_x1", vp), ("out_absmax", vp), ("tune", ci), ("y_split_scale", vp), ("splitk_ws", vp), ("splitk_ws_bytes", cs),
                ("skip_mask", vp), ("skip_mode", ci), ("skip_halo", ci), ("skip_ws", vp), ("tile_skip", vp),
                ("y_enc", vp), ("y_enc_stride", ci)]


PACK_MAX = 24


class PackItem(C.Structure):
    _fields_ = [("w", vp), ("wp", vp), ("wd", vp), ("row_scale_wp", vp), ("row_scale_wd", vp), ("cout", ci), ("cin", ci),
                ("taps", ci), ("cin_off0", ci), ("cin_split", ci), ("cin_off1", ci), ("cin_pad", ci)]


_SIGS = {
    "rpnet_version": (ci, []),
    "rpnet_last_error_string": (C.c_char_p, []),
    "rpnet_pack_conv_weight": (ci, [vp, vp, vp, ci, ci, ci, ci, ci, ci, ci, vp]),
    "rpnet_split_bf16": (ci, [vp, vp, ci, vp, cs, ci, ci, vp]),
    "rpnet_split_f16": (ci, [vp, vp, ci, vp, vp, vp, vp, cs, ci, ci, ci, vp]),
    "rpnet_pack_conv_weight_split": (ci, [vp, vp, vp, ci, ci, ci, ci, ci, ci, ci, ci, vp, vp, vp]),
    "rpnet_pack_conv_weights_split": (ci, [C.POINTER(PackItem), ci, ci, vp]),
    "rpnet_conv_fwd": (ci, [C.POINTER(ConvDesc), vp]),
    "rpnet_upconv_collapse_weights": (ci, [vp, vp, ci, ci, vp]),
    "rpnet_conv_up4_supported": (ci, [C.POINTER(ConvDesc), ci]),
    "rpnet_conv_up4_stats_blocks": (ci, [C.POINTER(ConvDesc)]),
    "rpnet_conv_up4": (ci, [C.POINTER(ConvDesc), ci, vp]),
    "rpnet_conv_wgrad_up4_supported": (ci, [C.POINTER(ConvDesc)]),
    "rpnet_conv_wgrad_up4_workspace_bytes": (cs, [ci, ci, ci, ci, ci]),
    "rpnet_conv_wgrad_up4": (ci, [C.POINTER(ConvDesc), vp, vp, vp, cs, vp]),
    "rpnet_conv_stats_blocks": (ci, [C.POINTER(ConvDesc)]),
    "rpnet_conv_tile_variant": (ci, [C.POINTER(ConvDesc)]),
    "rpnet_conv_splitk_workspace_bytes": (cs, [C.POINTER(ConvDesc)]),
    "rpnet_bn_stats_from_partial": (ci, [vp, ci, ci, ci, ci, ci, vp, vp, vp, vp, vp, cf, cf, vp, vp, vp, vp, vp]),
    "rpnet_conv_wgrad_workspace_bytes": (cs, [ci, ci, ci, ci, ci, ci]),
    "rpnet_conv_wgrad": (ci, [C.POINTER(ConvDesc), vp, vp, ci, ci, ci, ci, vp, cs, vp]),
    "rpnet_conv1_fwd": (ci, [vp, vp, vp, vp, vp, vp, ci, ci, ci, ci, vp, vp, ci, vp]),
    "rpnet_conv1_stats_blocks": (ci, [ci, ci, ci, ci, ci]),
    "rpnet_pow2_scale": (ci, [vp, vp, vp]),
    "rpnet_predict_scales": (ci, [vp, vp, vp, ci, cf, ci, vp, vp]),
    "rpnet_conv1_wgrad_workspace_bytes": (cs, [ci, ci, ci, ci]),
    "rpnet_conv1_wgrad": (ci, [vp, vp, vp, ci, ci, ci, ci, vp, cs, vp]),
    "rpnet_conv1_wgrad_bn": (ci, [vp, vp, vp, vp, vp, vp, ci, ci, ci, ci, ci, vp, cs, vp, vp, vp]),
    "rpnet_conv1_bn_relu": (ci, [vp, vp, vp, vp, vp, vp, vp, ci, vp, vp, vp, ci, ci, ci, ci, ci, vp]),
    "rpnet_conv1_bn_bwd_rows": (ci, [ci, ci, ci, ci, ci]),
    "rpnet_conv1_bn_bwd_partial": (ci, [vp, vp, vp, vp, vp, vp, ci, ci, ci, ci, ci, vp]),
    "rpnet_conv1_dgrad_bn": (ci, [vp, vp, vp, vp, vp, vp, vp, vp, ci, ci, ci, ci, ci, vp]),
    "rpnet_bn_bwd_coef_offset": (cs, [ci, ci]),
    "rpnet_bn_workspace_bytes": (cs, [ci, ci]),
    "rpnet_bn_stats": (ci, [vp, ci, ci, ci, ci, vp, vp, vp, vp, vp, cf, cf, vp, vp, vp, vp, vp, cs, vp]),
    "rpnet_bn_eval_affine": (ci, [vp, vp, vp, vp, cf, vp, vp, ci, vp]),
    "rpnet_bn_relu": (ci, [vp, vp, vp, vp, vp, ci, vp, vp, vp, ci, ci, ci, ci, ci, vp, ci, vp]),
    "rpnet_bn_act_scale": (ci, [vp, vp, vp, ci, ci, ci, ci, vp]),
    "rpnet_bn_bwd": (ci, [vp, vp, vp, vp, vp, vp, vp, vp, vp, ci, vp, vp, vp, ci, ci, ci, ci, ci, vp, vp, ci, ci, vp, cs, vp, ci, vp]),
    "rpnet_bn_eval_relu": (ci, [vp, vp, vp, vp, vp, cs, ci, vp]),
    "rpnet_bn_eval_bwd": (ci, [vp, vp, vp, vp, vp, vp, vp, vp, ci, vp, vp, vp, ci, ci, ci, ci, ci, vp, cs, vp]),
    "rpnet_bias_relu_bwd_workspace_bytes": (cs, [ci]),
    "rpnet_bias_relu_bwd": (ci, [vp, vp, vp, vp, cs, ci, vp, cs, vp]),
    "rpnet_maxpool3_fwd": (ci, [vp, vp, ci, ci, ci, ci, ci, vp]),
    "rpnet_maxpool3_bwd": (ci, [vp, vp, vp, ci, ci, ci, ci, ci, vp]),
    "rpnet_maxpool2_fwd": (ci, [vp, vp, ci, ci, ci, ci, vp]),
    "rpnet_maxpool2_bwd": (ci, [vp, vp, vp, vp, ci, ci, ci, ci, vp]),
    "rpnet_upsample2_bwd": (ci, [vp, vp, ci, ci, ci, ci, vp]),
    "rpnet_mask_avgpool": (ci, [vp, vp, ci, ci, ci, ci, vp]),
    "rpnet_local_corr_fwd": (ci, [vp, vp, vp, ci, ci, ci, ci, ci, ci, vp]),
    "rpnet_local_corr_bwd_workspace_bytes": (cs, [ci, ci, ci, ci]),
    "rpnet_local_corr_bwd": (ci, [vp, vp, vp, vp, vp, ci, ci, ci, ci, ci, ci, vp, vp, cs, vp]),
    "rpnet_local_corr_split_fwd": (ci, [vp, vp, vp, ci, ci, ci, ci, ci, ci, ci, vp, vp, vp, vp, vp, vp]),
    "rpnet_local_corr_split_bwd": (ci, [vp, vp, vp, vp, vp, ci, ci, ci, ci, ci, ci, ci, vp, vp, vp, vp, cs, vp]),
    "rpnet_affine_register": (ci, [vp, vp, vp, vp, vp, vp, ci, ci, ci, ci, cd, cd, cd, cd, vp]),
    "rpnet_sum_n": (ci, [vp, ci, vp, cs, vp]),
    "rpnet_demons_workspace_bytes": (cs, [ci, ci, ci]),
    "rpnet_demons_register": (ci, [vp, vp, vp, ci, vp, vp, vp, ci, ci, ci, ci, cd, cd, cd, cd, vp, cs, vp]),
    "rpnet_displacement_warp": (ci, [vp, vp, vp, ci, ci, ci, cf, cf, cf, vp]),
    "rpnet_affine_warp": (ci, [vp, vp, vp, vp, vp, ci, ci, ci, cf, cf, cf, vp]),
    "rpnet_identity_grid_warp": (ci, [vp, vp, ci, ci, ci, cf, cf, cf, vp]),
    "rpnet_mask_adjoint": (ci, [vp, vp, vp, ci, ci, ci, ci, ci, ci, vp]),
    "rpnet_masked_pool_workspace_bytes": (cs, [ci, ci, ci, ci]),
    "rpnet_masked_pool_fwd": (ci, [vp, vp, vp, vp, ci, ci, ci, ci, vp, cs, vp]),
    "rpnet_masked_pool_bwd": (ci, [vp, vp, vp, vp, ci, ci, ci, ci, ci, vp]),
    "rpnet_cosine_match_fwd": (ci, [vp, vp, vp, ci, ci, ci, ci, cf, vp]),
    "rpnet_cosine_match_bwd_workspace_bytes": (cs, [ci, ci, ci, ci]),
    "rpnet_cosine_match_bwd": (ci, [vp, vp, vp, vp, vp, ci, ci, ci, ci, cf, ci, vp, cs, vp]),
    "rpnet_bilinear_up_fwd": (ci, [vp, vp, ci, ci, ci, ci, ci, vp]),
    "rpnet_bilinear_up_bwd": (ci, [vp, vp, ci, ci, ci, ci, ci, vp]),
    "rpnet_softmax_thresh_pool": (ci, [vp, vp, ci, ci, ci, ci, ci, ci, vp]),
    "rpnet_refine_glue_supported": (ci, [ci, ci, ci, ci, ci, ci]),
    "rpnet_refine_glue_fwd": (ci, [vp, vp, vp, vp, cf, vp, vp, vp, vp, ci, vp, vp, vp, vp, ci, ci, ci, ci, ci, ci, ci, vp]),
    "rpnet_refine_glue_bwd_workspace_bytes": (cs, [ci, ci, ci, ci, ci]),
    "rpnet_refine_glue_bwd": (ci, [vp, vp, vp, cf, vp, vp, ci, ci, ci, ci, ci, vp, cs, vp]),
    "rpnet_rowdot_scale": (ci, [vp, vp, vp, vp, vp, cs, ci, ci, ci, vp]),
    "rpnet_softmax_pool_bwd": (ci, [vp, vp, vp, ci, ci, ci, ci, ci, vp]),
    "rpnet_loss_workspace_bytes": (cs, [ci, ci, ci, ci]),
    "rpnet_dice_ce_fwd": (ci, [vp, vp, vp, vp, ci, ci, ci, ci, ci, ci, ci, vp, vp, cs, vp]),
    "rpnet_dice_ce_bwd": (ci, [vp, vp, vp, vp, vp, ci, ci, ci, ci, ci, ci, ci, vp, ci, vp]),
    "rpnet_dice_ce_multi_fwd": (ci, [C.POINTER(vp), ci, vp, vp, vp, ci, ci, ci, ci, vp, cs, vp]),
    "rpnet_dice_ce_multi_bwd": (ci, [C.POINTER(vp), C.POINTER(vp), ci, vp, vp, vp, ci, ci, ci, ci, vp]),
    "rpnet_objective_fwd": (ci, [C.POINTER(vp), C.POINTER(cf), ci, vp, vp, cf, vp, vp, ci, ci, ci, ci, vp, cs, vp]),
    "rpnet_objective_bwd": (ci, [C.POINTER(vp), C.POINTER(vp), C.POINTER(cf), ci, vp, vp, vp, vp, cf, ci, ci, ci, ci, vp]),
    "rpnet_argmax_masks": (ci, [vp, vp, vp, vp, ci, ci, ci, vp]),
    "rpnet_align_labels": (ci, [vp, vp, vp, cs, vp]),
    "rpnet_debug_lds_canary": (ci, [ci, ci, C.c_longlong, vp, vp]),
    "rpnet_debug_fastdiv_selftest": (C.c_longlong, [ci]),
    "rpnet_debug_mfma_spin": (ci, [ci, ci, C.c_longlong, vp, vp]),
}
ABI_SYMBOLS = tuple(_SIGS)
ABI_VERSION = 109


def lib_path():
    return _LIB_PATH


def load():
    global _lib
    if _lib is None:
        if not os.path.exists(_LIB_PATH):
            raise RuntimeError(f"{_LIB_PATH} not found: build it with `make -C rpnet_amd/csrc` "
                               "(or __graft_entry__.build()); rpnet_amd has no CPU fallback")
        lib = C.CDLL(_LIB_PATH)
        lib.rpnet_version.restype = ci
        if lib.rpnet_version() != ABI_VERSION:
            raise RuntimeError(f"{_LIB_PATH} has ABI version {lib.rpnet_version()}, this binding was written for {ABI_VERSION} "
                               "(include/rpnet_abi.h RPNET_ABI_VERSION): rebuild it with `make -C rpnet_amd/csrc`")
        for name, (res, args) in _SIGS.items():
            fn = getattr(lib, name)
            fn.restype, fn.argtypes = res, args
        _lib = lib
    return _lib


def ptr(t):
    return None if t is None else t.data_ptr()


try:
    _raw_stream, _cur_device = torch._C._cuda_getCurrentRawStream, torch._C._cuda_getDevice
except AttributeError:
    _raw_stream = None


def stream():
    if _raw_stream is not None:
        return _raw_stream(_cur_device())
    return torch.cuda.current_stream().cuda_stream


def call(name, *args):
    lib = load()
    rc = getattr(lib, name)(*args, stream())
    if rc != 0:
        raise RuntimeError(f"{name} failed (rc={rc}): {lib.rpnet_last_error_string().decode()}")


def query(name, *args):
    return getattr(load(), name)(*args)


def require_gpu(*tensors):
    for t in tensors:
        if t is not None and not t.is_cuda:
            raise RuntimeError("rpnet_amd runs on MI355X only: got a CPU tensor (there is no CPU fallback; "
                               "the CPU restatement lives in oracle/ and is test infrastructure)")
```

Measured before the change: 508.8.

## Fuse BatchNorm-backward channel sums into the preceding conv dgrad epilogue

During the dgrad convolution that produces dz for an upstream BatchNorm, the epilogue now also reads the saved pre-BN output and statistics, applies the ReLU mask, and accumulates per-tile, per-channel sums of dz and dz*xhat plus a max. These partials go to a workspace that rpnet_bn_bwd consumes instead of running its own reduction pass over dz and y. This removes one full read of two activation tensors per eligible BN layer, at the cost of extra loads, double-precision accumulation and LDS reductions in the conv epilogue, plus more register pressure and Python-side linking logic between layers.

```diff
diff --git a/include/rpnet_abi.h b/include/rpnet_abi.h
--- a/include/rpnet_abi.h
+++ b/include/rpnet_abi.h
@@ -17,7 +17,7 @@
     RPNET_ERR_WORKSPACE = -3
 };
 
-#define RPNET_ABI_VERSION 109
+#define RPNET_ABI_VERSION 110
 int rpnet_version(void);
 const char* rpnet_last_error_string(void);
 
@@ -81,6 +81,7 @@
 
 int rpnet_conv_fwd(const rpnet_conv_desc* d, rpnet_stream_t stream);
 int rpnet_conv_stats_blocks(const rpnet_conv_desc* d);
+int rpnet_conv_bn_bwd_rows(const rpnet_conv_desc* d);
 int rpnet_conv_tile_variant(const rpnet_conv_desc* d);
 size_t rpnet_conv_splitk_workspace_bytes(const rpnet_conv_desc* d);
 
diff --git a/rpnet_amd/csrc/conv_epilogue.h b/rpnet_amd/csrc/conv_epilogue.h
--- a/rpnet_amd/csrc/conv_epilogue.h
+++ b/rpnet_amd/csrc/conv_epilogue.h
@@ -23,10 +23,17 @@
 }
 constexpr int cmax(int a, int b) { return a > b ? a : b; }
 
-template <int WM, int WN, typename RowMap, bool AFF, bool ROWOPS>
+struct BnbAcc {
+    double s1[4], s2[4];
+    float mx[4];
+    f32x4 sc, sh, mu, is;
+};
+
+template <int WM, int WN, typename RowMap, bool AFF, bool ROWOPS, bool BNB = false>
 __device__ __forceinline__ float conv_epilogue_store(const rpnet_conv_desc& d, f32x16 (&acc)[WM][WN], const RowMap rows, const int M,
                                                      const int Cout, const int per_group, const int n0, const int wm,
-                                                     const int wn, const int li, const int h, float* slab, const int cso = 0) {
+                                                     const int wn, const int li, const int h, float* slab, const int cso = 0,
+                                                     BnbAcc* ba = nullptr) {
     constexpr int SW = WN * 32 + 4;
     const int lane = li + 32 * h;
     const int colbase = n0 + wn * WN * 32;
@@ -126,6 +133,21 @@
                     *reinterpret_cast<f32x4*>(&slab[rr * SW + c4 * 4]) = v4[q];
                 }
             }
+        }
+        if constexpr (BNB) {
+            const float* yl = d.bnb_y + colbase + (lane % (WN * 8)) * 4;
+#pragma unroll
+            for (int q = 0; q < NQ; ++q)
+                if (RowMap::kAlwaysValid || orow[q] >= 0) {
+                    const f32x4 yb = *reinterpret_cast<const f32x4*>(yl + (size_t)orow[q] * Cout);
+#pragma unroll
+                    for (int k = 0; k < 4; ++k) {
+                        const float dm = (yb[k] * ba->sc[k] + ba->sh[k] > 0.f) ? v4[q][k] : 0.f;
+                        ba->s1[k] += dm;
+                        ba->s2[k] += (double)dm * ((yb[k] - ba->mu[k]) * ba->is[k]);
+                        ba->mx[k] = fmaxf(ba->mx[k], fabsf(dm));
+                    }
+                }
         }
 #pragma unroll
         for (int q = 0; q < NQ; ++q) {
@@ -172,7 +194,7 @@
     return amax;
 }
 
-template <int WM, int WN, int WGM = 2, typename RowMap = LinearRows, bool WIDE = false>
+template <int WM, int WN, int WGM = 2, typename RowMap = LinearRows, bool WIDE = false, bool BNB = true>
 __device__ __forceinline__ void conv_epilogue(const rpnet_conv_desc& d, f32x16 (&acc)[WM][WN], const RowMap rows,
                                               const int M, const int Cout, const int HW, const int n0, const int tm,
                                               const int wm, const int wn, const int li, const int h, void* lds, const int cso = 0) {
@@ -223,7 +245,58 @@
     const bool aff = d.ep_scale != nullptr || d.ep_relu != 0;
     const bool rowops = d.out_scale_mode != 0 || d.accumulate != 0 || d.out_absmax != nullptr || d.y_split != nullptr;
     float amax = 0.f;
-    if (!aff && !rowops) conv_epilogue_store<WM, WN, RowMap, false, false>(d, acc, rows, M, Cout, per_group, n0, wm, wn, li, h, slab, cso);
+    if (BNB && d.bnb_partial) {
+        static_assert(64 % (WN * 8) == 0, "a lane keeps the same 4 channels in every row it visits");
+        constexpr int BNC = 64 * WN;
+        const int lane = li + 32 * h;
+        const int col = n0 + wn * WN * 32 + (lane % (WN * 8)) * 4;
+        const int r0 = rows(wm * WM * 32);
+        const int pgb = (d.N / d.bnb_groups) * HW;
+        const int gb = (r0 >= 0 ? r0 : 0) / pgb, G = d.bnb_groups;
+        BnbAcc ba;
+        ba.sc = *reinterpret_cast<const f32x4*>(d.bnb_stats + (size_t)(0 * G + gb) * Cout + col);
+        ba.sh = *reinterpret_cast<const f32x4*>(d.bnb_stats + (size_t)(1 * G + gb) * Cout + col);
+        ba.mu = *reinterpret_cast<const f32x4*>(d.bnb_stats + (size_t)(2 * G + gb) * Cout + col);
+        ba.is = *reinterpret_cast<const f32x4*>(d.bnb_stats + (size_t)(3 * G + gb) * Cout + col);
+#pragma unroll
+        for (int k = 0; k < 4; ++k) { ba.s1[k] = 0.0; ba.s2[k] = 0.0; ba.mx[k] = 0.f; }
+        if (!rowops) conv_epilogue_store<WM, WN, RowMap, false, false, true>(d, acc, rows, M, Cout, per_group, n0, wm, wn, li, h, slab, cso, &ba);
+        else amax = conv_epilogue_store<WM, WN, RowMap, false, true, true>(d, acc, rows, M, Cout, per_group, n0, wm, wn, li, h, slab, cso, &ba);
+#pragma unroll
+        for (int o = WN * 8; o < 64; o <<= 1)
+#pragma unroll
+            for (int k = 0; k < 4; ++k) {
+                ba.s1[k] += __shfl_xor(ba.s1[k], o, 64);
+                ba.s2[k] += __shfl_xor(ba.s2[k], o, 64);
+                ba.mx[k] = fmaxf(ba.mx[k], __shfl_xor(ba.mx[k], o, 64));
+            }
+        double* red = reinterpret_cast<double*>(lds);
+        float* redm = reinterpret_cast<float*>(red + WGM * BNC * 2);
+        __syncthreads();
+        if (lane < WN * 8) {
+            const int cl = wn * WN * 32 + lane * 4;
+#pragma unroll
+            for (int k = 0; k < 4; ++k) {
+                red[((size_t)wm * BNC + cl + k) * 2] = ba.s1[k];
+                red[((size_t)wm * BNC + cl + k) * 2 + 1] = ba.s2[k];
+                redm[wm * BNC + cl + k] = ba.mx[k];
+            }
+        }
+        __syncthreads();
+        for (int e = threadIdx.x; e < BNC * 2; e += WGM * 128) {
+            double sacc = 0.0;
+#pragma unroll
+            for (int r = 0; r < WGM; ++r) sacc += red[(size_t)r * BNC * 2 + e];
+            d.bnb_partial[((size_t)tm * Cout + n0) * 2 + e] = sacc;
+        }
+        if (d.bnb_pmax)
+            for (int e = threadIdx.x; e < BNC; e += WGM * 128) {
+                float m = 0.f;
+#pragma unroll
+                for (int r = 0; r < WGM; ++r) m = fmaxf(m, redm[r * BNC + e]);
+                d.bnb_pmax[(size_t)tm * Cout + n0 + e] = m;
+            }
+    } else if (!aff && !rowops) conv_epilogue_store<WM, WN, RowMap, false, false>(d, acc, rows, M, Cout, per_group, n0, wm, wn, li, h, slab, cso);
     else if (!aff) amax = conv_epilogue_store<WM, WN, RowMap, false, true>(d, acc, rows, M, Cout, per_group, n0, wm, wn, li, h, slab, cso);
     else if (!rowops) conv_epilogue_store<WM, WN, RowMap, true, false>(d, acc, rows, M, Cout, per_group, n0, wm, wn, li, h, slab, cso);
     else amax = conv_epilogue_store<WM, WN, RowMap, true, true>(d, acc, rows, M, Cout, per_group, n0, wm, wn, li, h, slab, cso);
diff --git a/rpnet_amd/csrc/conv_igemm.hip b/rpnet_amd/csrc/conv_igemm.hip
--- a/rpnet_amd/csrc/conv_igemm.hip
+++ b/rpnet_amd/csrc/conv_igemm.hip
@@ -2,7 +2,7 @@
 
 namespace rpnet {
 
-template <int WM, int WN, bool INSCALE>
+template <int WM, int WN, bool INSCALE, bool BNB = false>
 __global__ __launch_bounds__(256, (WM * WN >= 8 ? 2 : (WM * WN == 4 ? 3 : 4))) void conv_igemm_kernel(const rpnet_conv_desc d, const int M,
                                                           const int Cin, const int Cout,
                                                           const int tiles_n, const int ntiles) {
@@ -156,21 +156,22 @@
         __syncthreads();
     }
 
-    conv_epilogue<WM, WN>(d, acc, LinearRows{m0, M}, M, Cout, HW, n0, tm, wm, wn, li, h, smem);
-}
-
-template <int WM, int WN, bool INSCALE>
+    conv_epilogue<WM, WN, 2, LinearRows, false, BNB>(d, acc, LinearRows{m0, M}, M, Cout, HW, n0, tm, wm, wn, li, h, smem);
+}
+
+template <int WM, int WN, bool INSCALE, bool BNB = false>
 static int launch_igemm_t(const rpnet_conv_desc* d, int M, int Cin, int Cout, hipStream_t s) {
     constexpr int BM = 64 * WM, BN = 64 * WN;
     const int tiles_m = cdiv(M, BM), tiles_n = Cout / BN;
     const int ntiles = tiles_m * tiles_n;
-    hipLaunchKernelGGL((conv_igemm_kernel<WM, WN, INSCALE>), dim3(ntiles), dim3(256), 0, s, *d, M, Cin, Cout, tiles_n, ntiles);
+    hipLaunchKernelGGL((conv_igemm_kernel<WM, WN, INSCALE, BNB>), dim3(ntiles), dim3(256), 0, s, *d, M, Cin, Cout, tiles_n, ntiles);
     return check_launch("conv_igemm");
 }
 
 template <int WM, int WN>
 static int launch_igemm(const rpnet_conv_desc* d, int M, int Cin, int Cout, hipStream_t s) {
     if (d->in_scale_mode) return launch_igemm_t<WM, WN, true>(d, M, Cin, Cout, s);
+    if (d->bnb_partial) return launch_igemm_t<WM, WN, false, true>(d, M, Cin, Cout, s);
     return launch_igemm_t<WM, WN, false>(d, M, Cin, Cout, s);
 }
 
@@ -197,8 +198,8 @@
     return best;
 }
 
-extern "C" int rpnet_conv_stats_blocks(const rpnet_conv_desc* d) {
-    if (!d || d->groups < 1 || d->N % d->groups) return 0;
+static int tiles_per_group(const rpnet_conv_desc* d, int groups) {
+    if (!d || groups < 1 || d->N % groups) return 0;
     const int M = d->N * d->H * d->W, Cout = d->Co0 + d->Co1;
     int bm, wave_rows = 2;
     if (d->split_planes) {
@@ -207,9 +208,17 @@
         const int best = choose_tile(d, M, Cout);
         bm = (best == 0 || best == 1) ? 128 : 64;
     }
-    const long per_group = (long)(d->N / d->groups) * d->H * d->W;
+    const long per_group = (long)(d->N / groups) * d->H * d->W;
     if (per_group % bm) return 0;
     return (int)(per_group / bm);
+}
+
+extern "C" int rpnet_conv_stats_blocks(const rpnet_conv_desc* d) { return d ? tiles_per_group(d, d->groups) : 0; }
+
+extern "C" int rpnet_conv_bn_bwd_rows(const rpnet_conv_desc* d) {
+    if (!d || d->Co1 || d->y1 || d->stats_partial || d->ep_scale || d->ep_relu || d->in_scale_mode) return 0;
+    if (d->split_planes && rpnet::choose_tile_split(d, d->N * d->H * d->W, d->Co0) < 11) return 0;
+    return tiles_per_group(d, d->bnb_groups);
 }
 
 extern "C" int rpnet_conv_tile_variant(const rpnet_conv_desc* d) {
@@ -239,7 +248,11 @@
     RPNET_REQUIRE(!d->y_split || d->split_out_planes == 3 || d->y_split_scale, RPNET_ERR_ARG,
                   "conv_fwd: fp16 output planes (split_out_planes 1 / 2) need y_split_scale");
     RPNET_REQUIRE(!d->y_enc && !d->y_enc_stride, RPNET_ERR_ARG, "conv_fwd: y_enc / y_enc_stride are reserved (must be NULL / 0)");
-    RPNET_REQUIRE(!d->bnb_y && !d->bnb_stats && !d->bnb_partial && !d->bnb_pmax, RPNET_ERR_ARG, "conv_fwd: the bnb_* fields are reserved (must be NULL)");
+    RPNET_REQUIRE((!d->bnb_y && !d->bnb_stats && !d->bnb_partial && !d->bnb_pmax) || (d->bnb_y && d->bnb_stats && d->bnb_partial),
+                  RPNET_ERR_ARG, "conv_fwd: BatchNorm-backward sums need bnb_y, bnb_stats and bnb_partial");
+    RPNET_REQUIRE(!d->bnb_partial || rpnet_conv_bn_bwd_rows(d) > 0, RPNET_ERR_SHAPE,
+                  "conv_fwd: BatchNorm-backward sums need one destination, no epilogue affine or statistics, and source "
+                  "statistic groups that split into whole tiles; use rpnet_bn_bwd's own reduction pass");
     RPNET_REQUIRE((long)d->N * d->H * d->W < (1L << 31), RPNET_ERR_SHAPE, "conv_fwd: too many pixels");
     RPNET_REQUIRE((size_t)d->N * d->H * d->W * (d->C0 > d->C1 ? d->C0 : d->C1) * 4 < (1UL << 31) &&
                       (size_t)d->taps * Cin * Cout * 4 < (1UL << 31),
diff --git a/rpnet_amd/csrc/conv_split.hip b/rpnet_amd/csrc/conv_split.hip
--- a/rpnet_amd/csrc/conv_split.hip
+++ b/rpnet_amd/csrc/conv_split.hip
@@ -416,7 +416,7 @@
 #pragma unroll
                 for (int r = 0; r < 16; ++r) acc[i][j][r] *= f;
     }
-    conv_epilogue<WM, WN, WGM, LinearRows, NP == 1>(d, acc, LinearRows{m0, M}, M, Cout, HW, n0, tm, wm, wn, li, h, smem);
+    conv_epilogue<WM, WN, WGM, LinearRows, NP == 1, false>(d, acc, LinearRows{m0, M}, M, Cout, HW, n0, tm, wm, wn, li, h, smem);
 }
 
 template <int TW, int NP, int WN>
@@ -596,7 +596,7 @@
             }
         }
     }
-    conv_epilogue<WM, WN, 4, PatchRows<TW>, NP == 1>(d, acc, PatchRows<TW>{(n * H + y0) * W + x0, W}, d.N * HW, Cout, HW, n0, tm, wm, wn,
+    conv_epilogue<WM, WN, 4, PatchRows<TW>, NP == 1, false>(d, acc, PatchRows<TW>{(n * H + y0) * W + x0, W}, d.N * HW, Cout, HW, n0, tm, wm, wn,
                                             li, h, smem);
 }
 
@@ -779,7 +779,7 @@
         __syncthreads();
         if (++tap == 9) { tap = 0; ++ci; }
     }
-    conv_epilogue<WM, WN, 2, PatchRows<TW>, NP == 1>(d, acc, PatchRows<TW>{(n * H + y0) * W + x0, W}, d.N * HW, Cout, HW, n0, tm, wm, wn,
+    conv_epilogue<WM, WN, 2, PatchRows<TW>, NP == 1, false>(d, acc, PatchRows<TW>{(n * H + y0) * W + x0, W}, d.N * HW, Cout, HW, n0, tm, wm, wn,
                                             li, h, smem);
 }
 
diff --git a/rpnet_amd/csrc/conv_split_dma.hip b/rpnet_amd/csrc/conv_split_dma.hip
--- a/rpnet_amd/csrc/conv_split_dma.hip
+++ b/rpnet_amd/csrc/conv_split_dma.hip
@@ -14,7 +14,7 @@
     }
 }
 
-template <int TW, int NP, int WN, bool K64 = false, int WM = 4>
+template <int TW, int NP, int WN, bool K64 = false, int WM = 4, bool BNB = false>
 __global__ __launch_bounds__(256, 1) void conv_igemm_split_dma_kernel(const rpnet_conv_desc d, const int Cin, const int Cout,
                                                                        const int tiles_n, const int ntiles, const int kshift) {
     constexpr int BM = 64 * WM, BN = 64 * WN, TH = BM / TW, PW = TW + 2, HALO = (TH + 2) * PW;
@@ -265,7 +265,7 @@
         if (sacc == 123.456f) d.y0[t] = sacc;
         return;
     }
-    conv_epilogue<WM, WN, 2, PatchRows<TW>, false>(d, acc, PatchRows<TW>{(n * H + y0) * W + x0 + (int)blockIdx.y * d.N * HW, W},
+    conv_epilogue<WM, WN, 2, PatchRows<TW>, false, BNB>(d, acc, PatchRows<TW>{(n * H + y0) * W + x0 + (int)blockIdx.y * d.N * HW, W},
                                                     d.N * HW, Cout, HW, n0, tm, wm, wn, li, h, smem);
 }
 
@@ -369,7 +369,8 @@
     return parts;
 }
 
-int conv_fwd_split_dma(const rpnet_conv_desc* d, int M, int Cin, int Cout, int tw, int wn, hipStream_t s, int parts, int bm) {
+template <bool BNB>
+static int conv_fwd_split_dma_t(const rpnet_conv_desc* d, int M, int Cin, int Cout, int tw, int wn, hipStream_t s, int parts, int bm) {
     const int tiles_m = M / bm, tiles_n = Cout / (64 * wn);
     const int ntiles = tiles_m * tiles_n;
     rpnet_conv_desc dp = *d;
@@ -391,7 +392,7 @@
         dp.out_absmax = nullptr; dp.y_split = nullptr; dp.split_out_planes = 0; dp.y_split_scale = nullptr;
     }
 #define RPNET_DMA(TWV, WNV, K64V) \
-    hipLaunchKernelGGL((conv_igemm_split_dma_kernel<TWV, 2, WNV, K64V>), dim3(ntiles, parts), dim3(256), 0, s, dp, Cin, Cout, tiles_n, ntiles, kshift)
+    hipLaunchKernelGGL((conv_igemm_split_dma_kernel<TWV, 2, WNV, K64V, 4, BNB>), dim3(ntiles, parts), dim3(256), 0, s, dp, Cin, Cout, tiles_n, ntiles, kshift)
     if (d->split_planes == 1) {
         if (wn != 2 || Cin % 64 || d->C0 % 64) {
             set_error("conv_igemm_split_dma: one plane needs 128-wide tiles and channel counts in multiples of 64 per source");
@@ -404,9 +405,9 @@
             return RPNET_ERR_ARG;
         }
         if (tw == 32)
-            hipLaunchKernelGGL((conv_igemm_split_dma_kernel<32, 2, 1, false, 2>), dim3(ntiles, 1), dim3(256), 0, s, dp, Cin, Cout, tiles_n, ntiles, 0);
+            hipLaunchKernelGGL((conv_igemm_split_dma_kernel<32, 2, 1, false, 2, BNB>), dim3(ntiles, 1), dim3(256), 0, s, dp, Cin, Cout, tiles_n, ntiles, 0);
         else
-            hipLaunchKernelGGL((conv_igemm_split_dma_kernel<16, 2, 1, false, 2>), dim3(ntiles, 1), dim3(256), 0, s, dp, Cin, Cout, tiles_n, ntiles, 0);
+            hipLaunchKernelGGL((conv_igemm_split_dma_kernel<16, 2, 1, false, 2, BNB>), dim3(ntiles, 1), dim3(256), 0, s, dp, Cin, Cout, tiles_n, ntiles, 0);
     } else if (d->split_planes == 2) {
         if (wn == 2) { if (tw == 32) RPNET_DMA(32, 2, false); else RPNET_DMA(16, 2, false); }
         else { if (tw == 32) RPNET_DMA(32, 1, false); else RPNET_DMA(16, 1, false); }
@@ -424,4 +425,9 @@
     return check_launch("conv_igemm_split_dma");
 }
 
-}
+int conv_fwd_split_dma(const rpnet_conv_desc* d, int M, int Cin, int Cout, int tw, int wn, hipStream_t s, int parts, int bm) {
+    if (d->bnb_partial) return conv_fwd_split_dma_t<true>(d, M, Cin, Cout, tw, wn, s, parts, bm);
+    return conv_fwd_split_dma_t<false>(d, M, Cin, Cout, tw, wn, s, parts, bm);
+}
+
+}
diff --git a/rpnet_amd/csrc/conv_up4_dma.hip b/rpnet_amd/csrc/conv_up4_dma.hip
--- a/rpnet_amd/csrc/conv_up4_dma.hip
+++ b/rpnet_amd/csrc/conv_up4_dma.hip
@@ -252,10 +252,10 @@
     __builtin_amdgcn_s_barrier();
 
     if constexpr (DG) {
-        conv_epilogue<WM, WN, 2, PatchRows<TW>, false>(d, acc, PatchRows<TW>{(n * Hl + y0) * Wl + x0, Wl}, d.N * Hl * Wl, Ncols, Hl * Wl, n0, tm,
+        conv_epilogue<WM, WN, 2, PatchRows<TW>, false, false>(d, acc, PatchRows<TW>{(n * Hl + y0) * Wl + x0, Wl}, d.N * Hl * Wl, Ncols, Hl * Wl, n0, tm,
                                                         wm, wn, li, h, smem);
     } else {
-        conv_epilogue<WM, WN, 2, PatchRowsUp<TW>, false>(d, acc, PatchRowsUp<TW>{(n * H + 2 * y0 + fpy) * W + 2 * x0 + fpx, 2 * W}, d.N * H * W,
+        conv_epilogue<WM, WN, 2, PatchRowsUp<TW>, false, false>(d, acc, PatchRowsUp<TW>{(n * H + 2 * y0 + fpy) * W + 2 * x0 + fpx, 2 * W}, d.N * H * W,
                                                           Cout_out, H * W, n0 - fphase * Cout_out, tm * 4 + fphase, wm, wn, li, h, smem,
                                                           fphase * Cout_out);
     }
diff --git a/rpnet_amd/functional.py b/rpnet_amd/functional.py
--- a/rpnet_amd/functional.py
+++ b/rpnet_amd/functional.py
@@ -386,10 +386,11 @@
 
 
 class Operand:
-    __slots__ = ("x", "p16", "pbf", "scale", "planes_only", "deferred", "masked")
-
-    def __init__(self, x, p16=None, pbf=None, scale=None, planes_only=False, deferred=None, masked=None):
+    __slots__ = ("x", "p16", "pbf", "scale", "planes_only", "deferred", "masked", "bnb")
+
+    def __init__(self, x, p16=None, pbf=None, scale=None, planes_only=False, deferred=None, masked=None, bnb=None):
         self.x, self.p16, self.pbf, self.scale = x, p16, pbf, scale
+        self.bnb = bnb
         self.deferred = deferred
         self.masked = masked
         self.planes_only = planes_only
@@ -412,6 +413,7 @@
 _EVAL_SPLITK = True
 _POOL_FUSE = True
 _CONV1_BN_FUSE = True
+_BNB_EPILOGUE = os.environ.get("RPNET_BNB_EPILOGUE", "1") == "1"
 _CONV1_RECOMP = True
 _UP4 = True
 _MASK_SKIP = os.environ.get("RPNET_MASK_SKIP", "1") == "1"
@@ -886,6 +888,9 @@
         ctx.save_for_backward(x0, x1, in_scale, weight, gamma, y, stats)
         ctx.yshape = (N, H, W, cout)
         ctx.pw, ctx.cfg, ctx.eval_mode, ctx.pool = pw, (groups, upsample, in_mode, first), False, pool
+        ctx.bnb_link = {"y": y, "stats": stats, "groups": groups} if (_BNB_EPILOGUE and y is not None and not pool) else None
+        produced["bnb_link"] = ctx.bnb_link
+        ctx.bnb_src = op0.bnb if (op0 is not None and x1 is None and in_scale is None and not upsample) else None
         ctx.up4 = (not first) and up4
         ctx.bias, ctx.beta, ctx.xs, ctx.sx, ctx.sx1 = bias, beta, xs, sx, sx1
         ctx.opts = (_ASYNC["on"], _MASK_SKIP)
@@ -978,6 +983,17 @@
         direct = _direct(gamma, async_on) and _direct(beta, async_on) and not bn_eval
         dgamma, dbeta = (None, None) if direct else (_empty((cout,), y), _empty((cout,), y))
         ARITH[("bn_bwd", "eval mode" if bn_eval else "own reduction pass")] += 1
+        link, given = getattr(ctx, "bnb_link", None), None
+        if link is not None:
+            g_dz, part, pmax, rows = (link.pop(k, None) for k in ("dz", "part", "pmax", "rows"))
+            if part is not None and not bn_eval and not ctx.pool and g_dz.data_ptr() == dz.data_ptr() and g_dz.shape == dz.shape:
+                given = (part, pmax, rows)
+                cur = torch.cuda.current_stream(dz.device)
+                if link.get("stream") != cur:
+                    part.record_stream(cur)
+                    pmax.record_stream(cur)
+        if not bn_eval:
+            ARITH[("bn_bwd_sums", "dgrad epilogue" if given is not None else "separate pass")] += 1
         if direct:
             _order_wait(gamma.data_ptr())
         if bn_eval:
@@ -987,7 +1003,8 @@
         else:
             call("rpnet_bn_bwd", ptr(dz), ptr(y), ptr(gamma), ptr(stats[0]), ptr(stats[1]), ptr(stats[2]), ptr(stats[3]),
                  ptr(dy), ptr(dys), np_ if dys is not None else 0, ptr(sdy), ptr(gamma.grad if direct else dgamma),
-                 ptr(beta.grad if direct else dbeta), N, H * W, cout, groups, 1 if direct else 0, None, None, 0,
+                 ptr(beta.grad if direct else dbeta), N, H * W, cout, groups, 1 if direct else 0,
+                 *((ptr(given[0]), ptr(given[1]), given[2]) if given is not None else (None, None, 0)),
                  W if ctx.pool else 0, ptr(ws), wsb, None, 0)
         if direct:
             _order_done(gamma.data_ptr())
@@ -1095,6 +1112,17 @@
                 else:
                     dd = _desc(dy, None, pw.wd, None, None, 0, g0, g1, N, H, W, pw.taps, 0,
                                out_scale=None if need_s else in_scale, out_mode=in_mode)
+                src = getattr(ctx, "bnb_src", None)
+                if src is not None and not up4 and need0 and x1 is None and in_scale is None and not upsample:
+                    dd.bnb_y, dd.bnb_stats, dd.bnb_groups = ptr(src["y"]), ptr(src["stats"]), src["groups"]
+                    rows = query("rpnet_conv_bn_bwd_rows", C.byref(dd))
+                    if rows > 0:
+                        part = torch.empty(src["groups"] * rows * c0 * 2, device=y.device, dtype=torch.float64)
+                        pmax = torch.empty(src["groups"] * rows * c0, device=y.device, dtype=torch.float32)
+                        dd.bnb_partial, dd.bnb_pmax = ptr(part), ptr(pmax)
+                        src.update(dz=g0, part=part, pmax=pmax, rows=rows, stream=torch.cuda.current_stream(y.device))
+                    else:
+                        dd.bnb_y, dd.bnb_stats, dd.bnb_groups = None, None, 0
                 if up4:
                     _cup4(dd, 2)
                 else:
@@ -1138,7 +1166,7 @@
                          bn.running_mean, bn.running_var, bn.num_batches_tracked if training else None, pw, training, groups,
                          1 if upsample else 0, in_mode, out_split, (op0, op1), produced)
     out = Operand(z, produced.get("p16"), produced.get("pbf"), produced.get("scale"), bool(produced.get("planes_only")),
-                  produced.get("deferred"))
+                  produced.get("deferred"), bnb=produced.get("bnb_link"))
     if pool and not produced.get("pooled"):
         out = maxpool2(out)
     return out
diff --git a/rpnet_amd/hip.py b/rpnet_amd/hip.py
--- a/rpnet_amd/hip.py
+++ b/rpnet_amd/hip.py
@@ -45,6 +45,7 @@
     "rpnet_conv_wgrad_up4_workspace_bytes": (cs, [ci, ci, ci, ci, ci]),
     "rpnet_conv_wgrad_up4": (ci, [C.POINTER(ConvDesc), vp, vp, vp, cs, vp]),
     "rpnet_conv_stats_blocks": (ci, [C.POINTER(ConvDesc)]),
+    "rpnet_conv_bn_bwd_rows": (ci, [C.POINTER(ConvDesc)]),
     "rpnet_conv_tile_variant": (ci, [C.POINTER(ConvDesc)]),
     "rpnet_conv_splitk_workspace_bytes": (cs, [C.POINTER(ConvDesc)]),
     "rpnet_bn_stats_from_partial": (ci, [vp, ci, ci, ci, ci, ci, vp, vp, vp, vp, vp, cf, cf, vp, vp, vp, vp, vp]),
@@ -120,7 +121,7 @@
     "rpnet_debug_mfma_spin": (ci, [ci, ci, C.c_longlong, vp, vp]),
 }
 ABI_SYMBOLS = tuple(_SIGS)
-ABI_VERSION = 109
+ABI_VERSION = 110
 
 
 def lib_path():
```

Measured after the change: 512.9 (median of 6 runs). About the same (+0.8%).
